# synthesizer-project/synference

Measured on AMD Instinct MI355X. Metric: posterior samples/sec (accepted, prior-box rejection included), higher is better.
Workload: dtype f32

## Files before the change

include/synference_hip.h:

```cpp
#ifndef SYNFERENCE_HIP_H
#define SYNFERENCE_HIP_H

#include <stddef.h>
#include <stdint.h>

#ifdef __cplusplus
extern "C" {
#endif

typedef struct sf_flow sf_flow;
typedef struct sf_opt sf_opt;

enum sf_status {
  SF_OK = 0,
  SF_ERR_INVALID = -1,
  SF_ERR_HIP = -2,
  SF_ERR_NO_DEVICE = -3,
  SF_ERR_STATE = -4
};

enum sf_kind { SF_MAF = 0, SF_NSF = 1, SF_NSF_AR = 2, SF_MAF_AR = 3 };

typedef struct sf_flow_desc {
  int32_t kind;
  int32_t D;
  int32_t C;
  int32_t H;
  int32_t T;
  int32_t K;
  int32_t NB;
  int32_t scale_fn;
  int32_t hidden_bf16;
  float tail_bound;
  float min_bin_width;
  float min_bin_height;
  float min_derivative;
  float maf_eps;
  float lu_eps;
  const float* theta_mean;
  const float* theta_std;
  const float* x_mean;
  const float* x_std;
  const int32_t* perms;
  float ar_slope;
} sf_flow_desc;

int sf_flow_create(const sf_flow_desc* desc, sf_flow** out);
void sf_flow_destroy(sf_flow* f);
int64_t sf_flow_num_params(const sf_flow* f);
int64_t sf_flow_packed_size(const sf_flow* f);

int sf_flow_set_params(sf_flow* f, const float* flat, int64_t n, int is_device, void* stream);

int sf_flow_get_params(sf_flow* f, float* flat, int64_t n, int is_device, void* stream);

int sf_flow_pack_table(const sf_flow* f, int32_t* src1, int32_t* src2, int64_t n_packed);
int64_t sf_flow_packed16_size(const sf_flow* f);
int sf_flow_pack_table16(const sf_flow* f, int32_t* src1, int32_t* src2, int64_t n_packed16);
int64_t sf_flow_packed16b_size(const sf_flow* f);
int sf_flow_pack_table16b(const sf_flow* f, int32_t* src, int64_t n);
int64_t sf_flow_trainc_size(const sf_flow* f);
int64_t sf_flow_trainc_grad_size(const sf_flow* f);
int sf_flow_trainc_table(const sf_flow* f, int32_t* src1, int32_t* src2, int64_t n, int32_t* gdst, int64_t n_params,
                         int32_t* desc , float* cst, int64_t n_cst);
int64_t sf_flow_cst_size(const sf_flow* f);
int sf_flow_train_path(const sf_flow* f, int64_t B, int want_dctx);
int sf_flow_describe(const sf_flow* f, char* buf, size_t buflen);

int sf_flow_log_prob(sf_flow* f, const float* theta , const float* x ,
                     int64_t B, float* out , void* stream);

int sf_flow_log_prob_grad(sf_flow* f, const float* theta , const float* x, int64_t rows_per_x, int64_t B,
                          float* lp , float* dtheta , void* stream);

int sf_map_step(int64_t B, int64_t D, float* phi , float* exp_avg , float* exp_avg_sq ,
                float* theta , const float* lp , const float* g_theta , const float* lo ,
                const float* hi , float* best_theta , float* best_lp , float learning_rate,
                int64_t step, int save_best, void* stream);

int sf_flow_inverse_from_noise(sf_flow* f, const float* z , const float* x ,
                               int64_t B, float* theta , float* logdet ,
                               void* stream);
int sf_flow_inverse_from_noise_sampler(sf_flow* f, const float* z , const float* x , int64_t B,
                                       float* theta , void* stream);
int sf_set_sampler_fp32(int on);

int sf_flow_sample_round(sf_flow* f, const float* x , int64_t S,
                         const uint32_t* slots, int64_t slot_base, int64_t n_slots,
                         uint32_t attempt, int32_t attempts_per_slot, uint64_t seed, uint32_t stream_id,
                         const float* lo , const float* hi ,
                         float* out , uint32_t* rejected, uint32_t* n_rejected,
                         int32_t* n_drawn, void* stream);

int sf_flow_prepare_context(sf_flow* f, const float* x , int64_t M, void* stream);
int sf_flow_release_context(sf_flow* f);

int sf_flow_sample(sf_flow* f, const float* x , int64_t M, int64_t S,
                   const float* lo, const float* hi, uint64_t seed, int32_t max_attempts,
                   float* out , int32_t* n_drawn , int64_t* n_unfilled ,
                   void* stream);

int sf_flow_set_sample_row_offset(sf_flow* f, int64_t row_offset);
int sf_flow_set_sample_output_f64(sf_flow* f, int on);
int sf_flow_set_sample_time_limit(sf_flow* f, double seconds);

int sf_flow_sample_slots(sf_flow* f, const float* x , int64_t M, int64_t S,
                         const uint32_t* slots, int64_t n_slots, const float* lo, const float* hi, uint64_t seed,
                         int32_t max_attempts, float* out , int64_t* n_unfilled , void* stream);

int sf_flow_sample_stats(const sf_flow* f, float* stats4);

int sf_flow_acceptance(sf_flow* f, const float* x , int64_t M, int64_t n,
                       const float* lo, const float* hi, uint64_t seed,
                       int32_t* count , void* stream);

int sf_flow_loss_grad(sf_flow* f, const float* flat , const float* theta, const float* x,
                      int64_t B, float grad_scale, float* loss , float* grad ,
                      void* stream);

int sf_flow_loss_grad_rows(sf_flow* f, const float* flat, const float* theta , const float* x ,
                           const int64_t* rows , int64_t B, float grad_scale, const float* weights,
                           float* loss, double* loss_sum, float* grad, float* dctx, void* stream);


int sf_flow_loss_grad_weighted(sf_flow* f, const float* flat, const float* theta, const float* x,
                               int64_t B, float grad_scale, const float* weights ,
                               float* loss, float* grad, float* dctx , void* stream);

int sf_flow_set_profiling(sf_flow* f, int on);
int sf_flow_train_stats(sf_flow* f, float* kernel_ms );

typedef struct sf_adam_desc {
  float lr, beta1, beta2, eps, weight_decay;
  int32_t decoupled;
} sf_adam_desc;
int sf_opt_create(int64_t n, const sf_adam_desc* d, sf_opt** out);
void sf_opt_destroy(sf_opt* o);
int sf_adam_step(sf_opt* o, float* params, const float* grad, float max_norm,
                 float* grad_norm_out, void* stream);
int sf_adam_apply(float* params, const float* grad, float* exp_avg, float* exp_avg_sq, int64_t n,
                  const sf_adam_desc* d, int64_t step, float max_norm, float* scratch, void* stream);

int sf_flow_train_epoch(sf_flow* f, float* flat, const float* theta, const float* x, const int64_t* order,
                        int64_t n_batches, int64_t batch, float grad_scale, float* exp_avg, float* exp_avg_sq,
                        const sf_adam_desc* d, int64_t step0, float max_norm, float* scratch ,
                        float* grad , double* loss_sum, void* stream);

#define SF_COMM_ID_BYTES 128
typedef struct sf_comm sf_comm;
int sf_comm_set_library(const char* path);
int sf_comm_library(char* path_out, int64_t cap, int* version_out);
int sf_comm_unique_id(void* id_out, int64_t bytes);
int sf_comm_create(const void* id, int64_t bytes, int nranks, int rank, sf_comm** out);
void sf_comm_destroy(sf_comm* c);
int sf_comm_info(const sf_comm* c, int* nranks, int* rank);
int sf_comm_all_reduce_sum(sf_comm* c, float* buf , int64_t n, void* stream);
int sf_flow_train_epoch_dp(sf_flow* f, float* flat, const float* theta, const float* x, const int64_t* order,
                           int64_t n_batches, int64_t batch, float grad_scale, float* exp_avg, float* exp_avg_sq,
                           const sf_adam_desc* d, int64_t step0, float max_norm, float* scratch ,
                           float* grad , double* loss_sum, sf_comm* comm, void* stream);
int sf_opt_state(sf_opt* o, float** exp_avg, float** exp_avg_sq, int64_t** step_host);

typedef struct sf_mlp sf_mlp;
enum sf_act { SF_ACT_SILU = 0, SF_ACT_RELU = 1, SF_ACT_TANH = 2 };
typedef struct sf_mlp_desc {
  int32_t n_in;
  int32_t n_layers;
  int32_t widths[4];
  int32_t act;
  const float* x_mean;
  const float* x_std;
} sf_mlp_desc;
int sf_mlp_create(const sf_mlp_desc* d, sf_mlp** out);
void sf_mlp_destroy(sf_mlp* m);
int64_t sf_mlp_num_params(const sf_mlp* m);
int sf_mlp_forward(sf_mlp* m, const float* flat, const float* x , int64_t B,
                   float* out , void* stream);
int sf_mlp_backward(sf_mlp* m, const float* flat, const float* x, const float* dout ,
                    int64_t B, float* grad , void* stream);

int sf_quantiles(const float* samples , int64_t N, int64_t S, int32_t D,
                 const float* q , int32_t Q, float* out , void* stream);
int sf_quantiles_large(const float* samples , int64_t N, int64_t S, int32_t D,
                       const float* q , int32_t Q, float* out , void* stream);

int sf_flux_to_abmag(const float* flux_njy, const float* err_njy, int64_t n, float mag_limit,
                     float* mag, float* mag_err, void* stream);

int sf_flux_to_asinh(const float* flux_njy, const float* err_njy, int64_t N, int32_t C, const float* f_b_njy ,
                     float* mag, float* mag_err, void* stream);

int sf_scatter_depths(const float* flux , int64_t N, int32_t C, const float* sigma, int32_t n_sigma_rows,
                      int32_t n_scatters, float min_flux_pc_error, uint64_t seed,
                      float* out , float* err_out, void* stream);

#define SF_NOISE_KIND_GENERAL 0
#define SF_NOISE_KIND_ASINH 1
#define SF_NOISE_SPACE_PHYSICAL 0
#define SF_NOISE_SPACE_AB 1
#define SF_NOISE_SPACE_ASINH 2
#define SF_NOISE_FLUX_SCATTER 0
#define SF_NOISE_FLUX_LIMIT 1
#define SF_NOISE_FLUX_NUMBER 2
typedef struct sf_noise_band {
  int32_t kind;
  int32_t interp_space;
  int32_t in_space;
  int32_t out_space;
  int32_t n_bins;
  int32_t table_offset;
  int32_t extrapolate;
  int32_t resample;
  int32_t upper_limits;
// ... 134 lines not shown
```

synference_amd/_lib.py:

```python
from __future__ import annotations

import ctypes as C
import os
from pathlib import Path

_HERE = Path(__file__).resolve().parent
LIB_PATH = _HERE / "lib" / "libsynference_hip.so"

c_f32p = C.POINTER(C.c_float)
c_i32p = C.POINTER(C.c_int32)
c_u32p = C.POINTER(C.c_uint32)


class sf_flow_desc(C.Structure):
    _fields_ = [
        ("kind", C.c_int32), ("D", C.c_int32), ("C", C.c_int32), ("H", C.c_int32),
        ("T", C.c_int32), ("K", C.c_int32), ("NB", C.c_int32), ("scale_fn", C.c_int32),
        ("hidden_bf16", C.c_int32),
        ("tail_bound", C.c_float), ("min_bin_width", C.c_float), ("min_bin_height", C.c_float),
        ("min_derivative", C.c_float), ("maf_eps", C.c_float), ("lu_eps", C.c_float),
        ("theta_mean", c_f32p), ("theta_std", c_f32p), ("x_mean", c_f32p), ("x_std", c_f32p),
        ("perms", c_i32p), ("ar_slope", C.c_float),
    ]


class sf_mlp_desc(C.Structure):
    _fields_ = [("n_in", C.c_int32), ("n_layers", C.c_int32), ("widths", C.c_int32 * 4), ("act", C.c_int32),
                ("x_mean", c_f32p), ("x_std", c_f32p)]


class sf_adam_desc(C.Structure):
    _fields_ = [("lr", C.c_float), ("beta1", C.c_float), ("beta2", C.c_float), ("eps", C.c_float),
                ("weight_decay", C.c_float), ("decoupled", C.c_int32)]


class sf_noise_band(C.Structure):
    _fields_ = [(n, C.c_int32) for n in ("kind", "interp_space", "in_space", "out_space", "n_bins", "table_offset",
                                         "extrapolate", "resample", "upper_limits", "has_limit", "flux_rule", "replace_err")] + \
               [(n, C.c_float) for n in ("in_to_unit", "zp_in", "zp_unit", "zp_out", "unit_to_out", "in_to_jy", "unit_per_jy",
                                         "jy_per_unit", "b_jy", "sigma_clip", "snr_threshold", "limit_value", "flux_number",
                                         "std_at_limit", "err_value", "min_err", "max_err")]


class sf_spectra_desc(C.Structure):
    _fields_ = [(n, C.c_void_p) for n in ("flux", "wave", "z", "sigma_pixels", "observed_wave", "curve_wave", "curve_r",
                                          "theory_r_arr", "norm_table", "out")] + \
               [(n, C.c_int64) for n in ("N", "ld_flux", "ld_out", "sigma_stride")] + \
               [(n, C.c_int32) for n in ("mode", "L", "M", "n_curve", "col0", "norm_frame", "unit_code", "med_lo", "med_hi",
                                         "h_limit")] + \
               [("theory_r", C.c_double), ("trunc", C.c_double)] + \
               [(n, C.c_float) for n in ("unit_scale", "clip_lo", "clip_hi")]


class sf_c2st_desc(C.Structure):
    _fields_ = [(n, C.c_int32) for n in ("n_in", "width", "n_cls", "max_iter", "n_iter_no_change", "early_stopping", "batch")] + \
               [("R", C.c_int64), ("seed", C.c_uint64)] + \
               [(n, C.c_float) for n in ("lr", "beta1", "beta2", "eps", "alpha")] + \
               [("tol", C.c_double)] + \
               [(n, C.c_void_p) for n in ("rows", "labels", "vmask", "init_weights")]


PROTOTYPES = {
    "sf_flow_create": (C.c_int, [C.POINTER(sf_flow_desc), C.POINTER(C.c_void_p)]),
    "sf_flow_destroy": (None, [C.c_void_p]),
    "sf_flow_num_params": (C.c_int64, [C.c_void_p]),
    "sf_flow_packed_size": (C.c_int64, [C.c_void_p]),
    "sf_flow_set_params": (C.c_int, [C.c_void_p, C.c_void_p, C.c_int64, C.c_int, C.c_void_p]),
    "sf_flow_pack_table": (C.c_int, [C.c_void_p, c_i32p, c_i32p, C.c_int64]),
    "sf_flow_describe": (C.c_int, [C.c_void_p, C.c_char_p, C.c_size_t]),
    "sf_flow_log_prob": (C.c_int, [C.c_void_p, C.c_void_p, C.c_void_p, C.c_int64, C.c_void_p, C.c_void_p]),
    "sf_flow_log_prob_grad": (C.c_int, [C.c_void_p, C.c_void_p, C.c_void_p, C.c_int64, C.c_int64, C.c_void_p, C.c_void_p,
                                        C.c_void_p]),
    "sf_map_step": (C.c_int, [C.c_int64, C.c_int64, C.c_void_p, C.c_void_p, C.c_void_p, C.c_void_p, C.c_void_p, C.c_void_p,
                              C.c_void_p, C.c_void_p, C.c_void_p, C.c_void_p, C.c_float, C.c_int64, C.c_int, C.c_void_p]),
    "sf_flow_inverse_from_noise": (C.c_int, [C.c_void_p, C.c_void_p, C.c_void_p, C.c_int64, C.c_void_p,
                                             C.c_void_p, C.c_void_p]),
    "sf_flow_sample_round": (C.c_int, [C.c_void_p, C.c_void_p, C.c_int64, C.c_void_p, C.c_int64, C.c_int64,
                                       C.c_uint32, C.c_int32, C.c_uint64, C.c_uint32, C.c_void_p, C.c_void_p,
                                       C.c_void_p, C.c_void_p, C.c_void_p, C.c_void_p, C.c_void_p]),
    "sf_flux_to_asinh": (C.c_int, [C.c_void_p, C.c_void_p, C.c_int64, C.c_int32, C.c_void_p, C.c_void_p, C.c_void_p,
                                   C.c_void_p]),
    "sf_scatter_depths": (C.c_int, [C.c_void_p, C.c_int64, C.c_int32, C.c_void_p, C.c_int32, C.c_int32, C.c_float, C.c_uint64,
                                    C.c_void_p, C.c_void_p, C.c_void_p]),
    "sf_scatter_empirical": (C.c_int, [C.c_void_p, C.c_int64, C.c_int32, C.POINTER(sf_noise_band), c_f32p, C.c_int64, C.c_int32,
                                       C.c_uint64, C.c_void_p, C.c_void_p, C.c_void_p]),
    "sf_apply_scalings": (C.c_int, [C.c_void_p, C.c_void_p, C.c_int64, C.c_int32, C.POINTER(sf_noise_band), c_f32p, C.c_int64,
                                    C.c_void_p, C.c_void_p, C.c_void_p]),
    "sf_spectra_transform": (C.c_int, [C.POINTER(sf_spectra_desc), C.c_void_p]),
    "sf_pit_ranks": (C.c_int, [C.c_void_p, C.c_void_p, C.c_int64, C.c_int64, C.c_int32, C.c_void_p, C.c_void_p]),
    "sf_tarp_coverage": (C.c_int, [C.c_void_p, C.c_void_p, C.c_int64, C.c_int64, C.c_int32, C.c_void_p, C.c_int32, C.c_int32,
                                   C.c_int32, C.c_int32, C.c_uint64, C.c_void_p, C.c_void_p, C.c_void_p, C.c_void_p,
                                   C.c_void_p]),
    "sf_copy_to_host_f64": (C.c_int, [C.c_void_p, C.c_void_p, C.c_int64, C.c_void_p]),
    "sf_flow_packed16_size": (C.c_int64, [C.c_void_p]),
    "sf_flow_pack_table16": (C.c_int, [C.c_void_p, C.c_void_p, C.c_void_p, C.c_int64]),
    "sf_flow_packed16b_size": (C.c_int64, [C.c_void_p]),
    "sf_flow_inverse_from_noise_sampler": (C.c_int, [C.c_void_p, C.c_void_p, C.c_void_p, C.c_int64, C.c_void_p, C.c_void_p]),
    "sf_set_sampler_fp32": (C.c_int, [C.c_int]),
    "sf_flow_set_sample_row_offset": (C.c_int, [C.c_void_p, C.c_int64]),
    "sf_flow_train_path": (C.c_int, [C.c_void_p, C.c_int64, C.c_int]),
    "sf_flow_trainc_size": (C.c_int64, [C.c_void_p]),
    "sf_flow_trainc_grad_size": (C.c_int64, [C.c_void_p]),
    "sf_flow_cst_size": (C.c_int64, [C.c_void_p]),
    "sf_flow_trainc_table": (C.c_int, [C.c_void_p, C.c_void_p, C.c_void_p, C.c_int64, C.c_void_p, C.c_int64, C.c_void_p,
                                       C.c_void_p, C.c_int64]),
    "sf_flow_pack_table16b": (C.c_int, [C.c_void_p, C.c_void_p, C.c_int64]),
    "sf_flow_get_params": (C.c_int, [C.c_void_p, C.c_void_p, C.c_int64, C.c_int, C.c_void_p]),
    "sf_flow_prepare_context": (C.c_int, [C.c_void_p, C.c_void_p, C.c_int64, C.c_void_p]),
    "sf_flow_release_context": (C.c_int, [C.c_void_p]),
    "sf_flow_sample": (C.c_int, [C.c_void_p, C.c_void_p, C.c_int64, C.c_int64, C.c_void_p, C.c_void_p,
                                 C.c_uint64, C.c_int32, C.c_void_p, C.c_void_p, C.POINTER(C.c_int64),
                                 C.c_void_p]),
    "sf_flow_sample_slots": (C.c_int, [C.c_void_p, C.c_void_p, C.c_int64, C.c_int64, C.c_void_p, C.c_int64, C.c_void_p,
                                       C.c_void_p, C.c_uint64, C.c_int32, C.c_void_p, C.POINTER(C.c_int64), C.c_void_p]),
    "sf_flow_sample_stats": (C.c_int, [C.c_void_p, C.POINTER(C.c_float)]),
    "sf_flow_acceptance": (C.c_int, [C.c_void_p, C.c_void_p, C.c_int64, C.c_int64, C.c_void_p, C.c_void_p,
                                     C.c_uint64, C.c_void_p, C.c_void_p]),
    "sf_flow_loss_grad": (C.c_int, [C.c_void_p, C.c_void_p, C.c_void_p, C.c_void_p, C.c_int64, C.c_float,
                                    C.c_void_p, C.c_void_p, C.c_void_p]),
    "sf_flow_loss_grad_rows": (C.c_int, [C.c_void_p, C.c_void_p, C.c_void_p, C.c_void_p, C.c_void_p, C.c_int64,
                                         C.c_float, C.c_void_p, C.c_void_p, C.c_void_p, C.c_void_p, C.c_void_p,
                                         C.c_void_p]),
    "sf_flow_train_epoch": (C.c_int, [C.c_void_p, C.c_void_p, C.c_void_p, C.c_void_p, C.c_void_p, C.c_int64, C.c_int64,
                                      C.c_float, C.c_void_p, C.c_void_p, C.POINTER(sf_adam_desc), C.c_int64, C.c_float,
                                      C.c_void_p, C.c_void_p, C.c_void_p, C.c_void_p]),
    "sf_flow_train_epoch_dp": (C.c_int, [C.c_void_p, C.c_void_p, C.c_void_p, C.c_void_p, C.c_void_p, C.c_int64, C.c_int64,
                                         C.c_float, C.c_void_p, C.c_void_p, C.POINTER(sf_adam_desc), C.c_int64, C.c_float,
                                         C.c_void_p, C.c_void_p, C.c_void_p, C.c_void_p, C.c_void_p]),
    "sf_comm_set_library": (C.c_int, [C.c_char_p]),
    "sf_comm_library": (C.c_int, [C.c_char_p, C.c_int64, C.POINTER(C.c_int)]),
    "sf_comm_unique_id": (C.c_int, [C.c_void_p, C.c_int64]),
    "sf_comm_create": (C.c_int, [C.c_void_p, C.c_int64, C.c_int, C.c_int, C.POINTER(C.c_void_p)]),
    "sf_comm_destroy": (None, [C.c_void_p]),
    "sf_comm_info": (C.c_int, [C.c_void_p, C.POINTER(C.c_int), C.POINTER(C.c_int)]),
    "sf_comm_all_reduce_sum": (C.c_int, [C.c_void_p, C.c_void_p, C.c_int64, C.c_void_p]),
    "sf_flow_loss_grad_weighted": (C.c_int, [C.c_void_p, C.c_void_p, C.c_void_p, C.c_void_p, C.c_int64,
                                             C.c_float, C.c_void_p, C.c_void_p, C.c_void_p, C.c_void_p,
                                             C.c_void_p]),
    "sf_flow_set_sample_time_limit": (C.c_int, [C.c_void_p, C.c_double]),
    "sf_flow_set_sample_output_f64": (C.c_int, [C.c_void_p, C.c_int]),
    "sf_flow_set_profiling": (C.c_int, [C.c_void_p, C.c_int]),
    "sf_flow_train_stats": (C.c_int, [C.c_void_p, C.POINTER(C.c_float)]),
    "sf_opt_create": (C.c_int, [C.c_int64, C.POINTER(sf_adam_desc), C.POINTER(C.c_void_p)]),
    "sf_opt_destroy": (None, [C.c_void_p]),
    "sf_adam_step": (C.c_int, [C.c_void_p, C.c_void_p, C.c_void_p, C.c_float, C.c_void_p, C.c_void_p]),
    "sf_adam_apply": (C.c_int, [C.c_void_p, C.c_void_p, C.c_void_p, C.c_void_p, C.c_int64,
                                C.POINTER(sf_adam_desc), C.c_int64, C.c_float, C.c_void_p, C.c_void_p]),
    "sf_opt_state": (C.c_int, [C.c_void_p, C.POINTER(C.c_void_p), C.POINTER(C.c_void_p),
                               C.POINTER(C.POINTER(C.c_int64))]),
    "sf_mlp_create": (C.c_int, [C.POINTER(sf_mlp_desc), C.POINTER(C.c_void_p)]),
    "sf_mlp_destroy": (None, [C.c_void_p]),
    "sf_mlp_num_params": (C.c_int64, [C.c_void_p]),
    "sf_mlp_forward": (C.c_int, [C.c_void_p, C.c_void_p, C.c_void_p, C.c_int64, C.c_void_p, C.c_void_p]),
    "sf_mlp_backward": (C.c_int, [C.c_void_p, C.c_void_p, C.c_void_p, C.c_void_p, C.c_int64, C.c_void_p,
                                  C.c_void_p]),
    "sf_quantiles": (C.c_int, [C.c_void_p, C.c_int64, C.c_int64, C.c_int32, C.c_void_p, C.c_int32, C.c_void_p,
                               C.c_void_p]),
    "sf_quantiles_large": (C.c_int, [C.c_void_p, C.c_int64, C.c_int64, C.c_int32, C.c_void_p, C.c_int32, C.c_void_p,
                                     C.c_void_p]),
    "sf_impute_missing": (C.c_int, [C.c_void_p, C.c_int64, C.c_int32, c_i32p, c_i32p, C.c_int32, C.c_void_p, C.c_void_p,
                                    C.c_void_p, C.c_int64, C.c_int64, C.c_float, C.c_float, C.c_float, C.c_int32, C.c_int32,
                                    C.c_float, C.c_int32, C.c_uint64, C.c_void_p, C.c_void_p, C.c_void_p, C.c_void_p,
                                    C.c_void_p, C.c_void_p, C.c_int64, C.c_void_p, C.c_void_p]),
    "sf_knn": (C.c_int, [C.c_void_p, C.c_int64, C.c_int32, C.c_void_p, C.c_int64, C.c_int32, C.c_int32, C.c_int64, C.c_void_p,
                         C.c_void_p, C.c_void_p]),
    "sf_kde_logsumexp": (C.c_int, [C.c_void_p, C.c_int64, C.c_int32, C.c_void_p, C.c_int64, C.c_void_p, C.c_void_p]),
    "sf_c2st_create": (C.c_int, [C.POINTER(sf_c2st_desc), C.POINTER(C.c_void_p), C.c_void_p]),
    "sf_c2st_destroy": (None, [C.c_void_p]),
    "sf_c2st_num_params": (C.c_int64, [C.c_void_p]),
    "sf_c2st_train": (C.c_int, [C.c_void_p, C.c_int32, C.c_int32, C.c_int32, C.c_int32, C.POINTER(C.c_int32), C.c_void_p]),
    "sf_c2st_scores": (C.c_int, [C.c_void_p, C.c_int32, C.c_int32, C.c_void_p, C.c_int64, C.c_void_p, C.c_void_p, C.c_void_p]),
    "sf_c2st_get": (C.c_int, [C.c_void_p, C.c_void_p, C.c_void_p, C.c_void_p, C.c_void_p]),
    "sf_flux_to_abmag": (C.c_int, [C.c_void_p, C.c_void_p, C.c_int64, C.c_float, C.c_void_p, C.c_void_p, C.c_void_p]),
    "sf_last_error": (C.c_char_p, []),
    "sf_version": (C.c_char_p, []),
    "sf_device_count": (C.c_int, []),
}

_lib = None


def load() -> C.CDLL:
    global _lib
    if _lib is not None:
        return _lib
    path = Path(os.environ.get("SYNFERENCE_HIP_LIB", LIB_PATH))
    if not path.exists():
        raise RuntimeError(
            f"{path} not found: build it with `python -c 'import __graft_entry__ as g; g.build()'` "
            "(hipcc --offload-arch=gfx950).  There is no CPU fallback for the flow engine.")
    lib = C.CDLL(str(path))
    for name, (res, args) in PROTOTYPES.items():
        fn = getattr(lib, name)
        fn.restype = res
        fn.argtypes = args
    _lib = lib
    return lib


def ptr(t):
    return None if t is None else C.c_void_p(t.data_ptr())


def stream_ptr(device):
    import torch
    return C.c_void_p(torch.cuda.current_stream(device).cuda_stream)


def check(rc: int) -> None:
    if rc != 0:
        msg = load().sf_last_error().decode("utf-8", "replace")
        raise RuntimeError(f"synference_hip error {rc}: {msg}")
```

synference_amd/csrc/sf_api.hip:

```cpp
#include <hip/hip_runtime.h>

#include <chrono>
#include <cmath>
#include <cstdio>
#include <cstdlib>
#include <cstring>
#include <string>
#include <vector>

#include "sf_internal.h"
#include "sf_train.h"
#include "sf_nsf1.h"
#include "sf_nsfar.h"
#include "sf_nsfc.h"
#include "sf_trainc.h"

namespace {
thread_local std::string g_err;

int hip_fail(hipError_t e, const char* what) {
  return sf_fail(SF_ERR_HIP, std::string(what) + ": " + hipGetErrorString(e));
}
}

static int ensure_device(sf_flow* f) {
  if (f->dev_ready) return SF_OK;
  int n = 0;
  if (hipGetDeviceCount(&n) != hipSuccess || n == 0)
    return sf_fail(SF_ERR_NO_DEVICE, "no HIP device visible: the gfx950 flow engine has no CPU fallback");
  SfFlowDev d;
  if (f->nsf1 || f->nsfar) {
    SF_TRY_SET(d.d_flat.alloc((size_t)f->L.n_params));
    static_cast<SfFlowDev&>(*f) = std::move(d);
    f->dev_ready = true;
    return SF_OK;
  }
  const size_t np = (size_t)f->L.n_packed;
  SF_TRY_SET(d.d_packed.alloc(np));
  SF_TRY_SET(hipMemset(d.d_packed, 0, np * sizeof(float)));
  SF_TRY_SET(d.d_cst.upload(f->L.cst));
  SF_TRY_SET(d.d_s1.alloc(np));
  SF_TRY_SET(d.d_s2.alloc(np));
  SF_TRY_SET(hipMemcpy(d.d_s1, f->L.src1.data(), np * sizeof(int32_t), hipMemcpyHostToDevice));
  SF_TRY_SET(hipMemcpy(d.d_s2, f->L.src2.data(), np * sizeof(int32_t), hipMemcpyHostToDevice));
  if ((f->L.dev.m16_ok || f->L.nsfS.ok) && f->L.n_packed16 > 0) {
    const size_t n16 = (size_t)f->L.n_packed16;
    SF_TRY_SET(d.d_packed16.alloc(n16));
    SF_TRY_SET(d.d_s16a.alloc(n16));
    SF_TRY_SET(d.d_s16b.alloc(n16));
    SF_TRY_SET(hipMemcpy(d.d_s16a, f->L.src16a.data(), n16 * sizeof(int32_t), hipMemcpyHostToDevice));
    SF_TRY_SET(hipMemcpy(d.d_s16b, f->L.src16b.data(), n16 * sizeof(int32_t), hipMemcpyHostToDevice));
  }
  if ((f->L.dev.m16_ok || f->L.nsfS.ok) && f->L.n_packed16B > 0) {
    const size_t nB = (size_t)f->L.n_packed16B;
    SF_TRY_SET(d.d_packed16B.alloc(nB));
    SF_TRY_SET(d.d_s16B.alloc(nB));
    SF_TRY_SET(hipMemcpy(d.d_s16B, f->L.src16B.data(), nB * sizeof(int32_t), hipMemcpyHostToDevice));
  }
  if (f->L.n_packedB > 0) {
    SF_TRY_SET(d.d_packedB.alloc((size_t)f->L.n_packedB));
    SF_TRY_SET(d.d_bsrc.alloc((size_t)f->L.n_packedB));
    SF_TRY_SET(hipMemcpy(d.d_bsrc, f->L.srcB.data(), (size_t)f->L.n_packedB * sizeof(int32_t), hipMemcpyHostToDevice));
  }
  SF_TRY_SET(d.d_flat.alloc((size_t)f->L.n_params));
  SF_TRY_SET(d.d_cnt.alloc(SF_MAX_ROUNDS));
  SF_TRY_SET(d.h_cnt.alloc(SF_MAX_ROUNDS));
  SF_TRY_SET(d.ev_dense[0].create());
  SF_TRY_SET(d.ev_dense[1].create());
  static_cast<SfFlowDev&>(*f) = std::move(d);
  f->dev_ready = true;
  return SF_OK;
}

sf_flow::~sf_flow() {
  sf_nsf1_destroy(nsf1);
  sf_nsfar_destroy(nsfar);
}

extern "C" {

const char* sf_last_error(void) { return g_err.c_str(); }
const char* sf_version(void) { return "synference_hip 0.2 (gfx950; mfma_f32_32x32x2 / 16x16x4)"; }
int sf_device_count(void) {
  int n = 0;
  if (hipGetDeviceCount(&n) != hipSuccess) return 0;
  return n;
}

int sf_flow_create(const sf_flow_desc* desc, sf_flow** out) {
  if (!desc || !out) return sf_fail(SF_ERR_INVALID, "null argument");
  if (desc->kind == SF_NSF && desc->D == 1) {
    sf_flow* f1 = new sf_flow();
    std::string err;
    int rc = sf_nsf1_create(*desc, &f1->nsf1, err);
    if (rc) { delete f1; return sf_fail(rc, err); }
    std::memset(&f1->L.dev, 0, sizeof(f1->L.dev));
    std::memset(&f1->L.trc, 0, sizeof(f1->L.trc));
    std::memset(&f1->L.nsc, 0, sizeof(f1->L.nsc));
    std::memset(&f1->L.nsfS, 0, sizeof(f1->L.nsfS));
    SfDev& v = f1->L.dev;
    v.kind = SF_NSF; v.D = 1; v.C = desc->C; v.H = desc->H; v.T = desc->T; v.K = desc->K; v.NB = desc->NB;
    f1->L.n_params = (int64_t)desc->T * f1->nsf1->P_mlp;
    *out = f1;
    return SF_OK;
  }
  if (desc->kind == SF_NSF_AR || desc->kind == SF_MAF_AR) {
    sf_flow* fa = new sf_flow();
    std::string err;
    int rc = sf_nsfar_create(*desc, &fa->nsfar, err);
    if (rc) { delete fa; return sf_fail(rc, err); }
    std::memset(&fa->L.dev, 0, sizeof(fa->L.dev));
    std::memset(&fa->L.trc, 0, sizeof(fa->L.trc));
    std::memset(&fa->L.nsc, 0, sizeof(fa->L.nsc));
    std::memset(&fa->L.nsfS, 0, sizeof(fa->L.nsfS));
    SfDev& v = fa->L.dev;
    v.kind = desc->kind; v.D = desc->D; v.C = desc->C; v.H = desc->H; v.T = desc->T; v.K = desc->K; v.NB = desc->NB;
    fa->L.n_params = fa->nsfar->n_params;
    *out = fa;
    return SF_OK;
  }
  sf_flow* f = new sf_flow();
  if (!sf_build_layout(*desc, f->L)) {
    std::string e = f->L.error;
    delete f;
    return sf_fail(SF_ERR_INVALID, e);
  }
  *out = f;
  return SF_OK;
}

void sf_flow_destroy(sf_flow* f) { delete f; }

int64_t sf_flow_num_params(const sf_flow* f) { return f ? f->L.n_params : 0; }
int64_t sf_flow_packed_size(const sf_flow* f) { return !f ? 0 : (f->nsfar ? (int64_t)f->nsfar->src.size() : f->L.n_packed); }

int sf_flow_pack_table(const sf_flow* f, int32_t* src1, int32_t* src2, int64_t n_packed) {
  if (!f || !src1 || !src2) return sf_fail(SF_ERR_INVALID, "null argument");
  if (f->nsfar) {
    if (n_packed != (int64_t)f->nsfar->src.size()) return sf_fail(SF_ERR_INVALID, "n_packed mismatch");
    std::memcpy(src1, f->nsfar->src.data(), (size_t)n_packed * sizeof(int32_t));
    for (int64_t i = 0; i < n_packed; ++i) src2[i] = -1;
    return SF_OK;
  }
  if (n_packed != f->L.n_packed) return sf_fail(SF_ERR_INVALID, "n_packed mismatch");
  if (n_packed == 0) return SF_OK;
  std::memcpy(src1, f->L.src1.data(), (size_t)n_packed * sizeof(int32_t));
  std::memcpy(src2, f->L.src2.data(), (size_t)n_packed * sizeof(int32_t));
  return SF_OK;
}

int64_t sf_flow_packed16_size(const sf_flow* f) { return (f && f->L.dev.m16_ok) ? f->L.n_packed16 : 0; }

int sf_flow_pack_table16(const sf_flow* f, int32_t* src1, int32_t* src2, int64_t n_packed16) {
  if (!f || !src1 || !src2) return sf_fail(SF_ERR_INVALID, "null argument");
  if (!f->L.dev.m16_ok || n_packed16 != f->L.n_packed16) return sf_fail(SF_ERR_INVALID, "no 16-row image or size mismatch");
  std::memcpy(src1, f->L.src16a.data(), (size_t)n_packed16 * sizeof(int32_t));
  std::memcpy(src2, f->L.src16b.data(), (size_t)n_packed16 * sizeof(int32_t));
  return SF_OK;
}

int64_t sf_flow_packed16b_size(const sf_flow* f) { return (f && f->L.dev.m16_ok) ? f->L.n_packed16B : 0; }

int sf_flow_pack_table16b(const sf_flow* f, int32_t* src, int64_t n) {
  if (!f || !src) return sf_fail(SF_ERR_INVALID, "null argument");
  if (!f->L.dev.m16_ok || n != f->L.n_packed16B) return sf_fail(SF_ERR_INVALID, "no split-bf16 image or size mismatch");
  std::memcpy(src, f->L.src16B.data(), (size_t)n * sizeof(int32_t));
  return SF_OK;
}

int64_t sf_flow_trainc_size(const sf_flow* f) { return (f && (f->L.trc.ok || f->L.nsc.ok)) ? f->L.n_imgC : 0; }
int64_t sf_flow_trainc_grad_size(const sf_flow* f) { return (f && (f->L.trc.ok || f->L.nsc.ok)) ? f->L.n_gradC : 0; }
int64_t sf_flow_cst_size(const sf_flow* f) { return f ? (int64_t)f->L.cst.size() : 0; }
int sf_flow_trainc_table(const sf_flow* f, int32_t* src1, int32_t* src2, int64_t n, int32_t* gdst, int64_t n_params,
                         int32_t* desc, float* cst, int64_t n_cst) {
  if (!f || !src1 || !src2 || !gdst || !desc || !cst) return sf_fail(SF_ERR_INVALID, "null argument");
  if ((!f->L.trc.ok && !f->L.nsc.ok) || n != f->L.n_imgC || n_params != f->L.n_params || n_cst != (int64_t)f->L.cst.size())
    return sf_fail(SF_ERR_INVALID, "no cooperative training image or size mismatch");
  static_assert(sizeof(SfTrcDev) <= 64 * sizeof(int32_t) && sizeof(SfNscDev) <= 64 * sizeof(int32_t), "descriptor words");
  std::memcpy(src1, f->L.srcC1.data(), (size_t)n * sizeof(int32_t));
  std::memcpy(src2, f->L.srcC2.data(), (size_t)n * sizeof(int32_t));
  std::memcpy(gdst, f->L.gdstC.data(), (size_t)n_params * sizeof(int32_t));
  std::memset(desc, 0, 64 * sizeof(int32_t));
  if (f->L.trc.ok) std::memcpy(desc, &f->L.trc, sizeof(SfTrcDev));
  else std::memcpy(desc, &f->L.nsc, sizeof(SfNscDev));
  std::memcpy(cst, f->L.cst.data(), (size_t)n_cst * sizeof(float));
  return SF_OK;
}

int sf_flow_describe(const sf_flow* f, char* buf, size_t buflen) {
  if (!f || !buf) return sf_fail(SF_ERR_INVALID, "null argument");
  const SfDev& v = f->L.dev;
  std::string s = "{";
  auto add = [&](const char* k, long val) { s += "\"" + std::string(k) + "\": " + std::to_string(val) + ", "; };
  if (f->nsfar) {
    const SfNsfAr& n = *f->nsfar;
    add("kind", n.affine ? SF_MAF_AR : SF_NSF_AR); add("D", n.D); add("C", n.C); add("H", n.H); add("T", n.T); add("K", n.K); add("NB", 2);
    add("Hp", n.Hp); add("t_stride", n.t_stride); add("n_params", (long)n.n_params); add("n_packed", (long)n.src.size());
    add("o_L0t", n.o_L0t); add("o_b0", n.o_b0); add("o_L1t", n.o_L1t); add("o_L1m", n.o_L1m); add("o_b1", n.o_b1);
    add("o_L2t", n.o_L2t); add("o_b2", n.o_b2); add("o_L0m", n.o_L0m); add("o_L2m", n.o_L2m); add("lds_bytes_train", (long)sf_nsfar_lds_bytes(n, 3));
    add("sampler_tiles16", sf_nsfar16_eligible(n) ? 1 : 0); add("s16_nt", n.s16_nt); add("s16_ni", n.s16_ni); add("s16_ks", n.s16_ks); add("s16_tpt", n.s16_tpt);
    add("o_F0", n.o_F0); add("o_fb0", n.o_fb0); add("o_F1", n.o_F1); add("o_fb1", n.o_fb1); add("o_F2", n.o_F2);
    auto arr = [&](const char* k, const std::vector<int32_t>& a, bool last) {
      s += "\"" + std::string(k) + "\": [";
      for (size_t i = 0; i < a.size(); ++i) s += std::to_string(a[i]) + (i + 1 < a.size() ? ", " : "");
      s += last ? "]}" : "], ";
    };
    arr("perm", n.perm, false); arr("ptype", n.ptype, false); arr("tend", n.tend, false); arr("ord", n.ord, false); arr("dimof", n.dimof, true);
    if (s.size() + 1 > buflen) return sf_fail(SF_ERR_INVALID, "buffer too small");
    std::memcpy(buf, s.c_str(), s.size() + 1);
    return SF_OK;
  }
  add("kind", v.kind); add("D", v.D); add("C", v.C); add("H", v.H); add("T", v.T); add("K", v.K);
  add("NB", v.NB); add("HT", v.HT); add("PT", v.PT); add("KMAX", v.KMAX); add("JP", v.JP);
  add("nGu", v.nGu); add("nGc", v.nGc); add("nGh", v.nGh); add("t_stride", v.t_stride);
  add("o_w0", v.o_w0); add("o_wc", v.o_wc); add("o_b0", v.o_b0); add("o_wk0", v.o_wk[0]);
  add("o_bk0", v.o_bk[0]); add("o_wk1", v.o_wk[1]); add("o_bk1", v.o_bk[1]); add("o_wf", v.o_wf);
  add("o_wk2", v.o_wk[2]); add("o_bk2", v.o_bk[2]); add("o_wk3", v.o_wk[3]); add("o_bk3", v.o_bk[3]);
  add("scale_fn", v.scale_fn);
  add("o_bf", v.o_bf); add("o_winu", v.o_winu); add("o_winc", v.o_winc); add("o_bin", v.o_bin);
  add("o_wg0", v.o_wg[0]); add("o_bg0", v.o_bg[0]); add("o_w10", v.o_w1[0]); add("o_b10", v.o_b1[0]);
  add("o_w20", v.o_w2[0]); add("o_b20", v.o_b2[0]); add("o_wg1", v.o_wg[1]); add("o_bg1", v.o_bg[1]);
  add("o_w11", v.o_w1[1]); add("o_b11", v.o_b1[1]); add("o_w21", v.o_w2[1]); add("o_b21", v.o_b2[1]);
  add("o_wout", v.o_wout); add("o_bout", v.o_bout); add("o_lu", v.o_lu);
  add("c_pscale", v.c_pscale); add("c_pshift", v.c_pshift); add("c_tdim", v.c_tdim);
  add("c_xmean", v.c_xmean); add("c_xstd", v.c_xstd); add("c_dslot", v.c_dslot);
  add("nsf_split_sampler", f->L.nsfS.ok); add("trainc_ok", f->L.trc.ok); add("nsfc_ok", f->L.nsc.ok);
  add("inc_ok", v.inc_ok); add("hidden_bf16", v.hidden_bf16); add("tB_stride", v.tB_stride); add("n_parts", v.n_parts); add("part_max", v.part_max);
  add("n_params", f->L.n_params); add("n_packed", f->L.n_packed);
  {
    int R = 0, NV = 0;
    SfDev vv = v;
    vv.packed16 = reinterpret_cast<const float*>(1);
    sf_ctab_shape(vv, R, NV);
    add("ctab_floats_per_galaxy", (long)v.T * NV * R);
  }
  add("o16_w0", v.o16_w0); add("o16_wc", v.o16_wc); add("o16_b0", v.o16_b0); add("o16_wk0", v.o16_wk[0]);
  add("o16_wk1", v.o16_wk[1]); add("o16_bk0", v.o16_bk[0]); add("o16_bk1", v.o16_bk[1]); add("o16_hv", v.o16_hv);
  add("o16_hvb", v.o16_hvb); add("o16_wh", v.o16_wh); add("o16_bh", v.o16_bh); add("o16_wp", v.o16_wp); add("t16_a_tab", v.t16_a_tab);
  add("t16_a", v.t16_a); add("t16B_stride", v.t16B_stride); add("nP16", v.nP16); add("o16B_wk0", v.o16B_wk[0]); add("o16B_wk1", v.o16B_wk[1]);
  add("m16_ok", v.m16_ok); add("m16_span", v.m16_span); add("nT16", v.nT16); add("nC16", v.nC16); add("t16_stride", v.t16_stride);
  s += "\"g16_tile\": [";
  for (int i = 0; i < SF_DMAX; ++i) s += std::to_string(v.g16_tile[i]) + (i + 1 < SF_DMAX ? ", " : "], ");
  s += "\"g16_lo\": [";
  for (int i = 0; i < SF_DMAX; ++i) s += std::to_string(v.g16_lo[i]) + (i + 1 < SF_DMAX ? ", " : "], ");
  s += "\"g_kend\": [";
  for (int i = 0; i < SF_DMAX; ++i) s += std::to_string(v.g_kend[i]) + (i + 1 < SF_DMAX ? ", " : "], ");
  s += "\"g_lo\": [";
  for (int i = 0; i < SF_DMAX; ++i) s += std::to_string(v.g_lo[i]) + (i + 1 < SF_DMAX ? ", " : "], ");
  s += "\"g_tile\": [";
  for (int i = 0; i < SF_DMAX; ++i) s += std::to_string(v.g_tile[i]) + (i + 1 < SF_DMAX ? ", " : "], ");
  s += "\"mt_kend\": [";
  for (int i = 0; i < 4; ++i) s += std::to_string(v.mt_kend[i]) + (i + 1 < 4 ? ", " : "], ");
  s += "\"cst\": [";
  for (size_t i = 0; i < f->L.cst.size(); ++i) {
    char t[40];
    std::snprintf(t, sizeof(t), "%.9g%s", f->L.cst[i], i + 1 < f->L.cst.size() ? ", " : "");
    s += t;
  }
  s += "]}";
  if (s.size() + 1 > buflen) return sf_fail(SF_ERR_INVALID, "buffer too small");
  std::memcpy(buf, s.c_str(), s.size() + 1);
  return SF_OK;
}

int sf_flow_set_params(sf_flow* f, const float* flat, int64_t n, int is_device, void* stream) {
  if (!f || !flat) return sf_fail(SF_ERR_INVALID, "null argument");
  if (n != f->L.n_params) return sf_fail(SF_ERR_INVALID, "parameter count mismatch");
  int rc = ensure_device(f);
  if (rc) return rc;
  hipStream_t st = (hipStream_t)stream;
  SF_TRY_SET(hipMemcpyAsync(f->d_flat, flat, (size_t)n * sizeof(float), is_device ? hipMemcpyDeviceToDevice : hipMemcpyHostToDevice, st));
  const float* src = f->d_flat;
  f->flat_valid = true;
  f->gt_image_valid = false;
  if (f->nsf1) { f->params_set = true; return SF_OK; }
  if (f->nsfar) {
    std::string err;
    rc = sf_nsfar_pack(f->nsfar, src, st, err);
    if (rc) return sf_fail(rc, err);
    f->params_set = true;
    return SF_OK;
  }
  SF_TRY_SET(sf_launch_pack(src, f->d_s1, f->d_s2, f->d_packed, (long)f->L.n_packed, st));
  if (f->d_packed16) SF_TRY_SET(sf_launch_pack(src, f->d_s16a, f->d_s16b, f->d_packed16, (long)f->L.n_packed16, st));
  f->wp_stale = true;
  if (f->d_packed16B) SF_TRY_SET(sf_launch_pack_bf16_split(src, f->d_s16B, f->d_packed16B, (long)f->L.n_packed16B, st));
  f->packed16_stale = false;
  if (f->L.n_packedB > 0) SF_TRY_SET(sf_launch_pack_bf16(src, f->d_bsrc, f->d_packedB, (long)f->L.n_packedB, st));
  f->params_set = true;
  f->ctab_x = nullptr;
  return SF_OK;
}

int sf_flow_get_params(sf_flow* f, float* flat, int64_t n, int is_device, void* stream) {
  if (!f || !flat) return sf_fail(SF_ERR_INVALID, "null argument");
  if (n != f->L.n_params) return sf_fail(SF_ERR_INVALID, "parameter count mismatch");
  if (!f->params_set || !f->flat_valid)
    return sf_fail(SF_ERR_STATE, "no parameters held by the handle: after sf_flow_loss_grad the caller's vector is the master copy "
                              "(call sf_flow_set_params first)");
  hipStream_t st = (hipStream_t)stream;
  SF_TRY_SET(hipMemcpyAsync(flat, f->d_flat, (size_t)n * sizeof(float), is_device ? hipMemcpyDeviceToDevice : hipMemcpyDeviceToHost, st));
  if (!is_device) SF_TRY_SET(hipStreamSynchronize(st));
  return SF_OK;
}

int sf_flow_log_prob(sf_flow* f, const float* theta, const float* x, int64_t B, float* out, void* stream) {
  if (!f) return sf_fail(SF_ERR_INVALID, "null handle");
  if (B == 0) return SF_OK;
  if (!theta || !x || !out) return sf_fail(SF_ERR_INVALID, "null argument");
  if (!f->params_set) return sf_fail(SF_ERR_STATE, "sf_flow_set_params has not been called");
  if (B < 0) return sf_fail(SF_ERR_INVALID, "B < 0");
  if (f->nsf1) {
    std::string err;
    int rc = sf_nsf1_log_prob(f->nsf1, f->d_flat, theta, x, (long)B, out, (hipStream_t)stream, err);
    return rc ? sf_fail(rc, err) : SF_OK;
  }
  if (f->nsfar) {
    std::string err;
    int rc = sf_nsfar_log_prob(f->nsfar, theta, x, (long)B, out, (hipStream_t)stream, err);
    return rc ? sf_fail(rc, err) : SF_OK;
  }
  SF_TRY_SET(sf_launch_logprob(f->dev(), theta, x, (long)B, out, (hipStream_t)stream));
  return SF_OK;
}

int sf_flow_inverse_from_noise(sf_flow* f, const float* z, const float* x, int64_t B, float* theta,
                               float* logdet, void* stream) {
  if (!f) return sf_fail(SF_ERR_INVALID, "null handle");
  if (B == 0) return SF_OK;
  if (!z || !x || !theta) return sf_fail(SF_ERR_INVALID, "null argument");
  if (!f->params_set) return sf_fail(SF_ERR_STATE, "sf_flow_set_params has not been called");
  if (f->nsf1) {
    std::string err;
    int rc = sf_nsf1_inverse(f->nsf1, f->d_flat, z, x, (long)B, theta, logdet, (hipStream_t)stream, err);
    return rc ? sf_fail(rc, err) : SF_OK;
  }
  if (f->nsfar) {
    std::string err;
    int rc = sf_nsfar_inverse(f->nsfar, z, x, (long)B, theta, logdet, (hipStream_t)stream, err);
    return rc ? sf_fail(rc, err) : SF_OK;
  }
  SfSampleArgsHost a;
  a.x = x; a.z_in = z; a.n_items = (long)B; a.out = theta; a.logdet_out = logdet;
  SF_TRY_SET(sf_launch_inverse(f->dev(), a, (hipStream_t)stream));
  return SF_OK;
}

static void nsf_sampler_view(const sf_flow* f, SfDev& m);
static SfDev sampler_dev(const sf_flow* f, const float* x);
int sf_flow_inverse_from_noise_sampler(sf_flow* f, const float* z, const float* x, int64_t B, float* theta, void* stream) {
  if (!f) return sf_fail(SF_ERR_INVALID, "null handle");
  if (B == 0) return SF_OK;
  if (!z || !x || !theta) return sf_fail(SF_ERR_INVALID, "null argument");
  if (!f->params_set) return sf_fail(SF_ERR_STATE, "sf_flow_set_params has not been called");
  if (f->nsf1 || f->nsfar) {
    int rc = sf_flow_inverse_from_noise(f, z, x, B, theta, nullptr, stream);
    return rc ? rc : 1;
  }
  if (f->L.dev.kind == SF_NSF) {
    SfDev ms = f->dev();
    nsf_sampler_view(f, ms);
    SfSampleArgsHost a;
    a.x = x; a.z_in = z; a.n_items = (long)B; a.out = theta;
    SF_TRY_SET(sf_launch_inverse(ms, a, (hipStream_t)stream));
    return ms.hidden_bf16 == 2 ? SF_OK : 1;
  }
  const SfDev m = f->dev();
  const SfMaf16Plan pl = sf_maf16_plan(m);
  if (!pl.sampler16) {
    SfSampleArgsHost a;
    a.x = x; a.z_in = z; a.n_items = (long)B; a.out = theta;
    SF_TRY_SET(sf_launch_inverse(m, a, (hipStream_t)stream));
    return 1;
  }
  if (pl.fp32) {
    int rc = sf_flow_prepare_context(f, x, B, stream);
    if (rc) return rc;
    const SfDev mt = sampler_dev(f, x);
    if (sf_maf16_plan(mt).fused) {
      SfSampleArgsHost a;
      a.x = x; a.z_in = z; a.n_items = (long)B; a.out = theta; a.S = 1;
      hipError_t e = sf_launch_maf_find16_zin(mt, a, (hipStream_t)stream);
      (void)sf_flow_release_context(f);
      if (e != hipSuccess) return hip_fail(e, "sf_launch_maf_find16_zin");
      return 3;
    }
    (void)sf_flow_release_context(f);
  }
  SF_TRY_SET(sf_launch_maf_inv16b_hook(m, z, x, (long)B, theta, (hipStream_t)stream));
  return pl.fp32 ? 2 : SF_OK;
}

extern "C++" {
static int g_sampler_fp32 = -2;
void sf_sampler_fp32_set(int on) { g_sampler_fp32 = on < 0 ? -1 : (on ? 1 : 0); }
int sf_sampler_fp32_get() {
  if (g_sampler_fp32 == -2) { const char* e = std::getenv("SF_SAMPLER_FP32"); g_sampler_fp32 = (e && *e) ? (std::atoi(e) != 0 ? 1 : 0) : -1; }
  return g_sampler_fp32;
}
int sf_sampler_fp32_for(int kind) {
  const int g = sf_sampler_fp32_get();
  return g < 0 ? (kind == SF_MAF ? 1 : 0) : g;
}
}
int sf_set_sampler_fp32(int on) {
  sf_sampler_fp32_set(on);
  return SF_OK;
}

int sf_flow_train_path(const sf_flow* f, int64_t B, int want_dctx) {
  if (!f) return sf_fail(SF_ERR_INVALID, "null handle");
  if (f->nsf1) return 4;
  if (f->nsfar) return 5;
  if (B > 0 && sf_trainc_eligible(f->L, want_dctx != 0)) return sf_trainc_groups((long)B, &f->L.trc, f->L.dev.T);
  if (B > 0 && sf_nsfc_eligible(f->L, want_dctx != 0)) return 3;
  return 0;
}

static void seed_keys(uint64_t seed, uint32_t stream_id, uint32_t& k0, uint32_t& k1) {
  k0 = (uint32_t)(seed & 0xffffffffu);
  k1 = (uint32_t)(seed >> 32) ^ stream_id;
}

static size_t ctab_limit_bytes() {
  static long v = -1;
  if (v < 0) {
    const char* e = std::getenv("SF_CTAB_MAX_MB");
    v = e ? std::atol(e) : 4096;
  }
  return (size_t)v << 20;
}

int sf_flow_prepare_context(sf_flow* f, const float* x, int64_t M, void* stream) {
  if (!f) return sf_fail(SF_ERR_INVALID, "null handle");
  f->ctab_x = nullptr;
  f->ctab_M = 0;
  if (M == 0) return SF_OK;
  if (!x) return sf_fail(SF_ERR_INVALID, "null argument");
  if (M < 0) return sf_fail(SF_ERR_INVALID, "M < 0");
  if (!f->params_set) return sf_fail(SF_ERR_STATE, "sf_flow_set_params has not been called");
  if (f->nsf1 || f->nsfar) return SF_OK;
  SfDev m = f->dev();
  int R = 0, NV = 0;
  sf_ctab_shape(m, R, NV);
  const size_t need = (size_t)M * m.T * NV * R;
  if (need == 0 || need * sizeof(float) > ctab_limit_bytes()) return SF_OK;
  SF_TRY_SET(f->d_ctab.grow(need));
  m.ctab_R = R; m.ctab_NV = NV;
  if (f->wp_stale && m.kind == SF_MAF && m.m16_ok && m.packed16 && m.o16_wp >= 0) {
    SF_TRY_SET(sf_launch_maf_fuse16(m, (hipStream_t)stream));
    f->wp_stale = false;
  }
  SF_TRY_SET(sf_launch_ctab(m, x, (long)M, f->d_ctab, (hipStream_t)stream));
  f->ctab_x = x;
  f->ctab_M = M;
  return SF_OK;
}

int sf_flow_release_context(sf_flow* f) {
  if (!f) return sf_fail(SF_ERR_INVALID, "null handle");
  f->ctab_x = nullptr;
  f->ctab_M = 0;
  return SF_OK;
}

static void nsf_sampler_view(const sf_flow* f, SfDev& m) {
  const SfNsfSamp& s = f->L.nsfS;
  if (m.kind != SF_NSF || !s.ok || m.hidden_bf16 || !f->d_packed16 || !f->d_packed16B || f->packed16_stale || sf_sampler_fp32_for(SF_NSF)) return;
  m.packed = f->d_packed16;
  m.t_stride = s.t_stride;
  m.o_winu = s.o_winu; m.o_winc = s.o_winc; m.o_bin = s.o_bin; m.o_wout = s.o_wout; m.o_bout = s.o_bout; m.o_lu = s.o_lu;
  for (int k = 0; k < SF_NBMAX; ++k) {
    m.o_wg[k] = s.o_wg[k]; m.o_bg[k] = s.o_bg[k]; m.o_b1[k] = s.o_b1[k]; m.o_b2[k] = s.o_b2[k];
    m.o_w1[k] = 0; m.o_w2[k] = 0;
    m.oB_w1[k] = s.oB_w1[k]; m.oB_w2[k] = s.oB_w2[k];
  }
  m.n_parts = s.n_parts; m.part_max = s.part_floats_max; m.part_bytes_max = s.part_bytes_max; m.head_part = s.head_part;
  for (int p = 0; p < 5; ++p) { m.part_off[p] = s.part_off[p]; m.partB_off[p] = s.partB_off[p]; }
  for (int k = 0; k < SF_NBMAX; ++k) m.blk_part[k] = s.blk_part[k];
  m.packedB = f->d_packed16B;
  m.tB_stride = s.tB_stride;
  m.hidden_bf16 = 2;
  m.packed16 = nullptr; m.packed16B = nullptr;
}
static SfDev sampler_dev(const sf_flow* f, const float* x) {
  SfDev m = f->dev();
  if (f->ctab_x != nullptr && f->ctab_x == x) {
    sf_ctab_shape(m, m.ctab_R, m.ctab_NV);
    m.ctab = f->d_ctab;
  }
  nsf_sampler_view(f, m);
  return m;
}

int sf_flow_sample_round(sf_flow* f, const float* x, int64_t S, const uint32_t* slots, int64_t slot_base,
                         int64_t n_slots, uint32_t attempt, int32_t attempts_per_slot, uint64_t seed,
                         uint32_t stream_id,
                         const float* lo, const float* hi, float* out, uint32_t* rejected,
                         uint32_t* n_rejected, int32_t* n_drawn, void* stream) {
  if (!f || !x || !out || !rejected || !n_rejected) return sf_fail(SF_ERR_INVALID, "null argument");
  if (f->nsf1 || f->nsfar) return sf_fail(SF_ERR_INVALID, "sf_flow_sample_round is not offered for the one-parameter / autoregressive NSF: use sf_flow_sample / sf_flow_sample_slots");
  if (!f->params_set) return sf_fail(SF_ERR_STATE, "sf_flow_set_params has not been called");
  if (S < 1 || S > 0x7fffffffll) return sf_fail(SF_ERR_INVALID, "S must be in 1 .. 2^31-1");
  if ((lo == nullptr) != (hi == nullptr)) return sf_fail(SF_ERR_INVALID, "lo and hi must be given together");
  if ((uint64_t)(slot_base + n_slots) > 0xffffffffull)
    return sf_fail(SF_ERR_INVALID, "slot ids must fit 32 bits: split the catalogue");
  const int A = attempts_per_slot;
  if (A < 1 || A > 32 || (A & (A - 1))) return sf_fail(SF_ERR_INVALID, "attempts_per_slot must be 1,2,4,8,16 or 32");
  SfSampleArgsHost a;
  a.x = x; a.S = (long)S; a.slots = slots; a.slot_base = (long)slot_base; a.n_items = (long)n_slots * A;
  a.attempts_per_slot = A; a.attempt = attempt; seed_keys(seed, stream_id, a.k0, a.k1);
  a.rng_slot_offset = (unsigned long long)f->sample_row_offset * (unsigned long long)S;
  a.lo = lo; a.hi = hi; a.out = out; a.rejected = rejected; a.n_rejected = n_rejected; a.n_drawn = n_drawn;
  if (f->ctab_x == x && (uint64_t)(slot_base + n_slots) > (uint64_t)f->ctab_M * (uint64_t)S && slots == nullptr)
    return sf_fail(SF_ERR_INVALID, "slots reach past the rows given to sf_flow_prepare_context");
  SF_TRY_SET(sf_launch_inverse(sampler_dev(f, x), a, (hipStream_t)stream));
  return SF_OK;
}

static int ensure_queue(sf_flow* f, int64_t n_slots, int64_t M) {
  if (!f->d_queue) SF_TRY_SET(f->d_queue.alloc(1));
  if (!f->h_queue) SF_TRY_SET(f->h_queue.alloc(1));
  uint64_t cap = 1u << 16;
  while (cap < (uint64_t)n_slots && cap < (1ull << 20)) cap <<= 1;
  if (f->d_ring.cap() < cap) {
    SF_TRY_SET(f->d_ring.grow(cap));
    hipError_t e = hipMemset(f->d_ring, 0, cap * sizeof(unsigned long long));
    if (e != hipSuccess) { (void)f->d_ring.reset(); return hip_fail(e, "hipMemset(retry ring)"); }
    f->ring_dirty = false;
  }
  if (f->d_rej[0].cap() < (size_t)n_slots) {
    static_cast<SfFlowRej&>(*f) = SfFlowRej();
    SfFlowRej r;
    SF_TRY_SET(r.d_rej[0].alloc((size_t)n_slots));
    SF_TRY_SET(r.d_rej[1].alloc((size_t)n_slots));
    static_cast<SfFlowRej&>(*f) = std::move(r);
  }
  SF_TRY_SET(f->d_galacc.grow((size_t)M));
  return SF_OK;
}

static int sample_persistent(sf_flow* f, const float* x, int64_t M, int64_t S, const uint32_t* slots, int64_t n_slots,
                             const float* lo, const float* hi, uint64_t seed, int32_t max_attempts, float* out,
                             int32_t* n_drawn, int64_t* n_unfilled, hipStream_t st) {
  if (n_unfilled) *n_unfilled = 0;
  if (n_slots == 0) return SF_OK;
  if ((uint64_t)(M * S) > 0xfff00000ull) return sf_fail(SF_ERR_INVALID, "M*S must stay below 2^32 - 2^20: split the catalogue");
  int rc = ensure_queue(f, n_slots, M);
  if (rc) return rc;
  const bool capped = max_attempts > 0;
  const uint32_t ceiling = capped ? (uint32_t)max_attempts : 0x40000000u;
  {
    rc = sf_flow_prepare_context(f, x, M, (void*)st);
    if (rc) return rc;
  }
  const SfDev m = sampler_dev(f, x);
  SfSampleArgsHost a;
  a.x = x; a.S = (long)S; seed_keys(seed, 0, a.k0, a.k1);
  a.rng_slot_offset = (unsigned long long)f->sample_row_offset * (unsigned long long)S;
  a.lo = lo; a.hi = hi; a.out = out; a.n_drawn = n_drawn; a.out_f64 = f->sample_out_f64 ? 1 : 0;
  a.q = f->d_queue; a.ring = f->d_ring; a.ring_mask = (uint32_t)(f->d_ring.cap() - 1);
  a.out_slots = (uint32_t)(M * S);
  const uint32_t* cur = slots;
  int64_t pending = n_slots;
  const auto t_start = std::chrono::steady_clock::now();
  auto out_of_time = [&]() {
    return f->sample_time_limit_s > 0.0 &&
           std::chrono::duration<double>(std::chrono::steady_clock::now() - t_start).count() > f->sample_time_limit_s;
  };
  const bool fast16 = m.kind == SF_MAF && m.m16_ok && !m.hidden_bf16 && m.packed16 != nullptr;
  const uint32_t first_window = fast16 ? 1024u : 256u;
  uint32_t attempt = 0, limit = ceiling < first_window ? ceiling : first_window;
  int buf = 0, stage = 0;
  double evals = 0.0;
  float rej0 = 0.f;
  int64_t dropped = 0;
  const bool progress_rule = !capped;
  uint32_t acc_from = 64;
  const uint64_t S_rule = slots ? 1ull : (uint64_t)S;
  auto rule_due = [&](uint32_t att_now) { return progress_rule && (uint64_t)(att_now - acc_from) * S_rule >= 100000ull; };
  int64_t persist_min = 8192;
  {
    static long env_pm = -1;
    if (env_pm < 0) { const char* e = std::getenv("SF_PERSIST_MIN"); env_pm = e ? std::atol(e) : 0; }
    if (env_pm > 0) persist_min = env_pm;
  }
  for (;;) {
    if (f->ring_dirty) SF_TRY_SET(hipMemsetAsync(f->d_ring, 0, f->d_ring.cap() * sizeof(unsigned long long), st));
    f->ring_dirty = true;
    SF_TRY_SET(hipMemsetAsync(f->d_queue, 0, sizeof(SfQueue), st));
#ifdef SF_Q_STATS
    SF_TRY_SET(hipMemsetAsync(&f->d_queue->stats[10], 0xff, sizeof(unsigned long long), st));
#endif
    if (progress_rule && stage == 0) SF_TRY_SET(hipMemsetAsync(f->d_galacc, 0, (size_t)M * sizeof(int32_t), st));
    a.slots = cur; a.slot_base = 0; a.n_items = (long)pending; a.n_total = (uint32_t)pending;
    {
      static int env_il = -1;
      if (env_il < 0) { const char* e = std::getenv("SF_INTERLEAVE"); env_il = e ? std::atoi(e) : 128; }
      a.dense_G = (!cur && env_il > 0 && pending == M * S && M > 1 && (int64_t)env_il * S < (int64_t)1 << 31) ? (uint32_t)env_il : 0u;
      {
        uint32_t run = fast16 ? 16u : 32u;
        while (run > 1 && S % (int64_t)run != 0) run >>= 1;
        a.dense_run = run;
// ... 461 lines not shown
```

synference_amd/csrc/sf_internal.h:

```cpp
#pragma once
#include <hip/hip_runtime.h>
#include <stdint.h>

#include "sf_buf.h"
#include "sf_layout.h"
#include "sf_queue.h"

struct SfSampleArgsHost {
  const float* x = nullptr;
  const float* z_in = nullptr;
  long S = 1;
  const uint32_t* slots = nullptr;
  long slot_base = 0;
  long n_items = 0;
  uint32_t attempt = 0, k0 = 0, k1 = 0;
  unsigned long long rng_slot_offset = 0;
  int attempts_per_slot = 1;
  int log2_attempts = 0;
  const float* lo = nullptr;
  const float* hi = nullptr;
  float* out = nullptr;
  int out_f64 = 0;
  float* logdet_out = nullptr;
  uint32_t* rejected = nullptr;
  uint32_t* n_rejected = nullptr;
  int32_t* n_drawn = nullptr;
  int32_t* count = nullptr;
  uint32_t* best = nullptr;
  const uint32_t* att_list = nullptr;
  struct SfQueue* q = nullptr;
  unsigned long long* ring = nullptr;
  uint32_t ring_mask = 0;
  uint32_t attempt_limit = 0xffffffffu;
  uint32_t n_total = 0;
  uint32_t out_slots = 0;
  uint32_t dense_G = 0;
  uint32_t dense_run = 1;
  uint32_t list_mul = 0, list_log2 = 0;
  int32_t* gal_acc = nullptr;
#ifdef SF_Q_STATS
  uint32_t* qtrace = nullptr;
#endif
};
#ifdef __HIPCC__
__device__ __forceinline__ void sf_out_store(const SfSampleArgsHost& a, size_t idx, float v) {
  if (a.out_f64) reinterpret_cast<double*>(a.out)[idx] = (double)v;
  else a.out[idx] = v;
}
#endif


hipError_t sf_launch_logprob(const SfDev& m, const float* theta, const float* x, long B, float* out,
                             hipStream_t st);
hipError_t sf_launch_inverse(const SfDev& m, const SfSampleArgsHost& a, hipStream_t st);
bool sf_maf16_enabled(const SfDev& m, const SfSampleArgsHost& a);
hipError_t sf_launch_maf_inv16(const SfDev& m, const SfSampleArgsHost& a, hipStream_t st);
hipError_t sf_launch_maf_inv16b_hook(const SfDev& m, const float* z, const float* x, long n, float* out, hipStream_t st);
void sf_sampler_fp32_set(int on);
int sf_sampler_fp32_get();
int sf_sampler_fp32_for(int kind);
void sf_ctab_shape(const SfDev& m, int& R, int& NV);
hipError_t sf_launch_ctab(const SfDev& m, const float* x, long M, float* tab, hipStream_t st);
hipError_t sf_launch_maf_ctab16(const SfDev& m, const float* x, long M, float* tab, hipStream_t st);
hipError_t sf_launch_maf_fuse16(const SfDev& m, hipStream_t st);
struct SfMaf16Plan {
  bool ok16 = false;
  bool sampler16 = false;
  bool fp32 = false;
  bool span = false;
  bool head_mfma = false;
  int dd = 0;
  bool fused = false;
};
SfMaf16Plan sf_maf16_plan(const SfDev& m);
hipError_t sf_launch_maf_find16_zin(const SfDev& m, const SfSampleArgsHost& a, hipStream_t st);
hipError_t sf_launch_pack(const float* flat, const int32_t* s1, const int32_t* s2, float* packed, long n,
                          hipStream_t st);
hipError_t sf_launch_pack_bf16(const float* flat, const int32_t* src, unsigned short* out, long n, hipStream_t st);
hipError_t sf_launch_pack_bf16_split(const float* flat, const int32_t* src, unsigned short* out, long n, hipStream_t st);
hipError_t sf_launch_fill_nan_rows(float* out, const uint32_t* slots, long n, int D, hipStream_t st, int out_f64 = 0);
hipError_t sf_launch_fill_i32(int32_t* p, long n, int32_t v, hipStream_t st);
hipError_t sf_launch_exclusive_scan_i32(const int32_t* cnt, int n, int32_t* offs, int32_t* total, hipStream_t st);
hipError_t sf_launch_account_window(const uint32_t* list, const uint32_t* best, long n, long S, uint32_t a_lo, uint32_t A,
                                    int32_t* n_drawn, int32_t* gal_acc, hipStream_t st);
hipError_t sf_launch_filter_survivors(uint32_t* list, unsigned int* n_surv, long S, const int32_t* gal_acc, float* out,
                                      int D, hipStream_t st, int out_f64 = 0);

#include <string>
#define SF_MAX_DEVICES 16
struct SfAttrCache {
  bool done[SF_MAX_DEVICES] = {false};
  bool need(int& dev) {
    dev = 0;
    if (hipGetDevice(&dev) != hipSuccess || dev < 0 || dev >= SF_MAX_DEVICES) return true;
    return !done[dev];
  }
  void set(int dev) { if (dev >= 0 && dev < SF_MAX_DEVICES) done[dev] = true; }
};
struct SfResidentCache {
  int dev[8] = {-1, -1, -1, -1, -1, -1, -1, -1};
  size_t sh[8] = {0};
  int val[8] = {0};
  int n = 0;
  bool get(int d, size_t s, int& v) const {
    for (int i = 0; i < 8; ++i)
      if (dev[i] == d && sh[i] == s) { v = val[i]; return true; }
    return false;
  }
  void put(int d, size_t s, int v) { dev[n & 7] = d; sh[n & 7] = s; val[n & 7] = v; ++n; }
};
void sf_set_error(const std::string& msg);
int sf_fail(int code, const std::string& msg);
inline std::string sf_hip_message(const char* call, hipError_t e) {
  std::string s = std::string(call) + ": ";
  for (const char* op : {".alloc(", ".grow(", ".upload(", ".create("})
    if (s.find(op) != std::string::npos) { s += std::string(sf_buf_last_call()) + ": "; break; }
  return s + hipGetErrorString(e);
}
#define SF_TRY_ERR(call)                                                     \
  do {                                                                       \
    hipError_t e_ = (call);                                                  \
    if (e_ != hipSuccess) {                                                  \
      err = sf_hip_message(#call, e_);                                       \
      return SF_ERR_HIP;                                                     \
    }                                                                        \
  } while (0)
#define SF_TRY_SET(call)                                                                                   \
  do {                                                                                                     \
    hipError_t e_ = (call);                                                                                \
    if (e_ != hipSuccess) return sf_fail(SF_ERR_HIP, sf_hip_message(#call, e_));                          \
  } while (0)
struct sf_comm;
int sf_comm_all_reduce_impl(sf_comm* c, float* buf, long n, hipStream_t st);

#define SF_LOSS_PARTS 64
#define SF_MAX_ROUNDS 80
struct SfNsf1;
struct SfFlowDev {
  SfBuf<float> d_packed;
  SfBuf<float> d_cst;
  SfBuf<int32_t> d_s1, d_s2;
  SfBuf<float> d_packed16;
  SfBuf<int32_t> d_s16a, d_s16b;
  SfBuf<unsigned short> d_packed16B;
  SfBuf<int32_t> d_s16B;
  SfBuf<unsigned short> d_packedB;
  SfBuf<int32_t> d_bsrc;
  SfBuf<float> d_flat;
  SfBuf<uint32_t> d_cnt;
  SfPinned<uint32_t> h_cnt;
  SfEvent ev_dense[2];
};
struct SfFlowTrain {
  SfBuf<float> d_packedT;
  SfBuf<int32_t> d_t1, d_t2;
  SfBuf<float> d_gpacked;
  SfBuf<int32_t> d_gdst;
};
struct SfFlowTrainC {
  SfBuf<float> d_imgC;
  SfBuf<int32_t> d_sC1, d_sC2, d_gdstC;
  SfBuf<int32_t> d_gsrcC;
  SfBuf<int32_t> d_gzeroC;
  long n_gzeroC = 0;
};
struct SfFlowGt {
  SfBuf<float> d_gtT;
  SfBuf<int32_t> d_gt1, d_gt2;
};
struct SfFlowRej { SfBuf<uint32_t> d_rej[2]; };
struct sf_flow : SfFlowDev, SfFlowTrain, SfFlowTrainC, SfFlowGt, SfFlowRej {
  SfLayout L;
  struct SfNsfAr* nsfar = nullptr;
  SfNsf1* nsf1 = nullptr;
  ~sf_flow();
  bool dev_ready = false;
  bool params_set = false;
  bool train_ready = false;
  bool flat_valid = false;
  bool gt_image_valid = false;
  long gt_simds = 0;
  bool packed16_stale = false;
  SfBuf<float> d_gpartC;
  SfBuf<long long> d_gfixC;
  bool trainc_ready = false;
  SfBuf<float> d_ustash;
  SfBuf<float> d_act;
  SfBuf<SfQueue> d_queue;
  SfPinned<SfQueue> h_queue;
  SfBuf<unsigned long long> d_ring;
  bool ring_dirty = false;
  SfBuf<int32_t> d_galacc;
  SfBuf<uint32_t> d_best;
  SfBuf<float> d_sqpart;
  int n_sqpart = 0;
  bool want_sq = false;
  bool prep_lite = false;
  bool packed_stale = false;
  double* d_losspart = nullptr;
  SfBuf<double> d_losspart_mem;
  bool losspart_used = false;
  bool wp_stale = true;
  bool sample_out_f64 = false;
  long long sample_row_offset = 0;
  double sample_time_limit_s = 0.0;
  bool profiling = false;
  SfEvent ev_train[2];
  bool ev_train_valid = false;
  float last_stats[4] = {0.f, 0.f, 0.f, 0.f};
  SfBuf<float> d_ctab;
  const float* ctab_x = nullptr;
  int64_t ctab_M = 0;
  SfDev dev() const {
    SfDev v = L.dev;
    v.packed = d_packed;
    v.packedT = d_packedT;
    v.cst = d_cst;
    v.packedB = d_packedB;
    v.packed16 = packed16_stale ? nullptr : d_packed16.get();
    v.packed16B = reinterpret_cast<const uint32_t*>(d_packed16B.get());
    v.ctab = nullptr;
    return v;
  }
};

int sf_hostio_copy_f64(const float* dev_src, double* host_dst, int64_t n, hipStream_t stream, std::string& err);
```

synference_amd/csrc/sf_layout.cpp:

```cpp
#include "sf_layout.h"

#include <cmath>
#include <cstring>
#include <functional>

namespace {

struct Emitter {
  std::vector<int32_t>& s1;
  std::vector<int32_t>& s2;
  std::vector<int32_t>* gidx = nullptr;
  int64_t cur = 0;

  int64_t pad_to(int64_t align) {
    while (cur % align) push(-1, -1);
    return cur;
  }
  void push(int32_t a, int32_t b, int64_t g = -1) {
    s1.push_back(a);
    s2.push_back(b);
    if (gidx) gidx->push_back((int32_t)(g >= 0 ? g : cur));
    ++cur;
  }
  int64_t linear(int OT, int nG, const std::vector<int>& orow, const std::vector<int>& irow,
// ... 820 lines not shown
                  const int ro = l & 15, ri = 4 * (l >> 4) + r;
                  const int64_t idx = fn(ot, ro, it, ri);
                  pushC((int32_t)idx);
                  if (idx >= 0) L.gdstC[(size_t)idx] = (int32_t)(gbase_t + g_off + ((int64_t)ot * IT + it) * 256 + (ro & 3) * 64 + (ro >> 2) * 16 + ri);
                }
        };
        auto tr_block = [&](int ITr, int OTk, const WFn& fn) {
          for (int it = 0; it < ITr; ++it)
            for (int ot = 0; ot < OTk; ++ot)
              for (int l = 0; l < 64; ++l)
                for (int r = 0; r < 4; ++r) pushC((int32_t)fn(ot, 4 * (l >> 4) + r, it, l & 15));
        };
        auto bias_block = [&](int OT, const std::function<int64_t(int, int)>& f1, int64_t g_off) {
          for (int ot = 0; ot < OT; ++ot)
            for (int ro = 0; ro < 16; ++ro) {
              const int64_t a1 = f1(ot, ro);
              pushC((int32_t)a1);
              if (a1 >= 0) L.gdstC[(size_t)a1] = (int32_t)(gbase_t + g_off + ot * 16 + ro);
            }
        };
        auto w_in = [&](int ot, int ro, int it, int ri) -> int64_t {
          const int oo = hid_unit(ot, ro), cc = in_col(it, ri, false);
          return (oo >= 0 && cc >= 0) ? lWin + (int64_t)oo * in_dim + cc : -1;
        };
        auto w_gate = [&](int64_t base) {
          return [&, base](int ot, int ro, int it, int ri) -> int64_t {
            const int oo = hid_unit(ot, ro), cc = in_col(it, ri, true);
            return (oo >= 0 && cc >= 0) ? base + (int64_t)oo * C + cc : -1;
          };
        };
        auto w_hid = [&](int64_t base) {
          return [&, base](int ot, int ro, int it, int ri) -> int64_t {
            const int oo = hid_unit(ot, ro), ii = hid_unit(it, ri);
            return (oo >= 0 && ii >= 0) ? base + (int64_t)oo * H + ii : -1;
          };
        };
        auto w_out = [&](int ot, int ro, int it, int ri) -> int64_t {
          const int oo = q_row(ot, ro), ii = hid_unit(it, ri);
          return (oo >= 0 && ii >= 0) ? lWout + (int64_t)oo * H + ii : -1;
        };
        auto hid_bias = [&](int64_t base) {
          return [&, base](int ot, int ro) -> int64_t { const int oo = hid_unit(ot, ro); return oo >= 0 ? base + oo : -1; };
        };
        int oC; int64_t g;
#define SF_NSC_FWD(field_o, field_g, OT_, IT_, fn)                                   \
  oC = hereC(); g = gcur; gcur += (int64_t)(OT_) * (IT_) * 256; fwd_block(OT_, IT_, fn, g); \
  if (t == 0) { c.field_o = oC; c.field_g = (int)g; }
#define SF_NSC_BIAS(field_o, field_g, OT_, fn)                                       \
  oC = hereC(); g = gcur; gcur += (int64_t)(OT_) * 16; bias_block(OT_, fn, g);       \
  if (t == 0) { c.field_o = oC; c.field_g = (int)g; }
        SF_NSC_FWD(o_win, g_win, NT, NI, w_in)
        SF_NSC_BIAS(o_bin, g_bin, NT, hid_bias(lbin))
        for (int k = 0; k < 2; ++k) {
          SF_NSC_FWD(o_wg[k], g_wg[k], NT, NI, w_gate(lWg[k]))
          SF_NSC_BIAS(o_bg[k], g_bg[k], NT, hid_bias(lbg[k]))
          SF_NSC_FWD(o_w1[k], g_w1[k], NT, NT, w_hid(lW1[k]))
          SF_NSC_BIAS(o_b1[k], g_b1[k], NT, hid_bias(lb1[k]))
          SF_NSC_FWD(o_w2[k], g_w2[k], NT, NT, w_hid(lW2[k]))
          SF_NSC_BIAS(o_b2[k], g_b2[k], NT, hid_bias(lb2[k]))
        }
        SF_NSC_FWD(o_wout, g_wout, OTQ, NT, w_out)
        SF_NSC_BIAS(o_bout, g_bout, OTQ, [&](int ot, int ro) -> int64_t { const int oo = q_row(ot, ro); return oo >= 0 ? lbout + oo : -1; })
#undef SF_NSC_FWD
#undef SF_NSC_BIAS
        {
          oC = hereC(); g = gcur; gcur += 2 * 256 + 16;
          if (t == 0) { c.o_lu = oC; c.g_lu = (int)g; }
          auto gpos = [&](int blk, int ro, int ri) { return (int32_t)(gbase_t + g + blk * 256 + (ro & 3) * 64 + (ro >> 2) * 16 + ri); };
          std::vector<int32_t> Lm(64, -1), Um(64, -1);
          int n = 0;
          for (int i = 0; i < D; ++i)
            for (int j = 0; j < i; ++j) { Lm[i * 8 + j] = (int32_t)(lLo + n); L.gdstC[(size_t)(lLo + n)] = gpos(0, i, j); ++n; }
          n = 0;
          for (int i = 0; i < D; ++i)
            for (int j = i + 1; j < D; ++j) { Um[i * 8 + j] = (int32_t)(lUp + n); L.gdstC[(size_t)(lUp + n)] = gpos(1, i, j); ++n; }
          for (int i = 0; i < 64; ++i) pushC(Lm[i]);
          for (int i = 0; i < 64; ++i) pushC(Um[i]);
          for (int i = 0; i < 8; ++i) { pushC(i < D ? (int32_t)(lDi + i) : -1); if (i < D) L.gdstC[(size_t)(lDi + i)] = (int32_t)(gbase_t + g + 512 + 8 + i); }
          for (int i = 0; i < 8; ++i) { pushC(i < D ? (int32_t)(lBi + i) : -1); if (i < D) L.gdstC[(size_t)(lBi + i)] = (int32_t)(gbase_t + g + 512 + i); }
          while ((L.srcC1.size() - (size_t)tbC) % 16) pushC(-1);
        }
        oC = hereC(); tr_block(NT, OTQ, w_out);
        if (t == 0) c.o_woutT = oC;
        for (int k = 0; k < 2; ++k) {
          oC = hereC(); tr_block(NT, NT, w_hid(lW2[k]));
          if (t == 0) c.o_w2T[k] = oC;
          oC = hereC(); tr_block(NT, NT, w_hid(lW1[k]));
          if (t == 0) c.o_w1T[k] = oC;
        }
        oC = hereC(); tr_block(1, NT, w_in);
        if (t == 0) c.o_winT = oC;
        if (t == 0) c.g_stride = (int)((gcur + 63) / 64 * 64);
      }
    }
  }
  E.pad_to(64);
  ET.pad_to(64);
  while (L.srcB.size() % 64) L.srcB.push_back(-1);
  while (L.src16a.size() % 1024) { L.src16a.push_back(-1); L.src16b.push_back(-1); }
  if (T == 1) {
    v.t_stride = (int)E.cur; v.tT_stride = (int)ET.cur; v.tB_stride = (int)L.srcB.size();
    v.t16_stride = (int)L.src16a.size();
  }
  if (d.kind == SF_NSF && L.nsfS.ok) {
    while (L.src16a.size() % 64) { L.src16a.push_back(-1); L.src16b.push_back(-1); }
    while (L.src16B.size() % 64) L.src16B.push_back(-1);
    if (T == 1) { L.nsfS.t_stride = (int)L.src16a.size(); L.nsfS.tB_stride = (int)L.src16B.size(); }
    if (L.nsfS.tB_stride & 7) L.nsfS.ok = 0;
    if (L.nsfS.ok) {
      SfNsfSamp& sS = L.nsfS;
      const size_t budget = (size_t)152 * 1024;
      std::vector<int> cf{0}, cb{0};
      for (int k = 0; k < NB; ++k) { cf.push_back(sS.o_wg[k]); cb.push_back(sS.oB_w1[k]); }
      cf.push_back(sS.o_wout); cb.push_back(sS.tB_stride);
      cf.push_back(sS.t_stride); cb.push_back(sS.tB_stride);
      sS.n_parts = 0; sS.part_off[0] = 0; sS.partB_off[0] = 0;
      std::vector<int> item_part(cf.size() - 1, 0);
      int sf0 = 0, sb0 = 0;
      bool okp = true;
      for (size_t i = 0; i + 1 < cf.size() && okp; ++i) {
        const size_t item = (size_t)(cf[i + 1] - cf[i]) * 4 + (size_t)(cb[i + 1] - cb[i]) * 2;
        if (item > budget) { okp = false; break; }
        if ((size_t)(cf[i + 1] - sf0) * 4 + (size_t)(cb[i + 1] - sb0) * 2 > budget) {
          if (sS.n_parts >= 3) { okp = false; break; }
          ++sS.n_parts;
          sS.part_off[sS.n_parts] = cf[i]; sS.partB_off[sS.n_parts] = cb[i];
          sf0 = cf[i]; sb0 = cb[i];
        }
        item_part[i] = sS.n_parts;
      }
      if (okp) {
        ++sS.n_parts;
        sS.part_off[sS.n_parts] = cf.back(); sS.partB_off[sS.n_parts] = cb.back();
        sS.part_floats_max = 0; sS.part_bytes_max = 0;
        for (int p = 0; p < sS.n_parts; ++p) {
          const int pf = sS.part_off[p + 1] - sS.part_off[p], pb = sS.partB_off[p + 1] - sS.partB_off[p];
          sS.part_floats_max = std::max(sS.part_floats_max, pf);
          sS.part_bytes_max = std::max(sS.part_bytes_max, pf * 4 + pb * 2);
          if ((sS.partB_off[p] & 7) || (sS.part_off[p] & 3)) okp = false;
        }
        for (int k = 0; k < NB; ++k) sS.blk_part[k] = item_part[1 + k];
        sS.head_part = item_part[1 + NB];
      }
      if (!okp) sS.ok = 0;
    }
    if (!L.nsfS.ok) { L.src16a.clear(); L.src16b.clear(); L.src16B.clear(); }
  }
  L.n_packed16 = (int64_t)L.src16a.size();
  if (d.kind == SF_MAF) while (L.src16B.size() % 2048) L.src16B.push_back(-1);
  if (T == 1) v.t16B_stride = (int)(L.src16B.size() / 2);
  L.n_packed16B = (int64_t)L.src16B.size();
  if (!v.m16_ok && !L.nsfS.ok) { L.src16B.clear(); L.n_packed16B = 0; }
  if (v.m16_ok && (size_t)v.t16_stride * sizeof(float) > 152 * 1024) v.m16_ok = 0;
  L.n_packedB = (int64_t)L.srcB.size();
  {
    const int budget = 152 * 1024 / 4;
    std::vector<int> cuts;
    if (d.kind == SF_MAF) {
      cuts = {0, v.t_stride};
    } else {
      cuts.push_back(0);
      for (int k = 0; k < NB; ++k) cuts.push_back(v.o_wg[k]);
      cuts.push_back(v.o_wout);
      cuts.push_back(v.t_stride);
    }
    v.n_parts = 0;
    v.part_max = 0;
    bool ok = true;
    int start = 0;
    std::vector<int> item_part(cuts.size() - 1, 0);
    v.part_off[0] = 0;
    for (size_t i = 0; i + 1 < cuts.size(); ++i) {
      const int item = cuts[i + 1] - cuts[i];
      if (item > budget) { ok = false; break; }
      if (cuts[i + 1] - start > budget) {
        if (v.n_parts >= 3) { ok = false; break; }
        v.part_off[++v.n_parts] = cuts[i];
        start = cuts[i];
      }
      item_part[i] = v.n_parts;
    }
    if (ok) {
      v.part_off[++v.n_parts] = cuts.back();
      for (int p = 0; p < v.n_parts; ++p) v.part_max = std::max(v.part_max, v.part_off[p + 1] - v.part_off[p]);
      if (d.kind == SF_NSF) {
        for (int k = 0; k < NB; ++k) v.blk_part[k] = item_part[1 + k];
        v.head_part = item_part[1 + NB];
      }
    } else {
      v.n_parts = 0;
    }
    for (int p = 0; p < 5; ++p) v.partB_off[p] = p == 0 ? 0 : v.tB_stride;
    v.part_bytes_max = v.part_max * 4 + (v.hidden_bf16 ? v.tB_stride * 2 : 0);
    if (v.hidden_bf16) {
      const int need = v.t_stride + (v.tB_stride + 1) / 2;
      if (v.n_parts != 1 || need > budget)
        return fail("hidden_bf16: one transform's fp32 + bf16 operand images must fit the 152 KiB LDS budget");
    }
  }
  if (L.trc.ok || L.nsc.ok) {
    while (L.srcC1.size() % 256) { L.srcC1.push_back(-1); L.srcC2.push_back(-1); }
    if (T == 1) { L.trc.t_stride = (int)L.srcC1.size(); L.nsc.t_stride = (int)L.srcC1.size(); }
    L.n_imgC = (int64_t)L.srcC1.size();
    L.n_gradC = (int64_t)T * (L.trc.ok ? L.trc.g_stride : L.nsc.g_stride);
    L.gdstC.resize((size_t)P, -1);
  }
  L.n_packed = E.cur;
  L.n_packedT = ET.cur;
  L.n_params = P;
  L.gdst.assign((size_t)P, -1);
  for (int64_t i = 0; i < E.cur; ++i) {
    if (L.src1[i] >= 0 && L.gdst[L.src1[i]] < 0) L.gdst[L.src1[i]] = gidx[i];
    if (L.src2[i] >= 0 && L.gdst[L.src2[i]] < 0) L.gdst[L.src2[i]] = gidx[i];
  }
  return true;
}

bool sf_build_mlp_layout(const sf_mlp_desc& d, SfMlpLayout& L) {
  auto fail = [&](const std::string& m) { L.error = m; return false; };
  if (d.n_in < 1 || d.n_in > 512) return fail("n_in must be in 1..512");
  if (d.n_layers < 1 || d.n_layers > SF_MLP_LMAX) return fail("n_layers must be in 1..4");
  if (d.act < 0 || d.act > 2) return fail("unknown activation");
  int wmax = 0;
  for (int l = 0; l < d.n_layers; ++l) {
    if (d.widths[l] < 1 || d.widths[l] > 128) return fail("layer widths must be in 1..128");
    wmax = std::max(wmax, d.widths[l]);
  }
  SfMlpDev& v = L.dev;
  std::memset(&v, 0, sizeof(v));
  v.n_in = d.n_in; v.L = d.n_layers; v.act = d.act; v.n_out = d.widths[d.n_layers - 1];
  v.HT = ceil_div(wmax, 32);
  L.cst.assign(2 * ((d.n_in + 3) / 4) * 4, 1.f);
  for (int i = 0; i < d.n_in; ++i) {
    L.cst[i] = d.x_mean ? d.x_mean[i] : 0.f;
    L.cst[((d.n_in + 3) / 4) * 4 + i] = d.x_std ? d.x_std[i] : 1.f;
  }
  std::vector<int32_t> gidx;
  Emitter E{L.src1, L.src2, &gidx};
  Emitter ET{L.srcT1, L.srcT2, nullptr};
  int64_t P = 0;
  int in_w = d.n_in;
  for (int l = 0; l < d.n_layers; ++l) {
    const int out_w = d.widths[l];
    v.width[l] = out_w;
    v.nG[l] = ceil_div(in_w, 8);
    v.nGo[l] = ceil_div(out_w, 8);
    const int64_t lW = P, lb = lW + (int64_t)out_w * in_w;
    P = lb + out_w;
    E.pad_to(64);
    v.o_w[l] = (int)E.linear(v.HT, v.nG[l], iota_rows(out_w, v.HT * 32), iota_rows(in_w, v.nG[l] * 8), lW, in_w, 1, nullptr);
    v.o_b[l] = (int)E.bias(v.HT, iota_rows(out_w, v.HT * 32), lb, -1);
    if (l > 0) {
      ET.pad_to(64);
      v.oT_w[l] = (int)ET.linear(v.HT, v.nGo[l], iota_rows(in_w, v.HT * 32), iota_rows(out_w, v.nGo[l] * 8), lW, 1,
                                 in_w, nullptr);
    }
    in_w = out_w;
  }
  E.pad_to(64);
  ET.pad_to(64);
  L.n_packed = E.cur;
  L.n_packedT = ET.cur;
  L.n_params = P;
  L.gdst.assign((size_t)P, -1);
  for (int64_t i = 0; i < E.cur; ++i)
    if (L.src1[i] >= 0) L.gdst[L.src1[i]] = gidx[i];
  return true;
}
```

synference_amd/csrc/sf_layout.h:

```cpp
#pragma once
#include <cstdint>
#include <string>
#include <vector>

#include "../../include/synference_hip.h"

#define SF_DMAX 16
#define SF_NBMAX 4

struct SfDev {
  const float* packed;
  const float* packedT;
  const float* cst;
  int kind, D, C, H, T, K, NB, scale_fn;
  int HT;
  int PT;
  int KMAX;
  int JP;
  int nGu, nGc, nGh;
  int t_stride;
  int n_parts, part_off[5], part_max;
  int blk_part[SF_NBMAX], head_part;
  int partB_off[5], part_bytes_max;
  int o_w0, o_wc, o_b0;
  int o_wk[SF_NBMAX], o_bk[SF_NBMAX];
  int o_wf, o_bf;
  int o_hv, o_hvb;
  int o_winu, o_winc, o_bin;
  int o_wg[SF_NBMAX], o_bg[SF_NBMAX];
  int o_w1[SF_NBMAX], o_b1[SF_NBMAX], o_w2[SF_NBMAX], o_b2[SF_NBMAX];
  int o_wout, o_bout;
  int o_lu;
  int tT_stride;
  int nGf;
  int oT_wf, oT_wk[SF_NBMAX], oT_w0;
  int oT_wout, oT_w1[SF_NBMAX], oT_w2[SF_NBMAX], oT_winu;
  int oT_wc;
  int oT_wg[SF_NBMAX];
  int inc_ok;
  int g_tile[SF_DMAX], g_kend[SF_DMAX];
  int g_lo[SF_DMAX];
  int mt_kend[4];
  const unsigned short* packedB;
  int hidden_bf16, nKS, tB_stride;
  int oB_wk[SF_NBMAX], oB_w1[SF_NBMAX], oB_w2[SF_NBMAX];
  const float* packed16;
  int m16_ok, nT16, nC16, t16_stride;
  int t16_a;
  int t16_a_tab;
  int o16_wh, o16_bh;
  int o16_wp;
  const uint32_t* packed16B;
  int t16B_stride, nP16, o16B_wk[2];
  int m16_span;
  int o16_w0, o16_wc, o16_b0, o16_wk[2], o16_bk[2], o16_hv, o16_hvb;
  int g16_tile[SF_DMAX];
  int g16_lo[SF_DMAX];
  const float* ctab;
  int ctab_R, ctab_NV;
  int c_pscale, c_pshift, c_tdim, c_xmean, c_xstd;
  int c_dslot;
  float logdet0;
  float tail_bound, min_w, min_h, min_d, eps, lu_eps, inv_sqrt_h, deriv_const;
};

#define SF_PACK_TANH_SCALE (-2)
#define SF_PACK_SPLIT_SCALED (1 << 29)
#define SF_PACK_SPLIT_INDEX 0x1fffffff
#define SF_TANH_PRESCALE 2.8853900817779268f

struct SfTrcDev {
  int ok;
  int NT, NI;
  int t_stride, g_stride;
  int o_win, o_b0, o_w1, o_b1, o_w2, o_b2, o_wf, o_bf;
  int o_wfT, o_w2T, o_w1T, o_winT;
  int g_win, g_b0, g_w1, g_b1, g_w2, g_b2, g_wf, g_bf;
  int kend[4];
  int kbeg[4];
  int c_insrc;
  int c_jobs, n_jobs;
};

struct SfNscDev {
  int ok;
  int NT, NI, OTQ, KM;
  int kc_h, kc_in[3];
  int t_stride, g_stride;
  int o_win, o_bin, o_wg[2], o_bg[2], o_w1[2], o_b1[2], o_w2[2], o_b2[2], o_wout, o_bout, o_lu;
  int o_woutT, o_w2T[2], o_w1T[2], o_winT;
  int g_win, g_bin, g_wg[2], g_bg[2], g_w1[2], g_b1[2], g_w2[2], g_b2[2], g_wout, g_bout, g_lu;
};

struct SfNsfSamp {
  int ok;
  int t_stride;
  int o_winu, o_winc, o_bin, o_wg[SF_NBMAX], o_bg[SF_NBMAX], o_b1[SF_NBMAX], o_b2[SF_NBMAX], o_wout, o_bout, o_lu;
  int tB_stride;
  int oB_w1[SF_NBMAX], oB_w2[SF_NBMAX];
  int n_parts, part_off[5], partB_off[5], blk_part[SF_NBMAX], head_part, part_floats_max, part_bytes_max;
};

struct SfLayout {
  SfDev dev;
  SfNsfSamp nsfS;
  SfTrcDev trc;
  SfNscDev nsc;
  std::vector<int32_t> srcC1, srcC2;
  std::vector<int32_t> gdstC;
  int64_t n_imgC = 0, n_gradC = 0;
  int64_t n_params = 0;
  int64_t n_packed = 0;
  std::vector<int32_t> src1, src2;
  std::vector<int32_t> srcT1, srcT2;
  int64_t n_packedT = 0;
  std::vector<int32_t> gdst;
  std::vector<int32_t> srcB;
  std::vector<int32_t> src16a, src16b;
  std::vector<int32_t> src16B;
  int64_t n_packed16B = 0;
  int64_t n_packed16 = 0;
  int64_t n_packedB = 0;
  std::vector<float> cst;
  std::string error;
};

static inline int sf_tile_row(int r, int h) { return (r & 3) + 8 * (r >> 2) + 4 * h; }

bool sf_build_layout(const sf_flow_desc& d, SfLayout& L);

#define SF_MLP_LMAX 4
struct SfMlpDev {
  const float* packed;
  const float* packedT;
  const float* cst;
  int n_in, n_out, L, act, HT;
  int nG[SF_MLP_LMAX];
  int nGo[SF_MLP_LMAX];
  int width[SF_MLP_LMAX];
  int o_w[SF_MLP_LMAX], o_b[SF_MLP_LMAX], oT_w[SF_MLP_LMAX];
};
struct SfMlpLayout {
  SfMlpDev dev;
  int64_t n_params = 0, n_packed = 0, n_packedT = 0;
  std::vector<int32_t> src1, src2, srcT1, srcT2, gdst;
  std::vector<float> cst;
  std::string error;
};
bool sf_build_mlp_layout(const sf_mlp_desc& d, SfMlpLayout& L);
```

synference_amd/csrc/sf_maf16.hip:

```cpp
#include "sf_maf16_pass.h"

template <int NB, bool SPAN>
__global__ __launch_bounds__(256, 3) void k_maf_inv16(SfDev m, SfSampleArgsHost a) {
  const int lane = threadIdx.x & 63, wave = threadIdx.x >> 6;
  const int s = lane & 15, g4 = lane >> 4;
  const long item = ((long)blockIdx.x * 4 + wave) * 16 + s;
  const bool valid = item < a.n_items;
  const long it = valid ? item : a.n_items - 1;
  const SfItem16 I = sf_item16(m, a, it, g4);
  f32x4 u = I.u;
  const uint32_t slot = I.slot, att_mine = I.att;
  const long gal = I.gal, ps_idx = I.ps;
  const float* xr = a.x + gal * m.C;
  float logdet = 0.f;

  const float* ctg = (m.ctab && !a.z_in) ? m.ctab + (size_t)gal * m.T * m.ctab_R : nullptr;
  f32x4 ct0;
  if (!ctg) ct0 = sf_ctx_tile16(m, xr, 0, g4);

  const int NT = m.nT16;
  SfPass16 S;
#pragma unroll
  for (int k = 0; k < 3; ++k)
#pragma unroll
    for (int ot = 0; ot < 4; ++ot)
#pragma unroll
      for (int r = 0; r < 4; ++r) S.act[k][ot][r] = 0.f;
  SfTiles16 tiles;
  tiles.pack(m);
  for (int t = m.T - 1; t >= 0; --t) {
    __syncthreads();
    {
      const float4* __restrict__ s4 = reinterpret_cast<const float4*>(m.packed16 + (size_t)t * m.t16_stride);
      float4* __restrict__ d4 = reinterpret_cast<float4*>(sf_lds16);
      const int n4 = m.t16_stride >> 2;
      const int lane_ = threadIdx.x & 63;
      const int ngroups = n4 >> 8;
      for (int gi = __builtin_amdgcn_readfirstlane(wave); gi < ngroups; gi += 4) sf_copy_group16(s4 + gi * 256 + lane_, d4 + gi * 256);
      __builtin_amdgcn_s_waitcnt(0x0f70);
    }
    __syncthreads();
    const float* tp = sf_lds16;
    if (ctg) {
#pragma unroll
      for (int ot = 0; ot < 4; ++ot)
        if (ot < NT) S.c0[ot] = *reinterpret_cast<const f32x4*>(ctg + (size_t)t * m.ctab_R + ot * 16 + 4 * g4);
    } else {
#pragma unroll
      for (int ot = 0; ot < 4; ++ot)
        if (ot < NT) {
          S.c0[ot] = sf_ld4(tp + m.o16_b0 + (ot * 4 + g4) * 4);
          S.c0[ot] = sf_mma16(sf_w16(tp + m.o16_wc, m.nC16, ot, 0, lane), ct0, S.c0[ot]);
        }
      for (int ic = 1; ic < m.nC16; ++ic) {
        const f32x4 ct = sf_ctx_tile16(m, xr, ic, g4);
#pragma unroll
        for (int ot = 0; ot < 4; ++ot)
          if (ot < NT) S.c0[ot] = sf_mma16(sf_w16(tp + m.o16_wc, m.nC16, ot, ic, lane), ct, S.c0[ot]);
      }
    }
#pragma unroll
    for (int r = 0; r < 4; ++r) S.ut[r] = 0.f;
    S.ldl = 0.f;
    const int dsl = (int)m.cst[m.c_dslot + t * SF_DMAX + s];
    {
      const int sl = __builtin_amdgcn_readlane(dsl, 0);
      S.ldl += sf_log(sf_pass16_deg1(m, tp, S.ut, sl, sf_slot16(u, sl, lane), g4));
    }
    for (int p = 2; p <= m.D; ++p) {
      const int sl = __builtin_amdgcn_readlane(dsl, p - 1);
      sf_pass16_tiles<SfHid16Plain, NB, SPAN, false>(m, tp, nullptr, S, NT, tiles, p, m.D, sl, sf_slot16(u, sl, lane), lane, g4);
    }
    logdet -= S.ldl;
    u = S.ut;
  }

  float th[4];
  bool ok = true;
#pragma unroll
  for (int r = 0; r < 4; ++r) {
    const int p = 4 * g4 + r;
    th[r] = 0.f;
    if (p < m.D) {
      const int td = (int)m.cst[m.c_tdim + p];
      th[r] = sf_div(u[r] - m.cst[m.c_pshift + p], m.cst[m.c_pscale + p]);
      ok = ok && (fabsf(th[r]) <= 3.0e38f);
      if (a.lo) ok = ok && (th[r] >= a.lo[td]) && (th[r] <= a.hi[td]);
    }
  }
  if (a.att_list && att_mine == 0xffffffffu) ok = false;
  const uint32_t acc16 = sf_accept16(ok, valid);
  const bool accepted = (acc16 >> s) & 1u;
  if (a.z_in) {
    if (valid) {
#pragma unroll
      for (int r = 0; r < 4; ++r)
        if (4 * g4 + r < m.D) a.out[item * m.D + (int)m.cst[m.c_tdim + 4 * g4 + r]] = th[r];
      if (a.logdet_out && g4 == 0) a.logdet_out[item] = logdet - m.logdet0;
    }
  } else if (a.best) {
    if (accepted && g4 == 0) atomicMin(&a.best[ps_idx], att_mine);
  } else if (a.count) {
    const long g_first = __shfl(gal, 0, 64);
    const long g_last = __shfl(gal, 15, 64);
    if (g_first == g_last) {
      if (lane == 0 && acc16) atomicAdd(&a.count[g_first], (int)__popc(acc16));
    } else if (accepted && g4 == 0) {
      atomicAdd(&a.count[gal], 1);
    }
  } else {
    const int A = a.attempts_per_slot;
    const int grp0 = (s / A) * A;
    const uint32_t gmask = (acc16 >> grp0) & ((1u << A) - 1u);
    const int first = gmask ? (int)__builtin_ctz(gmask) : -1;
    const int me = s - grp0;
    if (valid) {
      if (g4 == 0 && me == 0 && a.n_drawn && a.attempt > 0) sf_sat_add(&a.n_drawn[gal], first >= 0 ? first + 1 : A);
      if (me == first) {
#pragma unroll
        for (int r = 0; r < 4; ++r)
          if (4 * g4 + r < m.D) sf_out_store(a, (size_t)slot * m.D + (int)m.cst[m.c_tdim + 4 * g4 + r], th[r]);
      } else if (first < 0 && me == 0 && g4 == 0) {
        const uint32_t pos = atomicAdd(a.n_rejected, 1u);
        a.rejected[pos] = (uint32_t)slot;
      }
    }
  }
}

struct SfSamp16Args {
  SfDev m;
  SfSampleArgsHost a;
};

#define SF_SAMP16_TPW 2
template <int NB, int DD>
struct SfFix16 {
  static constexpr int NT = DD - 1;
  static constexpr int o_w0 = 0, o_b0 = NT * 256, o_bk0 = o_b0 + NT * 16, o_bk1 = o_bk0 + NT * 16;
  static constexpr int o_hv = o_b0 + NT * 16 * (1 + NB), o_hvb = o_hv + DD * 128;
  static constexpr int o_wh = (o_hvb + 2 * DD + 3) / 4 * 4, o_bh = o_wh + NT * 256;
  static constexpr int o_wp = (o_bh + 16 + 3) / 4 * 4;
  static constexpr int a_tab = (o_wp + NT * 256 + 1023) / 1024 * 1024;
  static constexpr int entries = NT == 4 ? 6 : (NT == 3 ? 4 : 2);
  static constexpr int oB_wk1 = entries * 512, B_stride = (NB * entries * 512 + 1023) / 1024 * 1024;
  static bool matches(const SfDev& m) {
    return m.nT16 == NT && m.o16_w0 == o_w0 && m.o16_b0 == o_b0 && m.o16_bk[0] == o_bk0 && (NB < 2 || m.o16_bk[1] == o_bk1) &&
           m.o16_hv == o_hv && m.o16_hvb == o_hvb && m.o16_wh == o_wh && m.o16_bh == o_bh && m.o16_wp == o_wp && m.t16_a_tab == a_tab &&
           m.o16B_wk[0] == 0 && (NB < 2 || m.o16B_wk[1] == oB_wk1) && m.t16B_stride == B_stride;
  }
  static __device__ __forceinline__ void apply(SfDev& m) {
    m.nT16 = NT; m.o16_w0 = o_w0; m.o16_b0 = o_b0; m.o16_bk[0] = o_bk0; m.o16_bk[1] = o_bk1; m.o16_hv = o_hv; m.o16_hvb = o_hvb;
    m.o16_wh = o_wh; m.o16_bh = o_bh; m.o16_wp = o_wp; m.t16_a_tab = a_tab; m.o16B_wk[0] = 0; m.o16B_wk[1] = oB_wk1; m.t16B_stride = B_stride;
  }
};

#ifndef SF_SAMP16_WG_FUSED
#define SF_SAMP16_WG_FUSED 4
#endif
template <int NB, bool SPAN, bool HM, int DD = 0, int PREC = 0>
__global__ __launch_bounds__(256, (SPAN ? 3 : (PREC == 2 ? SF_SAMP16_WG_FUSED : 4))) void k_maf_samp16(SfSamp16Args args_in) {
  static_assert(DD == 0 || (HM && !SPAN && DD >= 2 && DD <= 5), "unrolled passes: head tile, aligned placement, D <= 5");
  using HID = SfHid16<PREC>;
  constexpr int TPW = SF_SAMP16_TPW;
  constexpr int IPW = 64 * TPW;
  const int wave = threadIdx.x >> 6;
  unsigned int* ctrl = reinterpret_cast<unsigned int*>(
      sf_lds16 + (args_in.m.ctab ? args_in.m.t16_a_tab : args_in.m.t16_a) + HID::lds_floats(args_in.m, !SPAN));
  unsigned int pf;
  sf_q_begin<IPW>(args_in.a, ctrl, pf);
  float* ecb = reinterpret_cast<float*>(ctrl + SF_Q_WORDS(IPW));
  sf_ecb16_build<true>(ecb, args_in.m, args_in.a);
#ifdef SF_Q_STATS
  const unsigned long long qs_k0 = __builtin_amdgcn_s_memtime();
  unsigned long long qs_iters = 0, qs_last_work = 0;
  unsigned long long qs_ph[10] = {0, 0, 0, 0, 0, 0, 0, 0, 0, 0};
  if (threadIdx.x == 0) atomicMin(&args_in.a.q->stats[10], __builtin_amdgcn_s_memrealtime());
#endif
  for (;;) {
    const SfSamp16Args* ap;
    {
      auto kp = __builtin_amdgcn_kernarg_segment_ptr();
      asm volatile("" : "+s"(kp));
      ap = (const SfSamp16Args*)kp;
    }
    const SfDev& m_arg = ap->m;
    SfDev m_fix;
    if constexpr (DD > 0) { m_fix = m_arg; SfFix16<NB, DD>::apply(m_fix); }
    const SfDev& m = DD > 0 ? m_fix : m_arg;
    const SfSampleArgsHost& a = ap->a;
    const int lane = (threadIdx.x & 63) + sf_opaque_zero();
    const int s = lane & 15, g4 = lane >> 4;
#ifdef SF_Q_STATS
    const unsigned long long qs_t_top = __builtin_amdgcn_s_memrealtime();
#endif
    if (!sf_q_fetch<IPW, 64>(a, ctrl, pf)) {
#ifdef SF_Q_STATS
      if (threadIdx.x == 0) {
        for (int i = 0; i < 10; ++i) atomicAdd(&a.q->stats[14 + i], qs_ph[i]);
        atomicAdd(&a.q->stats[9], __builtin_amdgcn_s_memtime() - qs_k0);
        atomicMax(&a.q->stats[11], qs_iters);
        atomicMax(&a.q->stats[12], qs_last_work);
        atomicMax(&a.q->stats[13], __builtin_amdgcn_s_memrealtime());
      }
#endif
      break;
    }
#ifdef SF_Q_STATS
    if (a.qtrace && threadIdx.x == 0 && qs_iters < (2048u * 256u) / gridDim.x) {
      uint32_t* tr = a.qtrace + ((size_t)blockIdx.x * ((2048u * 256u) / gridDim.x) + qs_iters) * 4;
      tr[0] = (uint32_t)__builtin_amdgcn_s_memrealtime(); tr[1] = ctrl[0]; tr[2] = ctrl[1] | (ctrl[9] << 8);
    }
    ++qs_iters;
    const unsigned long long qs_t_fetch = __builtin_amdgcn_s_memrealtime();
    const int qs_o = ctrl[9] ? 5 : 0;
    qs_ph[qs_o + 0] += qs_t_fetch - qs_t_top;
    unsigned long long qs_t_mark = qs_t_fetch;
#endif
    const int NT = m.nT16;
    const unsigned int n_items = ctrl[0] << ctrl[1];
    f32x4 u_t[TPW];
    unsigned int g_t[TPW];
    f32x4& u_cur = u_t[0];
    unsigned int& gal_cur = g_t[0];
#pragma unroll
    for (int j = TPW - 1; j >= 0; --j) {
      const int wi = (j * 4 + wave) * 16 + s;
      const unsigned int n_ent = ctrl[0];
      const int lgA = (int)ctrl[1];
      const unsigned int e = (unsigned)wi >> lgA;
      const unsigned int ee = e < n_ent ? e : 0u;
      const uint32_t slot = ctrl[SF_Q_HDR + ee];
      const uint32_t att = ctrl[SF_Q_HDR + IPW + ee] + ((unsigned)wi & ((1u << lgA) - 1u));
      float z4[4];
      sf_normal4(a.k0, a.k1, (uint64_t)slot + a.rng_slot_offset, att, (uint32_t)g4, z4);
#pragma unroll
      for (int r = 0; r < 4; ++r) u_t[j][r] = (4 * g4 + r < m.D) ? z4[r] : 0.f;
      g_t[j] = slot / (uint32_t)a.S;
    }
    SfTiles16 tiles;
    if constexpr (DD == 0) tiles.pack(m);
    typename HID::State S;
    S.tab = DD > 0 ? true : m.ctab != nullptr;
    for (int t = m.T - 1; t >= 0; --t) {
      const int dsl = (int)m.cst[m.c_dslot + t * SF_DMAX + s];
      S.c0p = S.tab ? m.ctab + ((size_t)gal_cur * m.T + t) * m.ctab_R + (PREC == 2 ? m.nT16 * 16 : 0) : nullptr;
      if constexpr (PREC == 2) sf_pre16g_load<DD - 1>(S, g4);
      else if (HM && S.tab) sf_c0_prefetch(S, tiles.tile(2), g4);
#ifdef SF_Q_STATS
      { const unsigned long long n = __builtin_amdgcn_s_memrealtime(); qs_ph[qs_o + (t == m.T - 1 ? 1 : 3)] += n - qs_t_mark; qs_t_mark = n; }
#endif
      __syncthreads();
      sf_stage16<PREC, !SPAN>(m, t, S.tab ? m.t16_a_tab : m.t16_a, wave);
      __syncthreads();
#ifdef SF_Q_STATS
      { const unsigned long long n = __builtin_amdgcn_s_memrealtime(); qs_ph[qs_o + 2] += n - qs_t_mark; qs_t_mark = n; }
#endif
      const float* tp = sf_lds16;
      const void* tpB = sf_lds16 + (S.tab ? m.t16_a_tab : m.t16_a);
#pragma unroll 1
      for (int j = 0; j < TPW; ++j) {
        const bool tile_has_work = (unsigned)((j * 4 + wave) * 16) < n_items;
        if (tile_has_work) {
          if (j > 0) {
            S.c0p = S.tab ? m.ctab + ((size_t)gal_cur * m.T + t) * m.ctab_R + (PREC == 2 ? m.nT16 * 16 : 0) : nullptr;
            if constexpr (PREC == 2) sf_pre16g_load<DD - 1>(S, g4);
            else if (HM && S.tab) sf_c0_prefetch(S, tiles.tile(2), g4);
          }
          if (HM) S.hdone = sf_ld4(tp + m.o16_bh + g4 * 4);
          if constexpr (PREC == 2) {
            float* scr = (float*)tpB + HID::blk_floats(m) + wave * SF_G16_SCR + s * SF_G16_ROW;
            sf_transform16g<NB, DD>(m, tp, static_cast<const float*>(tpB), S, dsl, u_cur, scr, lane, g4);
          } else {
            S.xr = a.x + gal_cur * m.C;
            if constexpr (DD > 0) {
              sf_transform16s<HID, NB, DD>(m, tp, tpB, S, NT, dsl, u_cur, lane, g4);
            } else {
              HID::template clear<false, HM>(S);
#pragma unroll
              for (int r = 0; r < 4; ++r) S.ut[r] = 0.f;
              {
                const int sl = __builtin_amdgcn_readlane(dsl, 0);
                sf_pass16_deg1(m, tp, S.ut, sl, sf_slot16_own(u_cur, sl), g4);
              }
              for (int p = 2; p <= m.D; ++p) {
                const int sl = __builtin_amdgcn_readlane(dsl, p - 1);
                sf_pass16_tiles<HID, NB, SPAN, HM>(m, tp, tpB, S, NT, tiles, p, m.D, sl, sf_slot16_own(u_cur, sl), lane, g4);
              }
              u_cur = S.ut;
            }
          }
        }
        if (TPW > 1) {
          const f32x4 tu = u_t[0];
          const unsigned int tg = g_t[0];
#pragma unroll
          for (int q = 0; q + 1 < TPW; ++q) { u_t[q] = u_t[q + 1]; g_t[q] = g_t[q + 1]; }
          u_t[TPW - 1] = tu;
          g_t[TPW - 1] = tg;
        }
      }
    }
#ifdef SF_Q_STATS
    { const unsigned long long n = __builtin_amdgcn_s_memrealtime(); qs_ph[qs_o + 3] += n - qs_t_mark; qs_t_mark = n; }
#endif
#pragma unroll 1
    for (int j = 0; j < TPW; ++j) {
      const int wi = (j * 4 + wave) * 16 + s;
      const unsigned int n_ent = ctrl[0];
      const int lgA = (int)ctrl[1];
      const unsigned int e = (unsigned)wi >> lgA;
      const bool entry_ok = e < n_ent;
      const unsigned int ee = entry_ok ? e : 0u;
      const uint32_t slot = ctrl[SF_Q_HDR + ee];
      const uint32_t att_base = ctrl[SF_Q_HDR + IPW + ee];
      const uint32_t att = att_base + ((unsigned)wi & ((1u << lgA) - 1u));
      const bool valid = entry_ok && att < a.attempt_limit;
      float th[4];
      int tdc[4];
      const uint32_t acc16 = sf_accept16(sf_theta_box16(ecb, u_cur, g4, th, tdc), valid);
      const int A = 1 << lgA;
      int first, me;
      if (lgA <= 4) {
        const int grp0 = (s / A) * A;
        const uint32_t gmask = (acc16 >> grp0) & ((1u << A) - 1u);
        first = gmask ? (int)__builtin_ctz(gmask) : -1;
        me = s - grp0;
      } else {
        if ((threadIdx.x & 63) == 0) ctrl[20 + wave] = acc16 ? (unsigned)__builtin_ctz(acc16) : 16u;
        __syncthreads();
        const int gw0 = (int)(((e << lgA) >> 4) & 3u), gwn = A >> 4;
        first = -1;
#pragma unroll
        for (int w = 3; w >= 0; --w) {
          const unsigned int cw = ctrl[20 + w];
          if (w >= gw0 && w < gw0 + gwn && cw < 16u) first = (w - gw0) * 16 + (int)cw;
        }
        me = wi - (int)(e << lgA);
        if (TPW > 1) __syncthreads();
      }
      if (lgA == 0) {
        const int Dn = DD > 0 ? DD : m.D;
        const int* c2s = reinterpret_cast<const int*>(ecb) + 80;
        for (int e0 = 0; e0 < 16 * Dn; e0 += 64) {
          const int e = e0 + (lane & 63);
          const int se = (e / Dn) & 15, c = e - (e / Dn) * Dn;
          const int p = c2s[c];
          const int src = se + 16 * (p >> 2), rr = p & 3;
          const float v0 = __shfl(th[0], src, 64), v1 = __shfl(th[1], src, 64), v2 = __shfl(th[2], src, 64), v3 = __shfl(th[3], src, 64);
          const float v = rr == 0 ? v0 : (rr == 1 ? v1 : (rr == 2 ? v2 : v3));
          const uint32_t sl_e = (uint32_t)__shfl((int)slot, se, 64);
          if (e < 16 * Dn && ((acc16 >> se) & 1u)) sf_out_store(a, (size_t)sl_e * Dn + c, v);
        }
      } else if (valid && me == first) {
#pragma unroll
        for (int r = 0; r < 4; ++r)
          if (4 * g4 + r < m.D) sf_out_store(a, (size_t)slot * m.D + tdc[r], th[r]);
      }
      const bool leader = entry_ok && g4 == 0 && me == 0;
      const uint32_t room = a.attempt_limit > att_base ? a.attempt_limit - att_base : 0u;
      const uint32_t tried = room < (uint32_t)A ? room : (uint32_t)A;
      const bool hit = leader && first >= 0;
      const bool retry = leader && first < 0 && att_base + (uint32_t)A < a.attempt_limit;
      const bool surv = leader && first < 0 && !retry;
      if (leader && (a.n_drawn || a.gal_acc)) {
        const long gal = (long)(slot / (uint32_t)a.S);
        const int used = (first >= 0 ? first + 1 : (int)tried) - (att_base == 0u ? 1 : 0);
        if (a.n_drawn && used > 0) sf_sat_add(&a.n_drawn[gal], used);
        if (hit && a.gal_acc && att_base >= 64u) atomicAdd(&a.gal_acc[gal], 1);
      }
      if (retry) {
        const unsigned int pos = atomicAdd(&ctrl[2], 1u);
        ctrl[SF_Q_HDR + 2 * IPW + pos] = slot;
        ctrl[SF_Q_HDR + 3 * IPW + pos] = att_base + (uint32_t)A;
      }
      if (surv) {
        const unsigned int pos = atomicAdd(&ctrl[3], 1u);
        ctrl[SF_Q_HDR + 4 * IPW + pos] = slot;
      }
      const unsigned int n_res = (unsigned)__popcll(__ballot(hit || surv));
      const unsigned int n_ev = (unsigned)__popcll(__ballot(valid && g4 == 0));
      const unsigned int n_r0 = (unsigned)__popcll(__ballot(leader && first < 0 && att_base == 0u));
      if ((threadIdx.x & 63) == 0) {
        if (n_res) atomicAdd(&ctrl[4], n_res);
        if (n_ev) atomicAdd(&ctrl[5], n_ev);
        if (n_r0) atomicAdd(&ctrl[6], n_r0);
      }
      if (TPW > 1) {
        const f32x4 tu = u_t[0];
#pragma unroll
        for (int q = 0; q + 1 < TPW; ++q) u_t[q] = u_t[q + 1];
        u_t[TPW - 1] = tu;
      }
    }
#ifdef SF_Q_STATS
    qs_last_work = __builtin_amdgcn_s_memrealtime();
    qs_ph[qs_o + 4] += qs_last_work - qs_t_mark;
    if (a.qtrace && threadIdx.x == 0 && qs_iters <= (2048u * 256u) / gridDim.x)
      a.qtrace[((size_t)blockIdx.x * ((2048u * 256u) / gridDim.x) + qs_iters - 1) * 4 + 3] = (uint32_t)qs_last_work;
#endif
  }
}

template <int NB, int DD, int PREC = 0>
__global__ __launch_bounds__(256, 4) void k_maf_find16s(SfDev m, SfSampleArgsHost a) {
  using HID = SfHid16<PREC>;
  SfFix16<NB, DD>::apply(m);
  const int lane = threadIdx.x & 63, wave = threadIdx.x >> 6;
  const int s = lane & 15, g4 = lane >> 4;
  float* ecb = sf_lds16 + m.t16_a_tab + HID::lds_floats(m, true);
  sf_ecb16_build<false>(ecb, m, a);
  const int NT = m.nT16;
  f32x4 u_cur, u_oth;
  long gal_cur = 0, gal_oth = 0;
#pragma unroll
  for (int j = 1; j >= 0; --j) {
    const long item = ((long)blockIdx.x * 8 + j * 4 + wave) * 16 + s;
    const long it = item < a.n_items ? item : a.n_items - 1;
    const SfItem16 I = sf_item16(m, a, it, g4);
    if (j == 1) { u_oth = I.u; gal_oth = I.gal; }
    else { u_cur = I.u; gal_cur = I.gal; }
  }
  typename HID::State S;
  S.tab = true;
  if constexpr (PREC != 2) S.xr = nullptr;
  for (int t = m.T - 1; t >= 0; --t) {
    const int dsl = (int)m.cst[m.c_dslot + t * SF_DMAX + s];
    S.c0p = m.ctab + ((size_t)gal_cur * m.T + t) * m.ctab_R + (PREC == 2 ? m.nT16 * 16 : 0);
    if constexpr (PREC == 2) sf_pre16g_load<DD - 1>(S, g4);
    else sf_c0_prefetch(S, 0, g4);
    __syncthreads();
    sf_stage16<PREC, true>(m, t, m.t16_a_tab, wave);
    __syncthreads();
    const float* tp = sf_lds16;
    const void* tpB = sf_lds16 + m.t16_a_tab;
#pragma unroll 1
    for (int j = 0; j < 2; ++j) {
      if (((long)blockIdx.x * 8 + j * 4 + wave) * 16 < a.n_items) {
        if (j > 0) {
          S.c0p = m.ctab + ((size_t)gal_cur * m.T + t) * m.ctab_R + (PREC == 2 ? m.nT16 * 16 : 0);
          if constexpr (PREC == 2) sf_pre16g_load<DD - 1>(S, g4);
          else sf_c0_prefetch(S, 0, g4);
        }
        S.hdone = sf_ld4(tp + m.o16_bh + g4 * 4);
        if constexpr (PREC == 2) {
          float* scr = (float*)tpB + HID::blk_floats(m) + wave * SF_G16_SCR + s * SF_G16_ROW;
          sf_transform16g<NB, DD>(m, tp, static_cast<const float*>(tpB), S, dsl, u_cur, scr, lane, g4);
        } else {
          sf_transform16s<HID, NB, DD>(m, tp, tpB, S, NT, dsl, u_cur, lane, g4);
        }
      }
      { const f32x4 tu = u_cur; u_cur = u_oth; u_oth = tu; }
      { const long tg = gal_cur; gal_cur = gal_oth; gal_oth = tg; }
    }
  }
#pragma unroll 1
  for (int j = 0; j < 2; ++j) {
    const long item = ((long)blockIdx.x * 8 + j * 4 + wave) * 16 + s;
    const bool valid = item < a.n_items;
    const long it = valid ? item : a.n_items - 1;
    const long ps = it >> a.log2_attempts;
    const uint32_t att = a.att_list ? a.att_list[ps] : a.attempt + (uint32_t)(it & ((1L << a.log2_attempts) - 1));
    float th[4];
    int tdc[4];
    bool ok = sf_theta_box16(ecb, u_cur, g4, th, tdc);
    if (a.att_list && att == 0xffffffffu) ok = false;
    const uint32_t acc16 = sf_accept16(ok, valid);
    const bool accepted = (acc16 >> s) & 1u;
    if (a.z_in) {
      if (valid) {
#pragma unroll
        for (int r = 0; r < 4; ++r)
          if (4 * g4 + r < m.D) a.out[item * m.D + tdc[r]] = th[r];
      }
    } else if (a.best) {
      if (accepted && g4 == 0) atomicMin(&a.best[ps], att);
    } else if (a.count) {
      const long gal = (long)((uint32_t)(a.slots ? a.slots[ps] : (uint32_t)(a.slot_base + ps)) / (uint32_t)a.S);
      const long g_first = __shfl(gal, 0, 64), g_last = __shfl(gal, 15, 64);
      if (g_first == g_last) {
        if (lane == 0 && acc16) atomicAdd(&a.count[g_first], (int)__popc(acc16));
      } else if (accepted && g4 == 0) {
        atomicAdd(&a.count[gal], 1);
      }
    } else if (valid) {
      const uint32_t slot = a.slots ? a.slots[ps] : (uint32_t)(a.slot_base + ps);
      if (accepted) {
#pragma unroll
        for (int r = 0; r < 4; ++r)
          if (4 * g4 + r < m.D) sf_out_store(a, (size_t)slot * m.D + tdc[r], th[r]);
      } else if (g4 == 0) {
        const uint32_t pos = atomicAdd(a.n_rejected, 1u);
        a.rejected[pos] = slot;
      }
    }
    { const f32x4 tu = u_cur; u_cur = u_oth; u_oth = tu; }
  }
}

template <typename K>
static hipError_t sf_lds_optin16(K kernel, SfAttrCache& attr) {
  int dev;
  if (!attr.need(dev)) return hipSuccess;
  hipError_t e = hipFuncSetAttribute((const void*)kernel, hipFuncAttributeMaxDynamicSharedMemorySize, 160 * 1024);
  if (e == hipSuccess) attr.set(dev);
  return e;
}
template <typename F>
static hipError_t sf_visit_shape16(int NB, bool span, bool hm, F&& f) {
  auto nb = [&](auto sp, auto h) {
    return NB == 1 ? f(std::integral_constant<int, 1>{}, sp, h) : f(std::integral_constant<int, 2>{}, sp, h);
  };
  if (span) return nb(std::true_type{}, std::false_type{});
  if (hm) return nb(std::false_type{}, std::true_type{});
  return nb(std::false_type{}, std::false_type{});
}
template <typename F>
static hipError_t sf_visit_unrolled16(int NB, int dd, F&& f) {
  auto d = [&](auto nb) {
    switch (dd) {
      case 3: return f(nb, std::integral_constant<int, 3>{});
      case 4: return f(nb, std::integral_constant<int, 4>{});
      case 5: return f(nb, std::integral_constant<int, 5>{});
      default: return (hipError_t)hipErrorInvalidValue;
    }
  };
  if (NB == 1) return d(std::integral_constant<int, 1>{});
  if (NB == 2) return d(std::integral_constant<int, 2>{});
  return hipErrorInvalidValue;
}

static int sf_maf16_seq_d(const SfDev& m) {
  if (!m.ctab || m.m16_span || m.D < 3 || m.D > 5 || m.nT16 != m.D - 1) return 0;
  for (int p = 2; p <= m.D; ++p)
    if (m.g16_tile[p - 1] != p - 2) return 0;
  bool fits = false;
  if (m.NB == 1) fits = m.D == 3 ? SfFix16<1, 3>::matches(m) : (m.D == 4 ? SfFix16<1, 4>::matches(m) : SfFix16<1, 5>::matches(m));
  else if (m.NB == 2) fits = m.D == 3 ? SfFix16<2, 3>::matches(m) : (m.D == 4 ? SfFix16<2, 4>::matches(m) : SfFix16<2, 5>::matches(m));
  return fits ? m.D : 0;
}
SfMaf16Plan sf_maf16_plan(const SfDev& m) {
  SfMaf16Plan pl;
  pl.fp32 = sf_sampler_fp32_for(SF_MAF) != 0;
  pl.ok16 = m.kind == SF_MAF && m.m16_ok && !m.hidden_bf16 && m.packed16 != nullptr;
  pl.sampler16 = pl.ok16 && (m.packed16B != nullptr || pl.fp32);
  pl.span = m.m16_span != 0;
  pl.head_mfma = !m.m16_span && m.o16_wh >= 0;
  pl.dd = pl.head_mfma ? sf_maf16_seq_d(m) : 0;
  pl.fused = pl.dd > 0 && pl.fp32 && m.o16_wp >= 0 && m.ctab_R == 2 * m.nT16 * 16;
  return pl;
}

template <int NB, int DD, int PREC>
static hipError_t sf_launch_find16s(const SfDev& m, const SfSampleArgsHost& a, hipStream_t st) {
  static SfAttrCache attr;
  const size_t sh = ((size_t)m.t16_a_tab + (size_t)SfHid16<PREC>::lds_floats(m, true)) * sizeof(float) + 80 * sizeof(float);
  if (hipError_t e = sf_lds_optin16(k_maf_find16s<NB, DD, PREC>, attr); e != hipSuccess) return e;
  hipLaunchKernelGGL((k_maf_find16s<NB, DD, PREC>), dim3((unsigned)((a.n_items + 127) / 128)), dim3(256), sh, st, m, a);
  return hipGetLastError();
}

template <int NB, bool SPAN, bool HM, int PREC = 0>
__global__ __launch_bounds__(256, 3) void k_maf_inv16b(SfDev m, const float* __restrict__ z, const float* __restrict__ x,
                                                       long n, float* __restrict__ out) {
  using HID = SfHid16<PREC>;
  const int lane = threadIdx.x & 63, wave = threadIdx.x >> 6;
  const int s = lane & 15, g4 = lane >> 4;
  const long item = ((long)blockIdx.x * 4 + wave) * 16 + s;
  const bool valid = item < n;
  const long it = valid ? item : n - 1;
  f32x4 u;
#pragma unroll
  for (int r = 0; r < 4; ++r) u[r] = (4 * g4 + r < m.D) ? z[it * m.D + 4 * g4 + r] : 0.f;
  const int NT = m.nT16;
  SfTiles16 tiles;
  tiles.pack(m);
  typename HID::State S;
  HID::template clear<false, false>(S);
  for (int t = m.T - 1; t >= 0; --t) {
    __syncthreads();
    sf_stage16<PREC, !SPAN>(m, t, m.t16_a, wave);
    __syncthreads();
    const float* tp = sf_lds16;
    const void* tpB = sf_lds16 + m.t16_a;
    S.c0p = nullptr;
    S.tab = false;
    S.xr = x + it * m.C;
    if (HM) S.hdone = sf_ld4(tp + m.o16_bh + g4 * 4);
#pragma unroll
    for (int r = 0; r < 4; ++r) S.ut[r] = 0.f;
    const int dsl = (int)m.cst[m.c_dslot + t * SF_DMAX + s];
    {
      const int sl = __builtin_amdgcn_readlane(dsl, 0);
      sf_pass16_deg1(m, tp, S.ut, sl, sf_slot16(u, sl, lane), g4);
    }
    for (int p = 2; p <= m.D; ++p) {
      const int sl = __builtin_amdgcn_readlane(dsl, p - 1);
      sf_pass16_tiles<HID, NB, SPAN, HM>(m, tp, tpB, S, NT, tiles, p, m.D, sl, sf_slot16(u, sl, lane), lane, g4);
    }
    u = S.ut;
  }
  if (valid) {
#pragma unroll
    for (int r = 0; r < 4; ++r) {
      const int p = 4 * g4 + r;
      if (p < m.D) out[item * m.D + (int)m.cst[m.c_tdim + p]] = sf_div(u[r] - m.cst[m.c_pshift + p], m.cst[m.c_pscale + p]);
    }
  }
}

template <int NB, bool SPAN, bool HM, int PREC>
static hipError_t sf_launch16b_hook_p(const SfDev& m, const float* z, const float* x, long n, float* out, hipStream_t st) {
  static SfAttrCache attr;
  const size_t sh = ((size_t)m.t16_a + (size_t)SfHid16<PREC>::lds_floats(m, !SPAN)) * sizeof(float);
  if (hipError_t e = sf_lds_optin16(k_maf_inv16b<NB, SPAN, HM, PREC>, attr); e != hipSuccess) return e;
  hipLaunchKernelGGL((k_maf_inv16b<NB, SPAN, HM, PREC>), dim3((unsigned)((n + 63) / 64)), dim3(256), sh, st, m, z, x, n, out);
  return hipGetLastError();
}
hipError_t sf_launch_maf_inv16b_hook(const SfDev& m, const float* z, const float* x, long n, float* out, hipStream_t st) {
  const SfMaf16Plan pl = sf_maf16_plan(m);
  return sf_visit_shape16(m.NB, pl.span, pl.head_mfma, [&](auto nb, auto sp, auto hm) {
    return pl.fp32 ? sf_launch16b_hook_p<nb(), sp(), hm(), 1>(m, z, x, n, out, st)
                   : sf_launch16b_hook_p<nb(), sp(), hm(), 0>(m, z, x, n, out, st);
  });
}

__global__ __launch_bounds__(256) void k_maf_ctab16(SfDev m, const float* __restrict__ x, long M, float* __restrict__ tab) {
  const int lane = threadIdx.x & 63, wave = threadIdx.x >> 6;
  const int s = lane & 15, g4 = lane >> 4;
  const long gal = ((long)blockIdx.x * 4 + wave) * 16 + s;
  if (((long)blockIdx.x * 4 + wave) * 16 >= M) return;
  const bool valid = gal < M;
  const float* xr = x + (valid ? gal : M - 1) * m.C;
  const int NT = m.nT16;
  {
    const int t = blockIdx.y;
    const float* tp = m.packed16 + (size_t)t * m.t16_stride;
    f32x4 c0[4];
#pragma unroll
    for (int ot = 0; ot < 4; ++ot)
      if (ot < NT) c0[ot] = sf_ld4(tp + m.o16_b0 + (ot * 4 + g4) * 4);
    for (int ic = 0; ic < m.nC16; ++ic) {
      const f32x4 ct = sf_ctx_tile16(m, xr, ic, g4);
#pragma unroll
      for (int ot = 0; ot < 4; ++ot)
        if (ot < NT) c0[ot] = sf_mma16(sf_w16(tp + m.o16_wc, m.nC16, ot, ic, lane), ct, c0[ot]);
    }
    if (valid) {
#pragma unroll
      for (int ot = 0; ot < 4; ++ot)
        if (ot < NT)
          *reinterpret_cast<f32x4*>(tab + ((size_t)gal * m.T + t) * m.ctab_R + ot * 16 + 4 * g4) = c0[ot];
    }
    if (m.o16_wp >= 0) {
      f32x4 c1[4];
#pragma unroll
      for (int ot = 0; ot < 4; ++ot)
        if (ot < NT) {
          c1[ot] = sf_ld4(tp + m.o16_bk[0] + (ot * 4 + g4) * 4);
#pragma unroll
          for (int it = 0; it < 4; ++it)
            if (it < NT) c1[ot] = sf_mma16(sf_w16(tp + m.o16_wk[0], NT, ot, it, lane), c0[it], c1[ot]);
        }
      if (valid) {
#pragma unroll
        for (int ot = 0; ot < 4; ++ot)
          if (ot < NT)
            *reinterpret_cast<f32x4*>(tab + ((size_t)gal * m.T + t) * m.ctab_R + NT * 16 + ot * 16 + 4 * g4) = c1[ot];
      }
    }
  }
}
__global__ __launch_bounds__(256) void k_maf_fuse16(SfDev m) {
  const int t = blockIdx.x;
  const int NT = m.nT16;
  const int KN = NT < m.D - 1 ? NT : m.D - 1;
  const int n_ent = KN * NT - KN * (KN - 1) / 2;
  float* tp = const_cast<float*>(m.packed16) + (size_t)t * m.t16_stride;
  for (int i = threadIdx.x; i < n_ent * 16; i += blockDim.x) {
    const int e = i >> 4, g4 = (i >> 2) & 3, r = i & 3;
    int k = 1;
    while (k < KN && e >= sf_wp16_entry(NT, k + 1, k)) ++k;
    const int ot = k - 1 + (e - sf_wp16_entry(NT, k, k - 1));
    const int row = 4 * g4 + r;
    const int col = (int)m.cst[m.c_dslot + t * SF_DMAX + k - 1];
    double acc = 0.0;
    for (int it = 0; it < NT; ++it)
      for (int kk = 0; kk < 16; ++kk) {
        const float wk = tp[m.o16_wk[0] + ((ot * NT + it) * 64 + row + 16 * (kk >> 2)) * 4 + (kk & 3)];
        const float w0 = tp[m.o16_w0 + (it * 64 + kk + 16 * (col >> 2)) * 4 + (col & 3)];
        acc += (double)wk * (double)w0;
      }
    tp[m.o16_wp + e * 16 + g4 * 4 + r] = (float)acc;
  }
}
hipError_t sf_launch_maf_fuse16(const SfDev& m, hipStream_t st) {
  hipLaunchKernelGGL(k_maf_fuse16, dim3((unsigned)m.T), dim3(256), 0, st, m);
  return hipGetLastError();
}
hipError_t sf_launch_maf_ctab16(const SfDev& m, const float* x, long M, float* tab, hipStream_t st) {
  hipLaunchKernelGGL(k_maf_ctab16, dim3((unsigned)((M + 63) / 64), (unsigned)m.T), dim3(256), 0, st, m, x, M, tab);
  return hipGetLastError();
}

bool sf_maf16_enabled(const SfDev& m, const SfSampleArgsHost& a) {
  return sf_maf16_plan(m).ok16 && (a.attempts_per_slot <= 16 || a.best != nullptr);
}

static int sf_resident_blocks16(const void* fn, size_t sh, int cap) {
  int dev = 0, cus = 256, per = cap;
  if (hipGetDevice(&dev) == hipSuccess) {
    hipDeviceProp_t pr;
    if (hipGetDeviceProperties(&pr, dev) == hipSuccess && pr.multiProcessorCount > 0) cus = pr.multiProcessorCount;
  }
  int occ = 0;
  if (hipOccupancyMaxActiveBlocksPerMultiprocessor(&occ, fn, 256, sh) == hipSuccess && occ > 0) per = occ < cap ? occ : cap;
  return cus * per;
}

template <int NB, bool SPAN, bool HM, int DD, int PREC>
static hipError_t sf_launch16q_p(const SfDev& m, const SfSampleArgsHost& a, hipStream_t st) {
  static SfAttrCache attr;
  static SfResidentCache rcache;
  const size_t sh = ((size_t)(m.ctab ? m.t16_a_tab : m.t16_a) + (size_t)SfHid16<PREC>::lds_floats(m, !SPAN)) * sizeof(float) +
                    (SF_Q_WORDS(64 * SF_SAMP16_TPW) + 96) * sizeof(unsigned int);
  if (sh > 160 * 1024) return hipErrorInvalidValue;
  if (hipError_t e = sf_lds_optin16(k_maf_samp16<NB, SPAN, HM, DD, PREC>, attr); e != hipSuccess) return e;
  int resident = 0, cur_dev = 0;
  (void)hipGetDevice(&cur_dev);
  if (!rcache.get(cur_dev, sh, resident)) {
    resident = sf_resident_blocks16((const void*)k_maf_samp16<NB, SPAN, HM, DD, PREC>, sh, SPAN ? 3 : (PREC == 2 ? SF_SAMP16_WG_FUSED : 4));
    rcache.put(cur_dev, sh, resident);
  }
  long grid = (a.n_items + 64 * SF_SAMP16_TPW - 1) / (64 * SF_SAMP16_TPW);
  if (grid > resident) grid = resident;
  SfSamp16Args args;
  args.m = m;
  args.a = a;
  hipLaunchKernelGGL((k_maf_samp16<NB, SPAN, HM, DD, PREC>), dim3((unsigned)grid), dim3(256), sh, st, args);
  return hipGetLastError();
}
template <int NB, bool SPAN, bool HM, int DD>
static hipError_t sf_launch16q(const SfDev& m, const SfSampleArgsHost& a, const SfMaf16Plan& pl, hipStream_t st) {
  if constexpr (DD > 0) {
    if (pl.fused) return sf_launch16q_p<NB, SPAN, HM, DD, 2>(m, a, st);
  }
  if (pl.fp32) return sf_launch16q_p<NB, SPAN, HM, DD, 1>(m, a, st);
  if (!m.packed16B) return hipErrorInvalidValue;
  return sf_launch16q_p<NB, SPAN, HM, DD, 0>(m, a, st);
}
template <int NB, bool SPAN>
static hipError_t sf_launch16(const SfDev& m, const SfSampleArgsHost& a, hipStream_t st) {
  static SfAttrCache attr;
  const size_t sh = (size_t)m.t16_stride * sizeof(float);
  if (hipError_t e = sf_lds_optin16(k_maf_inv16<NB, SPAN>, attr); e != hipSuccess) return e;
  const long per_block = 4L * 16;
  hipLaunchKernelGGL((k_maf_inv16<NB, SPAN>), dim3((unsigned)((a.n_items + per_block - 1) / per_block)), dim3(256), sh, st, m, a);
  return hipGetLastError();
}
static hipError_t sf_launch_find16(const SfDev& m, const SfSampleArgsHost& a, const SfMaf16Plan& pl, hipStream_t st) {
  return sf_visit_unrolled16(m.NB, pl.dd, [&](auto nb, auto dd) {
    return pl.fused ? sf_launch_find16s<nb(), dd(), 2>(m, a, st)
                    : (pl.fp32 ? sf_launch_find16s<nb(), dd(), 1>(m, a, st) : sf_launch_find16s<nb(), dd(), 0>(m, a, st));
  });
}
hipError_t sf_launch_maf_find16_zin(const SfDev& m, const SfSampleArgsHost& a, hipStream_t st) {
  const SfMaf16Plan pl = sf_maf16_plan(m);
  return pl.fused ? sf_launch_find16(m, a, pl, st) : hipErrorInvalidValue;
}
hipError_t sf_launch_maf_inv16(const SfDev& m, const SfSampleArgsHost& a, hipStream_t st) {
  const SfMaf16Plan pl = sf_maf16_plan(m);
  if (a.q) {
    if (pl.dd > 0)
      return sf_visit_unrolled16(m.NB, pl.dd, [&](auto nb, auto dd) { return sf_launch16q<nb(), false, true, dd()>(m, a, pl, st); });
    return sf_visit_shape16(m.NB, pl.span, pl.head_mfma,
                            [&](auto nb, auto sp, auto hm) { return sf_launch16q<nb(), sp(), hm(), 0>(m, a, pl, st); });
  }
  if ((a.best || a.att_list || a.count) && !a.z_in && pl.dd > 0 && (pl.fp32 || m.packed16B)) return sf_launch_find16(m, a, pl, st);
  return sf_visit_shape16(m.NB, pl.span, false, [&](auto nb, auto sp, auto) { return sf_launch16<nb(), sp()>(m, a, st); });
}
```

synference_amd/csrc/sf_maf16_pass.h:

```cpp
#pragma once
#include <hip/hip_runtime.h>

#include <type_traits>

#include "sf_device.h"
#include "sf_internal.h"
#include "sf_rng.h"

typedef float f32x4 __attribute__((ext_vector_type(4)));
typedef float f32x2 __attribute__((ext_vector_type(2)));
#define SF_MFMA16(a, b, c) __builtin_amdgcn_mfma_f32_16x16x4f32((a), (b), (c), 0, 0, 0)

__device__ __forceinline__ float sf_sum4groups(float v) {
  v += __shfl_xor(v, 16, 64);
  v += __shfl_xor(v, 32, 64);
  return v;
}
__device__ __forceinline__ f32x4 sf_mma16(float4 w, const f32x4& in, f32x4 acc) {
  acc = SF_MFMA16(w.x, in[0], acc);
  acc = SF_MFMA16(w.y, in[1], acc);
  acc = SF_MFMA16(w.z, in[2], acc);
  acc = SF_MFMA16(w.w, in[3], acc);
  return acc;
}
// ... 471 lines not shown
                                              int lane, int g4) {
    sf_pass16b_span<LO, HI, NB>(m, tp, static_cast<const unsigned int*>(tpH), S, NT, sl, u_sl, lane, g4);
  }
  template <bool SEQ, bool HM>
  static __device__ __forceinline__ void clear(State& S) {
#pragma unroll
    for (int k = 0; k < 2; ++k)
#pragma unroll
      for (int pr = 0; pr < 2; ++pr)
#pragma unroll
        for (int c = SEQ ? 2 : 0; c < 4; ++c) { S.ph[k][pr][c] = 0u; S.pl[k][pr][c] = 0u; }
    if (!HM) {
#pragma unroll
      for (int ot = 0; ot < 4; ++ot)
#pragma unroll
        for (int r = 0; r < 4; ++r) S.head[ot][r] = 0.f;
    }
  }
  static __host__ __device__ int lds_floats(const SfDev& m, bool ) { return m.t16B_stride; }
};
template <> struct SfHid16<1> {
  using State = SfPass16F;
  template <int OT, int NB, bool CP, bool HM>
  static __device__ __forceinline__ void pass(const SfDev& m, const float* tp, const void* tpH, State& S, int NT, int sl, float u_sl,
                                              int lane, int g4, int next_ot) {
    sf_pass16f<OT, NB, CP, HM>(m, tp, static_cast<const float*>(tpH), S, NT, sl, u_sl, lane, g4, next_ot);
  }
  template <int LO, int HI, int NB>
  static __device__ __forceinline__ void span(const SfDev& m, const float* tp, const void* tpH, State& S, int NT, int sl, float u_sl,
                                              int lane, int g4) {
    sf_pass16f_span<LO, HI, NB>(m, tp, static_cast<const float*>(tpH), S, NT, sl, u_sl, lane, g4);
  }
  template <bool SEQ, bool HM>
  static __device__ __forceinline__ void clear(State& S) {
    if (!SEQ) {
#pragma unroll
      for (int k = 0; k < 2; ++k)
#pragma unroll
        for (int ot = 0; ot < 4; ++ot)
#pragma unroll
          for (int r = 0; r < 4; ++r) S.act[k][ot][r] = 0.f;
    }
    if (!HM) {
#pragma unroll
      for (int ot = 0; ot < 4; ++ot)
#pragma unroll
        for (int r = 0; r < 4; ++r) S.head[ot][r] = 0.f;
    }
  }
  static __host__ __device__ int lds_floats(const SfDev& m, bool cp) {
    const int nb = m.NB < 2 ? m.NB : 2;
    return nb * (cp ? m.nT16 * (m.nT16 + 1) / 2 : m.nT16 * m.nT16) * 256;
  }
};

struct SfPass16G {
  f32x4 act[4];
  f32x4 pre[4];
  f32x4 hdone;
  const float* c0p;
  bool tab;
};
__host__ __device__ constexpr int sf_wp16_entry(int NT, int k, int ot) { return (k - 1) * NT - (k - 1) * (k - 2) / 2 + ot - (k - 1); }
#define SF_G16_ROW 20
#define SF_G16_SCR (16 * SF_G16_ROW)
template <int NT>
__device__ __forceinline__ void sf_pre16g_load(SfPass16G& S, int g4) {
#pragma unroll
  for (int ot = 0; ot < NT; ++ot) S.pre[ot] = *reinterpret_cast<const f32x4*>(S.c0p + ot * 16 + 4 * g4);
}
__device__ __forceinline__ f32x4 sf_rank1(const f32x4& acc, const float4& w, float v) {
  const f32x2 vv = {v, v};
  const f32x2 lo = __builtin_elementwise_fma(f32x2{w.x, w.y}, vv, f32x2{acc[0], acc[1]});
  const f32x2 hi = __builtin_elementwise_fma(f32x2{w.z, w.w}, vv, f32x2{acc[2], acc[3]});
  return f32x4{lo[0], lo[1], hi[0], hi[1]};
}
template <int NT, int K>
struct SfWpCols {
  float4 w[NT - K + 1];
  __device__ __forceinline__ void load(const float* tp, int o_wp, int g4) {
#pragma unroll
    for (int q = 0; q <= NT - K; ++q) w[q] = *reinterpret_cast<const float4*>(tp + o_wp + sf_wp16_entry(NT, K, K - 1 + q) * 16 + 4 * g4);
  }
  __device__ __forceinline__ void apply(SfPass16G& S, float wv) const {
#pragma unroll
    for (int q = 0; q <= NT - K; ++q) S.pre[K - 1 + q] = sf_rank1(S.pre[K - 1 + q], w[q], wv);
  }
};
template <int OT, int NB, int NT>
__device__ __forceinline__ float sf_pass16g(const SfDev& m, const float* tp, const float* tpF, SfPass16G& S, int sl, float u_in,
                                            int lane, int g4) {
  const float4 wh = sf_w16(tp + m.o16_wh, NT, 0, OT, lane);
  float4 fw[OT + 1];
  f32x4 b1;
  if (NB == 2) {
    b1 = sf_ld4(tp + m.o16_bk[1] + (OT * 4 + g4) * 4);
#pragma unroll
    for (int it = 0; it <= OT; ++it) fw[it] = sf_w16f<true>(tpF, NT, OT, it, lane);
  }
  SfWpCols<NT, (OT + 2 <= NT ? OT + 2 : NT)> wu;
  if constexpr (OT + 2 <= NT) wu.load(tp, m.o16_wp, g4);
  __builtin_amdgcn_sched_barrier(0);
  if (NB == 2) {
#pragma unroll
    for (int it = 0; it < OT; ++it) b1 = sf_mma16(fw[it], S.act[it], b1);
  }
  f32x4 last = sf_tanh4(S.pre[OT]);
  if (NB == 2) {
    S.act[OT] = last;
    b1 = sf_mma16(fw[OT], last, b1);
    last = sf_tanh4(b1);
  }
  S.hdone = sf_mma16(wh, last, S.hdone);
  const bool odd = (sl & 1) != 0;
  const int src = (lane & 15) + 16 * (sl >> 1);
  const float av = __shfl(odd ? S.hdone[2] : S.hdone[0], src, 64);
  const float mv = __shfl(odd ? S.hdone[3] : S.hdone[1], src, 64);
  const float wv = sf_div(u_in - mv, sf_scale16(m, av));
  if constexpr (OT + 2 <= NT) wu.apply(S, wv);
  return wv;
}
template <int NB, int DD>
__device__ __forceinline__ void sf_transform16g(const SfDev& m, const float* tp, const float* tpF, SfPass16G& S, int dsl, f32x4& u,
                                                float* scr, int lane, int g4) {
  constexpr int NT = DD - 1;
  *reinterpret_cast<f32x4*>(scr + 4 * g4) = u;
  int sl[DD];
  float ud[DD];
#pragma unroll
  for (int q = 0; q < DD; ++q) {
    sl[q] = __builtin_amdgcn_readlane(dsl, q);
    ud[q] = scr[sl[q]];
  }
  {
    SfWpCols<NT, 1> wu;
    wu.load(tp, m.o16_wp, g4);
    const float av = tp[m.o16_hvb + 2 * sl[0]], mv = tp[m.o16_hvb + 2 * sl[0] + 1];
    const float wv = sf_div(ud[0] - mv, sf_scale16(m, av));
    wu.apply(S, wv);
    scr[sl[0]] = wv;
  }
  auto pass = [&](auto otc) {
    constexpr int OT = decltype(otc)::value;
    scr[sl[OT + 1]] = sf_pass16g<OT, NB, NT>(m, tp, tpF, S, sl[OT + 1], ud[OT + 1], lane, g4);
  };
  pass(std::integral_constant<int, 0>{});
  if constexpr (DD >= 3) pass(std::integral_constant<int, 1>{});
  if constexpr (DD >= 4) pass(std::integral_constant<int, 2>{});
  if constexpr (DD >= 5) pass(std::integral_constant<int, 3>{});
  u = *reinterpret_cast<const f32x4*>(scr + 4 * g4);
}
template <> struct SfHid16<2> {
  using State = SfPass16G;
  static __host__ __device__ int blk_floats(const SfDev& m) { return m.NB >= 2 ? m.nT16 * (m.nT16 + 1) / 2 * 256 : 0; }
  static __host__ __device__ int lds_floats(const SfDev& m, bool ) { return blk_floats(m) + 4 * SF_G16_SCR; }
};

__device__ __forceinline__ void sf_copy_group16(const float4* g, float4* l) {
  __builtin_amdgcn_global_load_lds((const void*)g, (void __attribute__((address_space(3)))*)l, 16, 0, 0);
  __builtin_amdgcn_global_load_lds((const void*)g, (void __attribute__((address_space(3)))*)l, 16, 1024, 0);
  __builtin_amdgcn_global_load_lds((const void*)g, (void __attribute__((address_space(3)))*)l, 16, 2048, 0);
  __builtin_amdgcn_global_load_lds((const void*)g, (void __attribute__((address_space(3)))*)l, 16, 3072, 0);
}

template <int PREC, bool CP>
__device__ __forceinline__ void sf_stage16(const SfDev& m, int t, int a_floats, int wave) {
  const int lane_ = threadIdx.x & 63;
  const int ga = a_floats >> 10;
  const float4* __restrict__ sa = reinterpret_cast<const float4*>(m.packed16 + (size_t)t * m.t16_stride);
  float4* __restrict__ d4 = reinterpret_cast<float4*>(sf_lds16);
  if constexpr (PREC == 0) {
    const int gb = m.t16B_stride >> 10;
    const float4* __restrict__ sb = reinterpret_cast<const float4*>(m.packed16B + (size_t)t * m.t16B_stride);
    for (int gi = __builtin_amdgcn_readfirstlane(wave); gi < ga + gb; gi += 4) {
      sf_copy_group16((gi < ga ? sa + gi * 256 : sb + (gi - ga) * 256) + lane_, d4 + gi * 256);
    }
  } else {
    for (int gi = __builtin_amdgcn_readfirstlane(wave); gi < ga; gi += 4) {
      sf_copy_group16(sa + gi * 256 + lane_, d4 + gi * 256);
    }
    const int NT = m.nT16, nb = m.NB < 2 ? m.NB : 2;
    const int per = CP ? NT * (NT + 1) / 2 : NT * NT;
    constexpr int K0 = PREC == 2 ? 1 : 0;
    float4* __restrict__ dF = d4 + (a_floats >> 2);
    for (int e = __builtin_amdgcn_readfirstlane(wave); e < (nb - K0) * per; e += 4) {
      const int k = K0 + (e >= per ? 1 : 0), ee = e - (k - K0) * per;
      int src_blk = ee;
      if (CP) {
        const int ot = ee >= 6 ? 3 : (ee >= 3 ? 2 : (ee >= 1 ? 1 : 0));
        src_blk = ot * NT + (ee - ot * (ot + 1) / 2);
      }
      const int owk = k ? m.o16_wk[1] : m.o16_wk[0];
      const float4* g = sa + ((owk >> 2) + src_blk * 64) + lane_;
      __builtin_amdgcn_global_load_lds((const void*)g, (void __attribute__((address_space(3)))*)(dF + e * 64), 16, 0, 0);
    }
  }
  __builtin_amdgcn_s_waitcnt(0x0f70);
}

struct SfHid16Plain {
  using State = SfPass16;
  template <int OT, int NB, bool CP, bool HM>
  static __device__ __forceinline__ void pass(const SfDev& m, const float* tp, const void*, State& S, int NT, int sl, float u_sl,
                                              int lane, int g4, int) {
    sf_pass16<OT, NB>(m, tp, S, NT, sl, u_sl, lane, g4);
  }
  template <int LO, int HI, int NB>
  static __device__ __forceinline__ void span(const SfDev& m, const float* tp, const void*, State& S, int NT, int sl, float u_sl,
                                              int lane, int g4) {
    sf_pass16_span<LO, HI, NB>(m, tp, S, NT, sl, u_sl, lane, g4);
  }
};

struct SfTiles16 {
  uint32_t hi = 0, lo = 0;
  __device__ __forceinline__ void pack(const SfDev& m) {
#pragma unroll
    for (int q = 0; q < SF_DMAX; ++q) {
      hi |= (uint32_t)(m.g16_tile[q] & 3) << (2 * q);
      lo |= (uint32_t)(m.g16_lo[q] & 3) << (2 * q);
    }
  }
  __device__ __forceinline__ int tile(int p) const { return (int)((hi >> (2 * (p - 1))) & 3u); }
};
template <typename HID, int NB, bool SPAN, bool HM>
__device__ __forceinline__ void sf_pass16_tiles(const SfDev& m, const float* tp, const void* tpH, typename HID::State& S, int NT,
                                                const SfTiles16& tb, int p, int D, int sl, float u_sl, int lane, int g4) {
  const uint32_t hi_t = (tb.hi >> (2 * (p - 1))) & 3u;
  const uint32_t lo_t = SPAN ? (tb.lo >> (2 * (p - 1))) & 3u : hi_t;
  const int nx = p < D ? (int)((tb.hi >> (2 * p)) & 3u) : -1;
  switch (lo_t * 4 + hi_t) {
    case 0: HID::template pass<0, NB, !SPAN, HM>(m, tp, tpH, S, NT, sl, u_sl, lane, g4, nx); break;
    case 5: HID::template pass<1, NB, !SPAN, HM>(m, tp, tpH, S, NT, sl, u_sl, lane, g4, nx); break;
    case 10: HID::template pass<2, NB, !SPAN, HM>(m, tp, tpH, S, NT, sl, u_sl, lane, g4, nx); break;
    case 15: HID::template pass<3, NB, !SPAN, HM>(m, tp, tpH, S, NT, sl, u_sl, lane, g4, nx); break;
    case 1: if constexpr (SPAN) HID::template span<0, 1, NB>(m, tp, tpH, S, NT, sl, u_sl, lane, g4); break;
    case 2: if constexpr (SPAN) HID::template span<0, 2, NB>(m, tp, tpH, S, NT, sl, u_sl, lane, g4); break;
    case 3: if constexpr (SPAN) HID::template span<0, 3, NB>(m, tp, tpH, S, NT, sl, u_sl, lane, g4); break;
    case 6: if constexpr (SPAN) HID::template span<1, 2, NB>(m, tp, tpH, S, NT, sl, u_sl, lane, g4); break;
    case 7: if constexpr (SPAN) HID::template span<1, 3, NB>(m, tp, tpH, S, NT, sl, u_sl, lane, g4); break;
    default: if constexpr (SPAN) HID::template span<2, 3, NB>(m, tp, tpH, S, NT, sl, u_sl, lane, g4); break;
  }
}

template <typename HID, int NB, int DD>
__device__ __forceinline__ void sf_transform16s(const SfDev& m, const float* tp, const void* tpH, typename HID::State& S, int NT,
                                                int dsl, f32x4& u, int lane, int g4) {
  HID::template clear<true, true>(S);
#pragma unroll
  for (int r = 0; r < 4; ++r) S.ut[r] = 0.f;
  {
    const int sl = __builtin_amdgcn_readlane(dsl, 0);
    sf_pass16_deg1(m, tp, S.ut, sl, sf_slot16_own(u, sl), g4);
  }
  auto seq_pass = [&](auto otc) {
    constexpr int OT = decltype(otc)::value;
    const int sl = __builtin_amdgcn_readlane(dsl, OT + 1);
    HID::template pass<OT, NB, true, true>(m, tp, tpH, S, NT, sl, sf_slot16_own(u, sl), lane, g4, OT + 2 < DD ? OT + 1 : -1);
  };
  seq_pass(std::integral_constant<int, 0>{});
  if constexpr (DD >= 3) seq_pass(std::integral_constant<int, 1>{});
  if constexpr (DD >= 4) seq_pass(std::integral_constant<int, 2>{});
  if constexpr (DD >= 5) seq_pass(std::integral_constant<int, 3>{});
  u = S.ut;
}

struct SfItem16 {
  f32x4 u;
  long gal, ps;
  uint32_t slot, att;
};
__device__ __forceinline__ SfItem16 sf_item16(const SfDev& m, const SfSampleArgsHost& a, long it, int g4) {
  SfItem16 I;
  I.ps = it >> a.log2_attempts;
  I.slot = a.z_in ? (uint32_t)it : (a.slots ? a.slots[I.ps] : (uint32_t)(a.slot_base + I.ps));
  I.att = a.att_list ? a.att_list[I.ps] : a.attempt + (uint32_t)(it & ((1L << a.log2_attempts) - 1));
  I.gal = a.z_in ? it : (long)(I.slot / (uint32_t)a.S);
  float z4[4];
  if (a.z_in) {
#pragma unroll
    for (int r = 0; r < 4; ++r) z4[r] = (4 * g4 + r < m.D) ? a.z_in[it * m.D + 4 * g4 + r] : 0.f;
  } else {
    sf_normal4(a.k0, a.k1, (uint64_t)I.slot + a.rng_slot_offset, I.att, (uint32_t)g4, z4);
  }
#pragma unroll
  for (int r = 0; r < 4; ++r) I.u[r] = (4 * g4 + r < m.D) ? z4[r] : 0.f;
  return I;
}

template <bool C2S>
__device__ __forceinline__ void sf_ecb16_build(float* ecb, const SfDev& m, const SfSampleArgsHost& a) {
  if (threadIdx.x < 16) {
    const int p = threadIdx.x;
    const bool on = p < m.D;
    const int td = on ? (int)m.cst[m.c_tdim + p] : 0;
    ecb[p * 5 + 0] = on ? m.cst[m.c_pshift + p] : 0.f;
    ecb[p * 5 + 1] = on ? __builtin_amdgcn_rcpf(m.cst[m.c_pscale + p]) : 0.f;
    ecb[p * 5 + 2] = (on && a.lo) ? a.lo[td] : -3.4e38f;
    ecb[p * 5 + 3] = (on && a.lo) ? a.hi[td] : 3.4e38f;
    reinterpret_cast<int*>(ecb)[p * 5 + 4] = td;
    if (C2S && on) reinterpret_cast<int*>(ecb)[80 + td] = p;
  }
}
__device__ __forceinline__ uint32_t sf_accept16(bool ok, bool valid) {
  const unsigned long long okb = __ballot(ok);
  return (uint32_t)(okb & (okb >> 16) & (okb >> 32) & (okb >> 48) & 0xffffull) & (uint32_t)(__ballot(valid) & 0xffffull);
}
__device__ __forceinline__ bool sf_theta_box16(const float* ecb, const f32x4& u, int g4, float (&th)[4], int (&tdc)[4]) {
  bool ok = true;
#pragma unroll
  for (int r = 0; r < 4; ++r) {
    const float* e = ecb + (4 * g4 + r) * 5;
    th[r] = (u[r] - e[0]) * e[1];
    tdc[r] = reinterpret_cast<const int*>(e)[4];
    ok = ok && (fabsf(th[r]) <= 3.0e38f) && (th[r] >= e[2]) && (th[r] <= e[3]);
  }
  return ok;
}
```

synference_amd/engine.py:

```python
from __future__ import annotations

import ctypes as C
import json
from typing import Optional, Tuple

import numpy as np
import torch

from . import _lib
from .spec import KIND_ID, FlowSpec, num_params


def retry_width(pending: int, attempt: int, max_attempts: int, total: int = 0) -> int:
    A = 1
    if attempt > 0:
        budget = 262144
        while A < 16 and 2 * A * pending <= budget and attempt + 2 * A <= max_attempts:
            A *= 2
    return A


def _ptr(t: Optional[torch.Tensor]):
    return None if t is None else C.c_void_p(t.data_ptr())


def _stream(device) -> C.c_void_p:
    return C.c_void_p(torch.cuda.current_stream(device).cuda_stream)


def _f32c(t, device) -> torch.Tensor:
    t = torch.as_tensor(t)
    return t.to(device=device, dtype=torch.float32).contiguous()


def spec_supports_log_prob_grad(spec) -> bool:
    return spec.kind == "maf" or (spec.kind == "nsf" and spec.D >= 2)


class HipFlow:

    def __init__(self, spec: FlowSpec, device="cuda:0"):
        self.spec = spec
        self.lib = _lib.load()
        self.device = torch.device(device)
        self._keep = (spec.theta_mean, spec.theta_std, spec.x_mean, spec.x_std, spec.perms)
        d = _lib.sf_flow_desc(
            kind=KIND_ID[spec.kind], D=spec.D, C=spec.C, H=spec.H, T=spec.T, K=spec.K, NB=spec.NB,
            scale_fn=0 if spec.scale_fn == "softplus" else 1, hidden_bf16=1 if spec.hidden_bf16 else 0,
            tail_bound=spec.tail_bound, min_bin_width=spec.min_bin_width, min_bin_height=spec.min_bin_height,
            min_derivative=spec.min_derivative, maf_eps=spec.maf_eps, lu_eps=spec.lu_eps,
            theta_mean=spec.theta_mean.ctypes.data_as(_lib.c_f32p),
            theta_std=spec.theta_std.ctypes.data_as(_lib.c_f32p),
            x_mean=spec.x_mean.ctypes.data_as(_lib.c_f32p),
            x_std=spec.x_std.ctypes.data_as(_lib.c_f32p),
            perms=spec.perms.ctypes.data_as(_lib.c_i32p) if spec.kind == "maf" else None, ar_slope=spec.ar_slope)
        h = C.c_void_p()
        _lib.check(self.lib.sf_flow_create(C.byref(d), C.byref(h)))
        self.handle = h
        self.n_params = int(self.lib.sf_flow_num_params(h))
        assert self.n_params == num_params(spec), (self.n_params, num_params(spec))

    def __del__(self):
        h = getattr(self, "handle", None)
        if h is not None and h.value:
            self.lib.sf_flow_destroy(h)
            self.handle = None

    def packed_size(self) -> int:
        return int(self.lib.sf_flow_packed_size(self.handle))

    def pack_table(self) -> Tuple[np.ndarray, np.ndarray]:
        n = self.packed_size()
        s1 = np.empty(n, np.int32)
        s2 = np.empty(n, np.int32)
        _lib.check(self.lib.sf_flow_pack_table(self.handle, s1.ctypes.data_as(_lib.c_i32p),
                                               s2.ctypes.data_as(_lib.c_i32p), n))
        return s1, s2

    def pack_table16(self) -> Tuple[np.ndarray, np.ndarray]:
        n = int(self.lib.sf_flow_packed16_size(self.handle))
        s1 = np.empty(n, np.int32)
        s2 = np.empty(n, np.int32)
        if n:
            _lib.check(self.lib.sf_flow_pack_table16(self.handle, s1.ctypes.data_as(_lib.c_i32p),
                                                     s2.ctypes.data_as(_lib.c_i32p), n))
        return s1, s2

    def pack_table16b(self) -> np.ndarray:
        n = int(self.lib.sf_flow_packed16b_size(self.handle))
        s = np.empty(n, np.int32)
        if n:
            _lib.check(self.lib.sf_flow_pack_table16b(self.handle, s.ctypes.data_as(_lib.c_i32p), n))
        return s

    TRC_FIELDS = ("ok NT NI t_stride g_stride o_win o_b0 o_w1 o_b1 o_w2 o_b2 o_wf o_bf o_wfT o_w2T o_w1T o_winT "
                  "g_win g_b0 g_w1 g_b1 g_w2 g_b2 g_wf g_bf kend0 kend1 kend2 kend3 kbeg0 kbeg1 kbeg2 kbeg3 c_insrc c_jobs "
                  "n_jobs").split()

    NSC_FIELDS = ("ok NT NI OTQ KM kc_h kc_in0 kc_in1 kc_in2 t_stride g_stride o_win o_bin o_wg0 o_wg1 o_bg0 o_bg1 o_w10 o_w11 "
                  "o_b10 o_b11 o_w20 o_w21 o_b20 o_b21 o_wout o_bout o_lu o_woutT o_w2T0 o_w2T1 o_w1T0 o_w1T1 o_winT "
                  "g_win g_bin g_wg0 g_wg1 g_bg0 g_bg1 g_w10 g_w11 g_b10 g_b11 g_w20 g_w21 g_b20 g_b21 g_wout g_bout g_lu").split()

    def trainc_table(self):
        n = int(self.lib.sf_flow_trainc_size(self.handle))
        if not n:
            return None
        s1 = np.empty(n, np.int32)
        s2 = np.empty(n, np.int32)
        gd = np.empty(self.n_params, np.int32)
        desc = np.zeros(64, np.int32)
        ncst = int(self.lib.sf_flow_cst_size(self.handle))
        cst = np.empty(ncst, np.float32)
        _lib.check(self.lib.sf_flow_trainc_table(self.handle, s1.ctypes.data, s2.ctypes.data, n, gd.ctypes.data, self.n_params,
                                                 desc.ctypes.data, cst.ctypes.data, ncst))
        d = {k: int(v) for k, v in zip(self.TRC_FIELDS if self.spec.kind == "maf" else self.NSC_FIELDS, desc)}
        d["n_grad"] = int(self.lib.sf_flow_trainc_grad_size(self.handle))
        return s1, s2, gd, d, cst

    def describe(self) -> dict:
        d = getattr(self, "_describe", None)
        if d is None:
            buf = C.create_string_buffer(1 << 16)
            _lib.check(self.lib.sf_flow_describe(self.handle, buf, len(buf)))
            d = self._describe = json.loads(buf.value.decode())
        return dict(d)

    def _dev(self):
        if not torch.cuda.is_available():
            raise RuntimeError("synference_amd: no GPU visible; the HIP flow engine has no CPU fallback")
        torch.cuda.set_device(self.device)

    def set_params(self, flat: torch.Tensor) -> None:
        self._dev()
        flat = _f32c(flat, self.device)
        _lib.check(self.lib.sf_flow_set_params(self.handle, _ptr(flat), flat.numel(), 1, _stream(self.device)))

    def get_params(self) -> torch.Tensor:
        self._dev()
        out = torch.empty(num_params(self.spec), dtype=torch.float32, device=self.device)
        _lib.check(self.lib.sf_flow_get_params(self.handle, _ptr(out), out.numel(), 1, _stream(self.device)))
        return out

    def log_prob(self, theta, x) -> torch.Tensor:
        self._dev()
        theta, x = _f32c(theta, self.device), _f32c(x, self.device)
        B = theta.shape[0]
        if theta.shape != (B, self.spec.D) or x.shape != (B, self.spec.C):
            raise ValueError(f"theta {tuple(theta.shape)} / x {tuple(x.shape)} do not match "
                             f"(B,{self.spec.D}) / (B,{self.spec.C})")
        out = torch.empty(B, dtype=torch.float32, device=self.device)
        _lib.check(self.lib.sf_flow_log_prob(self.handle, _ptr(theta), _ptr(x), B, _ptr(out), _stream(self.device)))
        return out

    GRAD_KINDS = ("maf", "nsf")

    def supports_log_prob_grad(self) -> bool:
        return spec_supports_log_prob_grad(self.spec)

    def log_prob_grad(self, theta, x, rows_per_x: int = 1, want_lp: bool = True, want_grad: bool = True):
        self._dev()
        theta, x = _f32c(theta, self.device), _f32c(x, self.device)
        B, R = theta.shape[0], int(rows_per_x)
        if R < 1:
            raise ValueError("rows_per_x must be >= 1")
        if theta.dim() != 2 or theta.shape[1] != self.spec.D or x.shape != ((B + R - 1) // R, self.spec.C):
            raise ValueError(f"theta {tuple(theta.shape)} / x {tuple(x.shape)} do not match (B,{self.spec.D}) / "
                             f"(ceil(B/{R}),{self.spec.C})")
        lp = torch.empty(B, dtype=torch.float32, device=self.device) if want_lp else None
        g = torch.empty_like(theta) if want_grad else None
        _lib.check(self.lib.sf_flow_log_prob_grad(self.handle, _ptr(theta), _ptr(x), R, B, _ptr(lp), _ptr(g),
                                                  _stream(self.device)))
        return lp, g

    def inverse(self, z, x) -> Tuple[torch.Tensor, torch.Tensor]:
        self._dev()
        z, x = _f32c(z, self.device), _f32c(x, self.device)
        B = z.shape[0]
        if z.shape != (B, self.spec.D) or x.shape != (B, self.spec.C):
            raise ValueError("shape mismatch")
        th = torch.empty_like(z)
        ld = torch.empty(B, dtype=torch.float32, device=self.device)
        _lib.check(self.lib.sf_flow_inverse_from_noise(self.handle, _ptr(z), _ptr(x), B, _ptr(th), _ptr(ld),
                                                       _stream(self.device)))
        return th, ld

    def inverse_sampler(self, z, x) -> Tuple[torch.Tensor, bool]:
        self._dev()
        z, x = _f32c(z, self.device), _f32c(x, self.device)
        B = z.shape[0]
        if z.shape != (B, self.spec.D) or x.shape != (B, self.spec.C):
            raise ValueError("shape mismatch")
        th = torch.empty_like(z)
        rc = self.lib.sf_flow_inverse_from_noise_sampler(self.handle, _ptr(z), _ptr(x), B, _ptr(th), _stream(self.device))
        if rc < 0:
            _lib.check(rc)
        self.last_sampler_rc = int(rc)
        return th, rc == 0

    def set_sample_row_offset(self, row_offset: int) -> None:
        _lib.check(self.lib.sf_flow_set_sample_row_offset(self.handle, int(row_offset)))

    def train_path(self, B: int, want_dctx: bool = False) -> int:
        return int(self.lib.sf_flow_train_path(self.handle, int(B), 1 if want_dctx else 0))

    def sample(self, x, S: int, lo=None, hi=None, seed: int = 0, max_attempts: Optional[int] = None,
               out: Optional[torch.Tensor] = None, return_counts: bool = False):
        max_attempts = int(max_attempts or 0)
        self._dev()
        x = _f32c(x, self.device)
        M = x.shape[0]
        if x.dim() != 2 or x.shape[1] != self.spec.C:
            raise ValueError(f"x must be (M,{self.spec.C})")
        lo_t = None if lo is None else _f32c(lo, self.device)
        hi_t = None if hi is None else _f32c(hi, self.device)
        if out is None:
            out = torch.empty((M, S, self.spec.D), dtype=torch.float32, device=self.device)
        nd = torch.empty(M, dtype=torch.int32, device=self.device) if return_counts else None
        unfilled = C.c_int64(0)
        f64 = out.dtype == torch.float64
        if out.shape != (M, S, self.spec.D) or not out.is_contiguous() or out.dtype not in (torch.float32, torch.float64):
            raise ValueError("out must be a contiguous (M,S,D) float32 / float64 tensor")
        if out.device.type != "cuda" and not (out.device.type == "cpu" and out.is_pinned()):
            raise ValueError("out must live on the flow's device or in pinned host memory")
        if f64:
            _lib.check(self.lib.sf_flow_set_sample_output_f64(self.handle, 1))
        try:
            _lib.check(self.lib.sf_flow_sample(self.handle, _ptr(x), M, S, _ptr(lo_t), _ptr(hi_t),
                                               C.c_uint64(seed & (2 ** 64 - 1)), max_attempts, _ptr(out), _ptr(nd),
                                               C.byref(unfilled), _stream(self.device)))
        finally:
            if f64:
                self.lib.sf_flow_set_sample_output_f64(self.handle, 0)
        self.last_unfilled = int(unfilled.value)
        st4 = (C.c_float * 4)()
        _lib.check(self.lib.sf_flow_sample_stats(self.handle, st4))
        self.last_sample_stats = dict(dense_ms=st4[0], rounds=int(st4[1]), rejected_round0=int(st4[2]), evaluations=st4[3])
        return (out, nd) if return_counts else out

    def sample_slots(self, x, S: int, slots: torch.Tensor, out: torch.Tensor, lo=None, hi=None, seed: int = 0,
                     max_attempts: Optional[int] = None) -> int:
        self._dev()
        x = _f32c(x, self.device)
        if x.dim() != 2 or x.shape[1] != self.spec.C:
            raise ValueError(f"x must be (M,{self.spec.C})")
        M = x.shape[0]
        if out.shape != (M, S, self.spec.D) or out.dtype != torch.float32 or not out.is_contiguous() or out.device != self.device:
            raise ValueError("out must be a contiguous float32 (M,S,D) tensor on the flow's device")
        if slots.dtype not in (torch.int32, torch.uint32) or not slots.is_contiguous() or slots.device != self.device:
            raise ValueError("slots must be a contiguous 32-bit integer tensor on the flow's device")
        lo_t = None if lo is None else _f32c(lo, self.device)
        hi_t = None if hi is None else _f32c(hi, self.device)
        unfilled = C.c_int64(0)
        _lib.check(self.lib.sf_flow_sample_slots(self.handle, _ptr(x), M, S, _ptr(slots), slots.numel(), _ptr(lo_t), _ptr(hi_t),
                                                 C.c_uint64(seed & (2 ** 64 - 1)), int(max_attempts or 0), _ptr(out),
                                                 C.byref(unfilled), _stream(self.device)))
        self.last_unfilled = int(unfilled.value)
        return self.last_unfilled

    def supports_f64_out(self) -> bool:
        ok = self.lib.sf_flow_set_sample_output_f64(self.handle, 1) == 0
        self.lib.sf_flow_set_sample_output_f64(self.handle, 0)
        return ok

    def set_sample_time_limit(self, seconds: Optional[float]) -> None:
        _lib.check(self.lib.sf_flow_set_sample_time_limit(self.handle, C.c_double(float(seconds or 0.0))))

    def set_profiling(self, on: bool) -> None:
        _lib.check(self.lib.sf_flow_set_profiling(self.handle, 1 if on else 0))

    def train_kernel_ms(self) -> float:
        ms = C.c_float(0.0)
        _lib.check(self.lib.sf_flow_train_stats(self.handle, C.byref(ms)))
        return float(ms.value)

    def prepare_context(self, x) -> None:
        self._dev()
        _lib.check(self.lib.sf_flow_prepare_context(self.handle, _ptr(x), x.shape[0], _stream(self.device)))

# ... 64 lines not shown
```

Measured before the change: 1.087 billion.

## Stage a compact per-layer weight image for the fused MAF16 sampler

```diff
diff --git a/include/synference_hip.h b/include/synference_hip.h
--- a/include/synference_hip.h
+++ b/include/synference_hip.h
@@ -59,6 +59,8 @@
 int sf_flow_pack_table16(const sf_flow* f, int32_t* src1, int32_t* src2, int64_t n_packed16);
 int64_t sf_flow_packed16b_size(const sf_flow* f);
 int sf_flow_pack_table16b(const sf_flow* f, int32_t* src, int64_t n);
+int64_t sf_flow_packed16c_size(const sf_flow* f);
+int sf_flow_pack_table16c(const sf_flow* f, int32_t* src, int64_t n);
 int64_t sf_flow_trainc_size(const sf_flow* f);
 int64_t sf_flow_trainc_grad_size(const sf_flow* f);
 int sf_flow_trainc_table(const sf_flow* f, int32_t* src1, int32_t* src2, int64_t n, int32_t* gdst, int64_t n_params,
diff --git a/synference_amd/_lib.py b/synference_amd/_lib.py
--- a/synference_amd/_lib.py
+++ b/synference_amd/_lib.py
@@ -105,6 +105,8 @@
     "sf_flow_trainc_table": (C.c_int, [C.c_void_p, C.c_void_p, C.c_void_p, C.c_int64, C.c_void_p, C.c_int64, C.c_void_p,
                                        C.c_void_p, C.c_int64]),
     "sf_flow_pack_table16b": (C.c_int, [C.c_void_p, C.c_void_p, C.c_int64]),
+    "sf_flow_packed16c_size": (C.c_int64, [C.c_void_p]),
+    "sf_flow_pack_table16c": (C.c_int, [C.c_void_p, C.c_void_p, C.c_int64]),
     "sf_flow_get_params": (C.c_int, [C.c_void_p, C.c_void_p, C.c_int64, C.c_int, C.c_void_p]),
     "sf_flow_prepare_context": (C.c_int, [C.c_void_p, C.c_void_p, C.c_int64, C.c_void_p]),
     "sf_flow_release_context": (C.c_int, [C.c_void_p]),
diff --git a/synference_amd/csrc/sf_api.hip b/synference_amd/csrc/sf_api.hip
--- a/synference_amd/csrc/sf_api.hip
+++ b/synference_amd/csrc/sf_api.hip
@@ -51,6 +51,10 @@
     SF_TRY_SET(hipMemcpy(d.d_s16a, f->L.src16a.data(), n16 * sizeof(int32_t), hipMemcpyHostToDevice));
     SF_TRY_SET(hipMemcpy(d.d_s16b, f->L.src16b.data(), n16 * sizeof(int32_t), hipMemcpyHostToDevice));
   }
+  if (f->L.dev.m16_ok && f->L.n_packed16 > 0 && sf_maf16_compact_fix(f->L.dev) == 1) {
+    SF_TRY_SET(d.d_packed16c.alloc((size_t)f->L.dev.t16c_stride * f->L.dev.T));
+    SF_TRY_SET(d.d_s16c.upload(f->L.src16c));
+  }
   if ((f->L.dev.m16_ok || f->L.nsfS.ok) && f->L.n_packed16B > 0) {
     const size_t nB = (size_t)f->L.n_packed16B;
     SF_TRY_SET(d.d_packed16B.alloc(nB));
@@ -165,6 +169,15 @@
   if (!f || !src) return sf_fail(SF_ERR_INVALID, "null argument");
   if (!f->L.dev.m16_ok || n != f->L.n_packed16B) return sf_fail(SF_ERR_INVALID, "no split-bf16 image or size mismatch");
   std::memcpy(src, f->L.src16B.data(), (size_t)n * sizeof(int32_t));
+  return SF_OK;
+}
+
+int64_t sf_flow_packed16c_size(const sf_flow* f) { return (f && f->L.dev.m16_ok) ? (int64_t)f->L.src16c.size() : 0; }
+
+int sf_flow_pack_table16c(const sf_flow* f, int32_t* src, int64_t n) {
+  if (!f || !src) return sf_fail(SF_ERR_INVALID, "null argument");
+  if (!f->L.dev.m16_ok || n == 0 || n != (int64_t)f->L.src16c.size()) return sf_fail(SF_ERR_INVALID, "no compact fused image or size mismatch");
+  std::memcpy(src, f->L.src16c.data(), (size_t)n * sizeof(int32_t));
   return SF_OK;
 }
 
@@ -187,6 +200,7 @@
   return SF_OK;
 }
 
+static SfDev sampler_dev(const sf_flow* f, const float* x);
 int sf_flow_describe(const sf_flow* f, char* buf, size_t buflen) {
   if (!f || !buf) return sf_fail(SF_ERR_INVALID, "null argument");
   const SfDev& v = f->L.dev;
@@ -238,6 +252,9 @@
   add("o16_wk1", v.o16_wk[1]); add("o16_bk0", v.o16_bk[0]); add("o16_bk1", v.o16_bk[1]); add("o16_hv", v.o16_hv);
   add("o16_hvb", v.o16_hvb); add("o16_wh", v.o16_wh); add("o16_bh", v.o16_bh); add("o16_wp", v.o16_wp); add("t16_a_tab", v.t16_a_tab);
   add("t16_a", v.t16_a); add("t16B_stride", v.t16B_stride); add("nP16", v.nP16); add("o16B_wk0", v.o16B_wk[0]); add("o16B_wk1", v.o16B_wk[1]);
+  add("t16c_stride", v.t16c_stride); add("o16c_bk1", v.o16c_bk1); add("o16c_hvb", v.o16c_hvb); add("o16c_bh", v.o16c_bh);
+  add("o16c_wh", v.o16c_wh); add("o16c_wp", v.o16c_wp); add("o16c_blk", v.o16c_blk); add("c16_fix", sf_maf16_compact_fix(v));
+  add("sampler_fused", (f->dev_ready && f->ctab_x) ? (sf_maf16_plan(sampler_dev(f, f->ctab_x)).fused ? 1 : 0) : 0);
   add("m16_ok", v.m16_ok); add("m16_span", v.m16_span); add("nT16", v.nT16); add("nC16", v.nC16); add("t16_stride", v.t16_stride);
   s += "\"g16_tile\": [";
   for (int i = 0; i < SF_DMAX; ++i) s += std::to_string(v.g16_tile[i]) + (i + 1 < SF_DMAX ? ", " : "], ");
@@ -449,6 +466,7 @@
   m.ctab_R = R; m.ctab_NV = NV;
   if (f->wp_stale && m.kind == SF_MAF && m.m16_ok && m.packed16 && m.o16_wp >= 0) {
     SF_TRY_SET(sf_launch_maf_fuse16(m, (hipStream_t)stream));
+    if (f->d_packed16c) SF_TRY_SET(sf_launch_maf_compact16(m, f->d_s16c, f->d_packed16c, (hipStream_t)stream));
     f->wp_stale = false;
   }
   SF_TRY_SET(sf_launch_ctab(m, x, (long)M, f->d_ctab, (hipStream_t)stream));
diff --git a/synference_amd/csrc/sf_internal.h b/synference_amd/csrc/sf_internal.h
--- a/synference_amd/csrc/sf_internal.h
+++ b/synference_amd/csrc/sf_internal.h
@@ -63,6 +63,8 @@
 hipError_t sf_launch_ctab(const SfDev& m, const float* x, long M, float* tab, hipStream_t st);
 hipError_t sf_launch_maf_ctab16(const SfDev& m, const float* x, long M, float* tab, hipStream_t st);
 hipError_t sf_launch_maf_fuse16(const SfDev& m, hipStream_t st);
+hipError_t sf_launch_maf_compact16(const SfDev& m, const int32_t* tab, float* out, hipStream_t st);
+int sf_maf16_compact_fix(const SfDev& m);
 struct SfMaf16Plan {
   bool ok16 = false;
   bool sampler16 = false;
@@ -142,6 +144,8 @@
   SfBuf<int32_t> d_s1, d_s2;
   SfBuf<float> d_packed16;
   SfBuf<int32_t> d_s16a, d_s16b;
+  SfBuf<float> d_packed16c;
+  SfBuf<int32_t> d_s16c;
   SfBuf<unsigned short> d_packed16B;
   SfBuf<int32_t> d_s16B;
   SfBuf<unsigned short> d_packedB;
@@ -219,6 +223,7 @@
     v.packedB = d_packedB;
     v.packed16 = packed16_stale ? nullptr : d_packed16.get();
     v.packed16B = reinterpret_cast<const uint32_t*>(d_packed16B.get());
+    v.packed16c = (packed16_stale || wp_stale) ? nullptr : d_packed16c.get();
     v.ctab = nullptr;
     return v;
   }
diff --git a/synference_amd/csrc/sf_layout.cpp b/synference_amd/csrc/sf_layout.cpp
--- a/synference_amd/csrc/sf_layout.cpp
+++ b/synference_amd/csrc/sf_layout.cpp
@@ -996,6 +996,30 @@
   L.n_packed16B = (int64_t)L.src16B.size();
   if (!v.m16_ok && !L.nsfS.ok) { L.src16B.clear(); L.n_packed16B = 0; }
   if (v.m16_ok && (size_t)v.t16_stride * sizeof(float) > 152 * 1024) v.m16_ok = 0;
+  if (d.kind == SF_MAF && v.m16_ok && !v.m16_span && v.o16_wp >= 0 && v.o16_wh >= 0 && NB <= 2 && D >= 3 && D <= 5 && v.nT16 == D - 1) {
+    const int NT = v.nT16;
+    auto run = [&](int from, int n) { for (int i = 0; i < n; ++i) L.src16c.push_back(from + i); };
+    auto align = [&](size_t q) { while (L.src16c.size() % q) L.src16c.push_back(-1); };
+    auto here = [&]() { return (int)L.src16c.size(); };
+    v.o16c_bk1 = here();
+    if (NB == 2) run(v.o16_bk[1], NT * 16);
+    v.o16c_hvb = here();
+    run(v.o16_hvb, 2 * D);
+    align(4);
+    v.o16c_bh = here();
+    run(v.o16_bh, 16);
+    v.o16c_wh = here();
+    run(v.o16_wh, NT * 256);
+    v.o16c_wp = here();
+    const int KN = std::min(NT, D - 1);
+    run(v.o16_wp, (KN * NT - KN * (KN - 1) / 2) * 16);
+    v.o16c_blk = here();
+    if (NB == 2)
+      for (int ot = 0; ot < NT; ++ot)
+        for (int it = 0; it <= ot; ++it) run(v.o16_wk[1] + (ot * NT + it) * 256, 256);
+    align(256);
+    v.t16c_stride = here();
+  }
   L.n_packedB = (int64_t)L.srcB.size();
   {
     const int budget = 152 * 1024 / 4;
diff --git a/synference_amd/csrc/sf_layout.h b/synference_amd/csrc/sf_layout.h
--- a/synference_amd/csrc/sf_layout.h
+++ b/synference_amd/csrc/sf_layout.h
@@ -50,6 +50,9 @@
   int t16_a_tab;
   int o16_wh, o16_bh;
   int o16_wp;
+  const float* packed16c;
+  int t16c_stride;
+  int o16c_bk1, o16c_hvb, o16c_bh, o16c_wh, o16c_wp, o16c_blk;
   const uint32_t* packed16B;
   int t16B_stride, nP16, o16B_wk[2];
   int m16_span;
@@ -120,6 +123,7 @@
   std::vector<int32_t> src16B;
   int64_t n_packed16B = 0;
   int64_t n_packed16 = 0;
+  std::vector<int32_t> src16c;
   int64_t n_packedB = 0;
   std::vector<float> cst;
   std::string error;
diff --git a/synference_amd/csrc/sf_maf16.hip b/synference_amd/csrc/sf_maf16.hip
--- a/synference_amd/csrc/sf_maf16.hip
+++ b/synference_amd/csrc/sf_maf16.hip
@@ -155,18 +155,48 @@
   }
 };
 
+template <int NB, int DD>
+struct SfFixC16 {
+  static constexpr int NT = DD - 1, ENT = NT * (NT + 1) / 2;
+  static constexpr int o_bk1 = 0, o_hvb = NB == 2 ? NT * 16 : 0, o_bh = o_hvb + (2 * DD + 3) / 4 * 4, o_wh = o_bh + 16;
+  static constexpr int o_wp = o_wh + NT * 256, o_blk = o_wp + ENT * 16;
+  static constexpr int size = (o_blk + (NB == 2 ? ENT * 256 : 0) + 255) / 256 * 256;
+  static constexpr int groups = size / 256;
+  static bool matches(const SfDev& m) {
+    return m.nT16 == NT && m.o16c_bk1 == o_bk1 && m.o16c_hvb == o_hvb && m.o16c_bh == o_bh && m.o16c_wh == o_wh && m.o16c_wp == o_wp &&
+           m.o16c_blk == o_blk && m.t16c_stride == size;
+  }
+  static __device__ __forceinline__ void apply(SfDev& m) {
+    m.o16_bk[1] = o_bk1; m.o16_hvb = o_hvb; m.o16_bh = o_bh; m.o16_wh = o_wh; m.o16_wp = o_wp;
+  }
+};
+template <int PREC>
+static __host__ __device__ __forceinline__ int sf_lds_floats16(const SfDev& m, bool cp) {
+  if constexpr (PREC == 2) return m.t16c_stride + 4 * SF_G16_SCR;
+  else return (m.ctab ? m.t16_a_tab : m.t16_a) + SfHid16<PREC>::lds_floats(m, cp);
+}
+template <int G>
+__device__ __forceinline__ void sf_stage16c(const float* src, int wave) {
+  const float4* __restrict__ g = reinterpret_cast<const float4*>(src) + (threadIdx.x & 63);
+  float4* __restrict__ l = reinterpret_cast<float4*>(sf_lds16);
+  for (int gi = __builtin_amdgcn_readfirstlane(wave); gi < G; gi += 4)
+    __builtin_amdgcn_global_load_lds((const void*)(g + gi * 64), (void __attribute__((address_space(3)))*)(l + gi * 64), 16, 0, 0);
+  __builtin_amdgcn_s_waitcnt(0x0f70);
+}
+
 #ifndef SF_SAMP16_WG_FUSED
 #define SF_SAMP16_WG_FUSED 4
 #endif
 template <int NB, bool SPAN, bool HM, int DD = 0, int PREC = 0>
 __global__ __launch_bounds__(256, (SPAN ? 3 : (PREC == 2 ? SF_SAMP16_WG_FUSED : 4))) void k_maf_samp16(SfSamp16Args args_in) {
   static_assert(DD == 0 || (HM && !SPAN && DD >= 2 && DD <= 5), "unrolled passes: head tile, aligned placement, D <= 5");
+  static_assert(PREC != 2 || DD >= 3, "fused first layer: unrolled kernels only (m_fix and the compact image's offsets)");
   using HID = SfHid16<PREC>;
   constexpr int TPW = SF_SAMP16_TPW;
   constexpr int IPW = 64 * TPW;
   const int wave = threadIdx.x >> 6;
-  unsigned int* ctrl = reinterpret_cast<unsigned int*>(
-      sf_lds16 + (args_in.m.ctab ? args_in.m.t16_a_tab : args_in.m.t16_a) + HID::lds_floats(args_in.m, !SPAN));
+  using FC = SfFixC16<NB, (PREC == 2 ? DD : 2)>;
+  unsigned int* ctrl = reinterpret_cast<unsigned int*>(sf_lds16 + sf_lds_floats16<PREC>(args_in.m, !SPAN));
   unsigned int pf;
   sf_q_begin<IPW>(args_in.a, ctrl, pf);
   float* ecb = reinterpret_cast<float*>(ctrl + SF_Q_WORDS(IPW));
@@ -187,6 +217,7 @@
     const SfDev& m_arg = ap->m;
     SfDev m_fix;
     if constexpr (DD > 0) { m_fix = m_arg; SfFix16<NB, DD>::apply(m_fix); }
+    if constexpr (PREC == 2) FC::apply(m_fix);
     const SfDev& m = DD > 0 ? m_fix : m_arg;
     const SfSampleArgsHost& a = ap->a;
     const int lane = (threadIdx.x & 63) + sf_opaque_zero();
@@ -251,13 +282,14 @@
       { const unsigned long long n = __builtin_amdgcn_s_memrealtime(); qs_ph[qs_o + (t == m.T - 1 ? 1 : 3)] += n - qs_t_mark; qs_t_mark = n; }
 #endif
       __syncthreads();
-      sf_stage16<PREC, !SPAN>(m, t, S.tab ? m.t16_a_tab : m.t16_a, wave);
+      if constexpr (PREC == 2) sf_stage16c<FC::groups>(m.packed16c + (size_t)t * FC::size, wave);
+      else sf_stage16<PREC, !SPAN>(m, t, S.tab ? m.t16_a_tab : m.t16_a, wave);
       __syncthreads();
 #ifdef SF_Q_STATS
       { const unsigned long long n = __builtin_amdgcn_s_memrealtime(); qs_ph[qs_o + 2] += n - qs_t_mark; qs_t_mark = n; }
 #endif
       const float* tp = sf_lds16;
-      const void* tpB = sf_lds16 + (S.tab ? m.t16_a_tab : m.t16_a);
+      const void* tpB = sf_lds16 + (PREC == 2 ? FC::o_blk : (S.tab ? m.t16_a_tab : m.t16_a));
 #pragma unroll 1
       for (int j = 0; j < TPW; ++j) {
         const bool tile_has_work = (unsigned)((j * 4 + wave) * 16) < n_items;
@@ -269,7 +301,7 @@
           }
           if (HM) S.hdone = sf_ld4(tp + m.o16_bh + g4 * 4);
           if constexpr (PREC == 2) {
-            float* scr = (float*)tpB + HID::blk_floats(m) + wave * SF_G16_SCR + s * SF_G16_ROW;
+            float* scr = sf_lds16 + FC::size + wave * SF_G16_SCR + s * SF_G16_ROW;
             sf_transform16g<NB, DD>(m, tp, static_cast<const float*>(tpB), S, dsl, u_cur, scr, lane, g4);
           } else {
             S.xr = a.x + gal_cur * m.C;
@@ -405,11 +437,13 @@
 template <int NB, int DD, int PREC = 0>
 __global__ __launch_bounds__(256, 4) void k_maf_find16s(SfDev m, SfSampleArgsHost a) {
   using HID = SfHid16<PREC>;
+  using FC = SfFixC16<NB, DD>;
   SfFix16<NB, DD>::apply(m);
   const int lane = threadIdx.x & 63, wave = threadIdx.x >> 6;
   const int s = lane & 15, g4 = lane >> 4;
-  float* ecb = sf_lds16 + m.t16_a_tab + HID::lds_floats(m, true);
+  float* ecb = sf_lds16 + sf_lds_floats16<PREC>(m, true);
   sf_ecb16_build<false>(ecb, m, a);
+  if constexpr (PREC == 2) FC::apply(m);
   const int NT = m.nT16;
   f32x4 u_cur, u_oth;
   long gal_cur = 0, gal_oth = 0;
@@ -430,10 +464,11 @@
     if constexpr (PREC == 2) sf_pre16g_load<DD - 1>(S, g4);
     else sf_c0_prefetch(S, 0, g4);
     __syncthreads();
-    sf_stage16<PREC, true>(m, t, m.t16_a_tab, wave);
+    if constexpr (PREC == 2) sf_stage16c<FC::groups>(m.packed16c + (size_t)t * FC::size, wave);
+    else sf_stage16<PREC, true>(m, t, m.t16_a_tab, wave);
     __syncthreads();
     const float* tp = sf_lds16;
-    const void* tpB = sf_lds16 + m.t16_a_tab;
+    const void* tpB = sf_lds16 + (PREC == 2 ? FC::o_blk : m.t16_a_tab);
 #pragma unroll 1
     for (int j = 0; j < 2; ++j) {
       if (((long)blockIdx.x * 8 + j * 4 + wave) * 16 < a.n_items) {
@@ -444,7 +479,7 @@
         }
         S.hdone = sf_ld4(tp + m.o16_bh + g4 * 4);
         if constexpr (PREC == 2) {
-          float* scr = (float*)tpB + HID::blk_floats(m) + wave * SF_G16_SCR + s * SF_G16_ROW;
+          float* scr = sf_lds16 + FC::size + wave * SF_G16_SCR + s * SF_G16_ROW;
           sf_transform16g<NB, DD>(m, tp, static_cast<const float*>(tpB), S, dsl, u_cur, scr, lane, g4);
         } else {
           sf_transform16s<HID, NB, DD>(m, tp, tpB, S, NT, dsl, u_cur, lane, g4);
@@ -530,6 +565,11 @@
   return hipErrorInvalidValue;
 }
 
+int sf_maf16_compact_fix(const SfDev& m) {
+  if (m.t16c_stride <= 0 || m.D < 3 || m.D > 5 || m.nT16 != m.D - 1 || m.NB < 1 || m.NB > 2) return -1;
+  if (m.NB == 1) return m.D == 3 ? SfFixC16<1, 3>::matches(m) : (m.D == 4 ? SfFixC16<1, 4>::matches(m) : SfFixC16<1, 5>::matches(m));
+  return m.D == 3 ? SfFixC16<2, 3>::matches(m) : (m.D == 4 ? SfFixC16<2, 4>::matches(m) : SfFixC16<2, 5>::matches(m));
+}
 static int sf_maf16_seq_d(const SfDev& m) {
   if (!m.ctab || m.m16_span || m.D < 3 || m.D > 5 || m.nT16 != m.D - 1) return 0;
   for (int p = 2; p <= m.D; ++p)
@@ -547,14 +587,14 @@
   pl.span = m.m16_span != 0;
   pl.head_mfma = !m.m16_span && m.o16_wh >= 0;
   pl.dd = pl.head_mfma ? sf_maf16_seq_d(m) : 0;
-  pl.fused = pl.dd > 0 && pl.fp32 && m.o16_wp >= 0 && m.ctab_R == 2 * m.nT16 * 16;
+  pl.fused = pl.dd > 0 && pl.fp32 && m.o16_wp >= 0 && m.ctab_R == 2 * m.nT16 * 16 && m.packed16c != nullptr && sf_maf16_compact_fix(m) == 1;
   return pl;
 }
 
 template <int NB, int DD, int PREC>
 static hipError_t sf_launch_find16s(const SfDev& m, const SfSampleArgsHost& a, hipStream_t st) {
   static SfAttrCache attr;
-  const size_t sh = ((size_t)m.t16_a_tab + (size_t)SfHid16<PREC>::lds_floats(m, true)) * sizeof(float) + 80 * sizeof(float);
+  const size_t sh = (size_t)sf_lds_floats16<PREC>(m, true) * sizeof(float) + 80 * sizeof(float);
   if (hipError_t e = sf_lds_optin16(k_maf_find16s<NB, DD, PREC>, attr); e != hipSuccess) return e;
   hipLaunchKernelGGL((k_maf_find16s<NB, DD, PREC>), dim3((unsigned)((a.n_items + 127) / 128)), dim3(256), sh, st, m, a);
   return hipGetLastError();
@@ -698,6 +738,18 @@
   hipLaunchKernelGGL(k_maf_fuse16, dim3((unsigned)m.T), dim3(256), 0, st, m);
   return hipGetLastError();
 }
+__global__ __launch_bounds__(256) void k_maf_compact16(SfDev m, const int32_t* __restrict__ tab, float* __restrict__ out) {
+  const float* tp = m.packed16 + (size_t)blockIdx.x * m.t16_stride;
+  float* op = out + (size_t)blockIdx.x * m.t16c_stride;
+  for (int i = threadIdx.x; i < m.t16c_stride; i += blockDim.x) {
+    const int s = tab[i];
+    op[i] = s >= 0 ? tp[s] : 0.f;
+  }
+}
+hipError_t sf_launch_maf_compact16(const SfDev& m, const int32_t* tab, float* out, hipStream_t st) {
+  hipLaunchKernelGGL(k_maf_compact16, dim3((unsigned)m.T), dim3(256), 0, st, m, tab, out);
+  return hipGetLastError();
+}
 hipError_t sf_launch_maf_ctab16(const SfDev& m, const float* x, long M, float* tab, hipStream_t st) {
   hipLaunchKernelGGL(k_maf_ctab16, dim3((unsigned)((M + 63) / 64), (unsigned)m.T), dim3(256), 0, st, m, x, M, tab);
   return hipGetLastError();
@@ -722,8 +774,7 @@
 static hipError_t sf_launch16q_p(const SfDev& m, const SfSampleArgsHost& a, hipStream_t st) {
   static SfAttrCache attr;
   static SfResidentCache rcache;
-  const size_t sh = ((size_t)(m.ctab ? m.t16_a_tab : m.t16_a) + (size_t)SfHid16<PREC>::lds_floats(m, !SPAN)) * sizeof(float) +
-                    (SF_Q_WORDS(64 * SF_SAMP16_TPW) + 96) * sizeof(unsigned int);
+  const size_t sh = (size_t)sf_lds_floats16<PREC>(m, !SPAN) * sizeof(float) + (SF_Q_WORDS(64 * SF_SAMP16_TPW) + 96) * sizeof(unsigned int);
   if (sh > 160 * 1024) return hipErrorInvalidValue;
   if (hipError_t e = sf_lds_optin16(k_maf_samp16<NB, SPAN, HM, DD, PREC>, attr); e != hipSuccess) return e;
   int resident = 0, cur_dev = 0;
diff --git a/synference_amd/csrc/sf_maf16_pass.h b/synference_amd/csrc/sf_maf16_pass.h
--- a/synference_amd/csrc/sf_maf16_pass.h
+++ b/synference_amd/csrc/sf_maf16_pass.h
@@ -647,8 +647,6 @@
 }
 template <> struct SfHid16<2> {
   using State = SfPass16G;
-  static __host__ __device__ int blk_floats(const SfDev& m) { return m.NB >= 2 ? m.nT16 * (m.nT16 + 1) / 2 * 256 : 0; }
-  static __host__ __device__ int lds_floats(const SfDev& m, bool ) { return blk_floats(m) + 4 * SF_G16_SCR; }
 };
 
 __device__ __forceinline__ void sf_copy_group16(const float4* g, float4* l) {
@@ -676,10 +674,9 @@
     }
     const int NT = m.nT16, nb = m.NB < 2 ? m.NB : 2;
     const int per = CP ? NT * (NT + 1) / 2 : NT * NT;
-    constexpr int K0 = PREC == 2 ? 1 : 0;
     float4* __restrict__ dF = d4 + (a_floats >> 2);
-    for (int e = __builtin_amdgcn_readfirstlane(wave); e < (nb - K0) * per; e += 4) {
-      const int k = K0 + (e >= per ? 1 : 0), ee = e - (k - K0) * per;
+    for (int e = __builtin_amdgcn_readfirstlane(wave); e < nb * per; e += 4) {
+      const int k = e >= per ? 1 : 0, ee = e - k * per;
       int src_blk = ee;
       if (CP) {
         const int ot = ee >= 6 ? 3 : (ee >= 3 ? 2 : (ee >= 1 ? 1 : 0));
diff --git a/synference_amd/engine.py b/synference_amd/engine.py
--- a/synference_amd/engine.py
+++ b/synference_amd/engine.py
@@ -93,6 +93,13 @@
             _lib.check(self.lib.sf_flow_pack_table16b(self.handle, s.ctypes.data_as(_lib.c_i32p), n))
         return s
 
+    def pack_table16c(self) -> np.ndarray:
+        n = int(self.lib.sf_flow_packed16c_size(self.handle))
+        s = np.empty(n, np.int32)
+        if n:
+            _lib.check(self.lib.sf_flow_pack_table16c(self.handle, s.ctypes.data_as(_lib.c_i32p), n))
+        return s
+
     TRC_FIELDS = ("ok NT NI t_stride g_stride o_win o_b0 o_w1 o_b1 o_w2 o_b2 o_wf o_bf o_wfT o_w2T o_w1T o_winT "
                   "g_win g_b0 g_w1 g_b1 g_w2 g_b2 g_wf g_bf kend0 kend1 kend2 kend3 kbeg0 kbeg1 kbeg2 kbeg3 c_insrc c_jobs "
                   "n_jobs").split()
@@ -124,6 +131,11 @@
             _lib.check(self.lib.sf_flow_describe(self.handle, buf, len(buf)))
             d = self._describe = json.loads(buf.value.decode())
         return dict(d)
+
+    def sampler_fused(self) -> bool:
+        buf = C.create_string_buffer(1 << 16)
+        _lib.check(self.lib.sf_flow_describe(self.handle, buf, len(buf)))
+        return bool(json.loads(buf.value.decode()).get("sampler_fused", 0))
 
     def _dev(self):
         if not torch.cuda.is_available():
```

After: 1.107 billion (median of 6 runs). +1.8%, better.
